# NVlabs/FasterViT

Measured on AMD Instinct MI355X. Metric: images/sec FasterViT-0 224x224 inference, bs=256/GPU, higher is better.
Workload: dtype f16; 1 GPU; faster_vit_0_224 inference, 224x224, batch 256/GPU, synthetic weights (tests/synth.py init family); global_batch=256, parallelism=dp1 (independent shards, no data-path collective), hat_operands=f16, streams=1

## Files before the change

fastervit_amd/_lib.py:

```python
from __future__ import annotations

import ctypes as C
import os
import subprocess

_HERE = os.path.dirname(os.path.abspath(__file__))
CSRC_DIR = os.path.join(_HERE, "csrc")
DIAG = os.environ.get("FVIT_DIAG", "0") == "1"
LIB_PATH = os.path.join(CSRC_DIR, "libfvit_hip_diag.so" if DIAG else "libfvit_hip.so")
if os.environ.get("FVIT_LIB_PATH"):
    LIB_PATH = os.path.abspath(os.environ["FVIT_LIB_PATH"])

FVIT_ABI_VERSION = 10
FVIT_F32, FVIT_F16, FVIT_BF16 = 0, 1, 2
FVIT_TILE_N, FVIT_TILE_K = 128, 64
FVIT_MASK_BIAS = -30000.0
FVIT_MAX_DENSE_SEQ = 208
FVIT_PROF_KINDS = 11

EXPORTED_SYMBOLS = (
    "fvit_abi_version", "fvit_last_error", "fvit_attention_spad", "fvit_attention_dense", "fvit_stage_workspace_bytes", "fvit_workspace_init",
    "fvit_hat_stage_forward", "fvit_hat_block_forward", "fvit_token_init", "fvit_token_init_dyn", "fvit_feature_tap", "fvit_token_init_dyn_backward", "fvit_feature_tap_backward", "fvit_window_partition", "fvit_window_reverse", "fvit_gemm_bias_act",
    "fvit_gemm_residual", "fvit_gemm_terms", "fvit_gemm_residual_splitk", "fvit_gemm_terms_lo", "fvit_window_attention_terms", "fvit_window_attention_long_terms",
    "fvit_gather_layernorm_terms", "fvit_win_mlp_fused_terms", "fvit_win_mlp_split_bytes", "fvit_win_mlp_fused_split", "fvit_win_block_fused_split",
    "fvit_win_block_fused_terms", "fvit_attn_block_fused_terms", "fvit_ct_block_fused_terms", "fvit_window_attention", "fvit_window_attention_long",
    "fvit_gather_layernorm", "fvit_ln_gemm_supported", "fvit_ln_gemm", "fvit_attn_block_supported", "fvit_attn_block_fused",
    "fvit_ct_block_supported", "fvit_ct_block_fused", "fvit_win_block_supported", "fvit_win_block_fused", "fvit_win_mlp_supported",
    "fvit_win_mlp_fused", "fvit_mlp_fused_supported", "fvit_mlp_fused", "fvit_bias_act_cl", "fvit_bias_residual_cl", "fvit_layernorm2d_cl", "fvit_map_pad_cl", "fvit_layernorm2d_crop_cl",
    "fvit_conv3x3_nhwc", "fvit_conv3x3_nhwc_terms", "fvit_conv3x3_dense_k", "fvit_conv3x3_patch_form", "fvit_conv3x3_nhwc_dense", "fvit_conv3x3_nhwc_px_dense", "fvit_conv3x3_c128_band_supported", "fvit_conv3x3_c128_band", "fvit_stem_conv3x3s2",
    "fvit_stem_fused", "fvit_window_attention_drop", "fvit_bwd_window_attention_drop", "fvit_global_avgpool_cl", "fvit_conv3x3_nhwc_px", "fvit_layernorm2d_px", "fvit_stem_conv3x3s2_px", "fvit_head_logits", "fvit_head_softmax_xent",
    "fvit_head_grad", "fvit_sgd_momentum", "fvit_bwd_blocks", "fvit_bwd_transpose16", "fvit_bwd_scale_cols", "fvit_bwd_gelu", "fvit_bwd_layernorm",
    "fvit_bwd_colsum_finish", "fvit_bwd_colsum16", "fvit_bwd_window_attention", "fvit_bwd_window_attention_long",
    "fvit_bwd_window_attention_long_workspace", "fvit_tune", "fvit_prof_enable", "fvit_prof_collect",
    "fvit_prof_records", "fvit_prof_kind_name",
    "fvit_hat_stage_forward_tail", "fvit_rows_avgpool", "fvit_conv3x3_c64_ln2d", "fvit_conv3x3_c128_band_ln2d",
)
DIAG_SYMBOLS = (
    "fvit_debug_lds_poison", "fvit_debug_regs_poison", "fvit_debug_poison_launches", "fvit_debug_rowhash_begin", "fvit_debug_rowhash_end",
    "fvit_debug_rowhash_dump", "fvit_debug_mlp_trace_begin", "fvit_debug_mlp_trace_end", "fvit_debug_mlp_inputs_begin", "fvit_debug_mlp_inputs_end",
    "fvit_debug_win_mlp_timeline", "fvit_debug_stem_timeline", "fvit_debug_conv_band_timeline", "fvit_debug_attn_block_timeline",
    "fvit_debug_ct_block_timeline",
)


class FvitDebugRowhashRecord(C.Structure):
    _fields_ = [("tag", C.c_char * 24), ("offset", C.c_int64), ("rows", C.c_int64)]


class FvitStageDesc(C.Structure):
    _fields_ = [(n, C.c_int32) for n in (
        "batch", "C", "heads", "dpad", "ws", "H", "W", "Hp", "Wp", "cw", "hier", "square", "hidden",
        "depth", "do_propagation", "operand_dtype", "spad", "gpad")] + [("qk_scale", C.c_float), ("weight_terms", C.c_int32)]


class FvitAttnWeights(C.Structure):
    _fields_ = [(n, C.c_void_p) for n in ("w_qkv", "b_qkv", "w_proj", "b_proj", "bias", "ln_w", "ln_b", "gamma",
                                                  "w_qkv_frag", "b_qkv_heads", "w_proj_frag", "rel_table")] + \
               [("rel_w", C.c_int32), ("rel_ng", C.c_int32)]


class FvitMlpWeights(C.Structure):
    _fields_ = [(n, C.c_void_p) for n in ("w_fc1", "b_fc1", "w_fc2", "b_fc2", "ln_w", "ln_b", "gamma", "w_fc1_frag", "w_fc2_frag")]


class FvitBlockWeights(C.Structure):
    _fields_ = [("attn", FvitAttnWeights), ("mlp", FvitMlpWeights), ("hat_attn", FvitAttnWeights),
                ("hat_mlp", FvitMlpWeights), ("pe_x", C.c_void_p), ("pe_ct", C.c_void_p),
                ("last", C.c_int32), ("_pad", C.c_int32)]


class FvitStageTables(C.Structure):
    _fields_ = [(n, C.c_void_p) for n in ("ln1_src", "ln1_add", "ct_src", "up_idx")]


class FvitStageTail(C.Structure):
    _fields_ = [("ln_w", C.c_void_p), ("ln_b", C.c_void_p), ("pool_out", C.c_void_p), ("ln_eps", C.c_float), ("pool_dtype", C.c_int32)]


class FvitMapView(C.Structure):
    _fields_ = [("data", C.c_void_p), ("stride_b", C.c_int64), ("stride_c", C.c_int64), ("stride_h", C.c_int64),
                ("stride_w", C.c_int64), ("dtype", C.c_int32), ("_pad", C.c_int32)]


class FvitProfEntry(C.Structure):
    _fields_ = [("launches", C.c_int64), ("ms", C.c_double), ("flops", C.c_double), ("bytes", C.c_double)]


class FvitProfRecord(C.Structure):
    _fields_ = [("kind", C.c_int32), ("grid", C.c_int32), ("ms", C.c_float), ("_pad", C.c_float), ("flops", C.c_double),
                ("bytes", C.c_double), ("name", C.c_char * 40)]


_lib = None


def build(verbose: bool = False) -> str:
    cmd = ["make", "-C", CSRC_DIR, "-j4"]
    res = subprocess.run(cmd, stdout=subprocess.PIPE, stderr=subprocess.STDOUT, text=True)
    if verbose:
        print(res.stdout)
    if res.returncode != 0 or not os.path.isfile(LIB_PATH):
        raise RuntimeError("building libfvit_hip.so failed:\n" + res.stdout)
    return LIB_PATH


def _declare(lib):
    vp, i32, f32 = C.c_void_p, C.c_int32, C.c_float
    lib.fvit_abi_version.restype = C.c_int
    lib.fvit_last_error.restype = C.c_char_p
    lib.fvit_attention_spad.restype = C.c_int
    lib.fvit_attention_spad.argtypes = [i32]
    lib.fvit_stage_workspace_bytes.restype = C.c_size_t
    lib.fvit_stage_workspace_bytes.argtypes = [C.POINTER(FvitStageDesc)]
    lib.fvit_workspace_init.restype = C.c_int
    lib.fvit_workspace_init.argtypes = [C.POINTER(FvitStageDesc), vp, C.c_size_t, vp]
    lib.fvit_hat_stage_forward.restype = C.c_int
    lib.fvit_hat_stage_forward.argtypes = [C.POINTER(FvitStageDesc), C.POINTER(FvitBlockWeights),
                                           C.POINTER(FvitStageTables), C.POINTER(FvitMapView), vp,
                                           C.POINTER(FvitMapView), vp, C.c_size_t, vp]
    lib.fvit_hat_stage_forward_tail.restype = C.c_int
    lib.fvit_hat_stage_forward_tail.argtypes = [C.POINTER(FvitStageDesc), C.POINTER(FvitBlockWeights),
                                                C.POINTER(FvitStageTables), C.POINTER(FvitMapView), vp,
                                                C.POINTER(FvitMapView), C.POINTER(FvitStageTail), vp, C.c_size_t, vp]
    lib.fvit_rows_avgpool.restype = C.c_int
    lib.fvit_rows_avgpool.argtypes = [i32, vp, vp, i32, i32, i32, vp]
    for fn in (lib.fvit_conv3x3_c64_ln2d, lib.fvit_conv3x3_c128_band_ln2d):
        fn.restype = C.c_int
        fn.argtypes = [i32, vp, vp, vp, vp, vp, vp, vp, f32, i32, i32, i32, vp, vp]
    lib.fvit_hat_block_forward.restype = C.c_int
    lib.fvit_hat_block_forward.argtypes = [C.POINTER(FvitStageDesc), C.POINTER(FvitBlockWeights),
                                           C.POINTER(FvitStageTables), vp, vp, vp, C.c_size_t, vp]
    lib.fvit_token_init.restype = C.c_int
    lib.fvit_token_init.argtypes = [C.POINTER(FvitMapView), vp, vp, vp, i32, i32, i32, i32, i32, i32, i32, i32, i32, vp]
    lib.fvit_token_init_dyn.restype = C.c_int
    lib.fvit_token_init_dyn.argtypes = [C.POINTER(FvitMapView), vp, vp, vp, i32, i32, i32, i32, i32, i32, i32, i32, i32, vp]
    lib.fvit_feature_tap.restype = C.c_int
    lib.fvit_feature_tap.argtypes = [C.POINTER(FvitMapView), i32, i32, i32, i32, vp, vp, vp, vp]
    lib.fvit_token_init_dyn_backward.restype = C.c_int
    lib.fvit_token_init_dyn_backward.argtypes = [C.POINTER(FvitMapView), vp, vp, vp, vp, vp, vp, i32, i32, i32, i32, i32, i32, i32, i32, i32, vp]
    lib.fvit_feature_tap_backward.restype = C.c_int
    lib.fvit_feature_tap_backward.argtypes = [vp, C.POINTER(FvitMapView), C.POINTER(FvitMapView), i32, i32, i32, i32, i32, i32, vp, vp, C.c_int64, vp, vp]
    lib.fvit_window_partition.restype = C.c_int
    lib.fvit_window_partition.argtypes = [C.POINTER(FvitMapView), i32, i32, i32, i32, i32, vp, vp]
    lib.fvit_window_reverse.restype = C.c_int
    lib.fvit_window_reverse.argtypes = [vp, i32, i32, i32, i32, i32, i32, i32, C.POINTER(FvitMapView), vp]
    lib.fvit_gemm_bias_act.restype = C.c_int
    lib.fvit_gemm_bias_act.argtypes = [i32, vp, i32, vp, i32, vp, vp, i32, i32, i32, i32, i32, vp]
    lib.fvit_gemm_residual.restype = C.c_int
    lib.fvit_gemm_residual.argtypes = [i32, vp, i32, vp, i32, vp, vp, vp, i32, i32, i32, i32, vp]
    lib.fvit_gemm_terms.restype = C.c_int
    lib.fvit_gemm_terms.argtypes = [i32, vp, i32, vp, i32, vp, vp, vp, i32, i32, i32, i32, i32, i32, vp]
    lib.fvit_gemm_residual_splitk.restype = C.c_int
    lib.fvit_gemm_residual_splitk.argtypes = [i32, vp, i32, vp, i32, vp, vp, vp, i32, i32, i32, i32, vp, C.c_size_t, vp]
    lib.fvit_gemm_terms_lo.restype = C.c_int
    lib.fvit_gemm_terms_lo.argtypes = [i32, vp, i32, vp, i32, vp, vp, vp, i32, i32, i32, i32, i32, i32, i32, vp]
    lib.fvit_window_attention_terms.restype = C.c_int
    lib.fvit_window_attention_terms.argtypes = [i32, vp, i32, i32, vp, i32, i32, vp, i32, i32, i32, i32, f32, vp]
    lib.fvit_window_attention_long_terms.restype = C.c_int
    lib.fvit_window_attention_long_terms.argtypes = [i32, vp, i32, i32, vp, i32, i32, vp, i32, i32, i32, i32, i32, i32, f32, vp]
    lib.fvit_gather_layernorm_terms.restype = C.c_int
    lib.fvit_gather_layernorm_terms.argtypes = [i32, vp, i32, vp, i32, vp, vp, vp, vp, vp, i32, i32, vp, vp, f32, i32, i32, i32, vp]
    lib.fvit_win_mlp_fused_terms.restype = C.c_int
    lib.fvit_win_mlp_fused_terms.argtypes = [i32, vp, i32, i32, i32, vp, vp, f32, vp, vp, vp, vp, vp, i32, vp]
    lib.fvit_win_mlp_split_bytes.restype = C.c_size_t
    lib.fvit_win_mlp_split_bytes.argtypes = [i32, i32, i32]
    lib.fvit_win_mlp_fused_split.restype = C.c_int
    lib.fvit_win_mlp_fused_split.argtypes = [i32, vp, i32, i32, i32, vp, vp, f32, vp, vp, vp, vp, vp, i32, vp, vp, i32, vp]
    lib.fvit_window_attention.restype = C.c_int
    lib.fvit_window_attention.argtypes = [i32, vp, i32, vp, i32, vp, i32, i32, i32, i32, f32, vp]
    lib.fvit_attention_dense.restype = C.c_int
    lib.fvit_attention_dense.argtypes = [i32, i32]
    lib.fvit_window_attention_long.restype = C.c_int
    lib.fvit_window_attention_long.argtypes = [i32, vp, i32, vp, i32, vp, i32, i32, i32, i32, i32, i32, f32, vp]
    lib.fvit_gather_layernorm.restype = C.c_int
    lib.fvit_gather_layernorm.argtypes = [i32, vp, i32, vp, i32, vp, vp, vp, vp, vp, i32, vp, vp, f32, i32, i32, i32, vp]
    lib.fvit_ln_gemm_supported.restype = C.c_int
    lib.fvit_ln_gemm_supported.argtypes = [i32, i32, i32, i32]
    lib.fvit_ln_gemm.restype = C.c_int
    lib.fvit_ln_gemm.argtypes = [i32, vp, i32, vp, i32, vp, vp, vp, vp, vp, vp, f32, i32, i32, i32, vp, i32, vp, vp, i32, i32, i32, vp]
    lib.fvit_attn_block_supported.restype = C.c_int
    lib.fvit_attn_block_supported.argtypes = [i32, i32, i32]
    lib.fvit_attn_block_fused.restype = C.c_int
    lib.fvit_attn_block_fused.argtypes = [i32, vp, i32, vp, i32, vp, vp, vp, vp, vp, f32, i32, vp, vp, vp, vp, vp, vp, vp, i32, i32, i32, i32,
                                          f32, vp]
    lib.fvit_mlp_fused_supported.restype = C.c_int
    lib.fvit_mlp_fused_supported.argtypes = [i32, i32]
    lib.fvit_mlp_fused.restype = C.c_int
    lib.fvit_mlp_fused.argtypes = [i32, vp, i32, i32, i32, vp, vp, f32, vp, vp, vp, vp, vp, vp]
    lib.fvit_bias_act_cl.restype = C.c_int
    lib.fvit_bias_act_cl.argtypes = [i32, vp, vp, C.c_int64, i32, i32, vp]
    lib.fvit_bias_residual_cl.restype = C.c_int
    lib.fvit_bias_residual_cl.argtypes = [i32, vp, vp, vp, C.c_int64, i32, vp]
    lib.fvit_layernorm2d_cl.restype = C.c_int
    lib.fvit_layernorm2d_cl.argtypes = [i32, vp, vp, vp, vp, f32, C.c_int64, i32, i32, vp]
    lib.fvit_map_pad_cl.restype = C.c_int
    lib.fvit_map_pad_cl.argtypes = [i32, vp, vp, i32, i32, i32, i32, i32, i32, vp]
    lib.fvit_layernorm2d_crop_cl.restype = C.c_int
    lib.fvit_layernorm2d_crop_cl.argtypes = [i32, vp, vp, vp, vp, f32, i32, i32, i32, i32, i32, i32, i32, vp]
    lib.fvit_conv3x3_nhwc.restype = C.c_int
    lib.fvit_conv3x3_nhwc.argtypes = [i32, vp, vp, vp, vp, vp, i32, i32, i32, i32, i32, i32, i32, vp, vp]
    lib.fvit_conv3x3_nhwc_terms.restype = C.c_int
    lib.fvit_conv3x3_nhwc_terms.argtypes = [i32, vp, vp, vp, vp, vp, i32, i32, i32, i32, i32, i32, i32, i32, vp, vp]
    lib.fvit_window_attention_drop.restype = C.c_int
    lib.fvit_window_attention_drop.argtypes = [i32, vp, i32, vp, i32, vp, i32, i32, i32, i32, f32, vp, vp]
    lib.fvit_bwd_window_attention_drop.restype = C.c_int
    lib.fvit_bwd_window_attention_drop.argtypes = [i32, vp, i32, vp, i32, vp, i32, f32, vp, vp, i32, i32, i32, i32, vp, vp]
# ... 176 lines not shown
```

fastervit_amd/conv_runtime.py:

```python
from __future__ import annotations

import ctypes
import os
from typing import NamedTuple, Optional

import torch
import torch.nn.functional as F

from . import _lib, hat_runtime

_CODE = {torch.float16: _lib.FVIT_F16, torch.bfloat16: _lib.FVIT_BF16}


def _stream(device=None):
    return torch.cuda.current_stream(device).cuda_stream


def _bn_scale_shift(bn):
    s = bn.weight.float() / torch.sqrt(bn.running_var.float() + bn.eps)
    t = bn.bias.float() - bn.running_mean.float() * s
    return s, t


def _fold(conv, bn, extra_scale=None):
    s, t = _bn_scale_shift(bn)
    w = conv.weight.float() * s.view(-1, 1, 1, 1)
    b = t if conv.bias is None else conv.bias.float() * s + t
    if extra_scale is not None:
        w = w * extra_scale.float().view(-1, 1, 1, 1)
        b = b * extra_scale.float()
    return w, b


def frag_pack_conv128(w2d: torch.Tensor) -> torch.Tensor:
    assert tuple(w2d.shape) == (128, 1152)
    dev = w2d.device
    wave = torch.arange(4, device=dev).view(4, 1, 1)
    ni = torch.arange(2, device=dev).view(1, 2, 1)
    sl = torch.arange(16, device=dev).view(1, 1, 16)
    ch = (32 * wave + (sl >> 2) * 8 + ni * 4 + (sl & 3)).reshape(-1)
    t = w2d[ch].view(4, 2, 16, 36, 4, 8)
    return t.permute(0, 3, 1, 4, 2, 5).contiguous().view(4, 36, 2, 64, 8)


class ConvWeight(NamedTuple):
    wcl: torch.Tensor
    wk: Optional[torch.Tensor]
    wband: Optional[torch.Tensor]
    terms: int
    cv: int
    wk_classic: Optional[torch.Tensor]


StemW = NamedTuple("StemW", [("conv0", ConvWeight), ("bias0", torch.Tensor), ("conv1", ConvWeight), ("bias1", torch.Tensor)])
BlockW = NamedTuple("BlockW", [("conv1", ConvWeight), ("bias1", torch.Tensor), ("conv2", ConvWeight), ("bias2", torch.Tensor)])
DownW = NamedTuple("DownW", [("ln_w", torch.Tensor), ("ln_b", torch.Tensor), ("eps", float), ("conv", ConvWeight), ("cin", int)])
TokW = NamedTuple("TokW", [("w", torch.Tensor), ("bias", torch.Tensor), ("pool_kernel", object), ("pool_stride", object), ("window", int)])
HeadW = NamedTuple("HeadW", [("w", torch.Tensor), ("b", torch.Tensor), ("ln", Optional[tuple])])


class DeployPlan:
    def __init__(self, model, dtype=torch.float16):
        if dtype not in _CODE:
            raise ValueError("deploy dtype must be torch.float16 or torch.bfloat16")
        self.model = model
        self.dtype = dtype
        self.code = _CODE[dtype]
        self.sig = None
        self.t = None
        self.zeros = None
        self.streams = 1
        self.shard_sizes = None
        self.serialize_shards = False
        self.join_from = None
        self.slot_base = 0
        self._warm_geometries = set()
        self.side = None
        self.dev = None
        self.use_hip_conv = True
        self.pad_channels = True
        self.down_weight_terms = int(os.environ.get("FVIT_DOWN_WEIGHT_TERMS", "1"))
        self.conv_weight_terms = int(os.environ.get("FVIT_CONV_WEIGHT_TERMS", "1"))
        self.precise = os.environ.get("FVIT_PRECISE_DEPLOY", "0") == "1"
        self.dense_k = os.environ.get("FVIT_CONV_DENSE_K", "1") != "0"
        self.fused_stem = os.environ.get("FVIT_NO_FUSED_STEM", "0") != "1"
        self.fuse_conv_ln2d = {64: os.environ.get("FVIT_FUSE_CONV64_LN2D", "1") != "0", 128: os.environ.get("FVIT_FUSE_CONV128_LN2D", "1") != "0"}
        self.fuse_reverse_ln2d = os.environ.get("FVIT_FUSE_REVERSE_LN2D", "1") != "0"
        self.fuse_pool = os.environ.get("FVIT_FUSE_POOL", "1") != "0"

    def _signature(self):
        m = self.model
        sig = []
        for name, p in list(m.named_parameters()) + list(m.named_buffers()):
            if ".blocks." in name and name.startswith(("levels.2.", "levels.3.")):
                continue
            sig.append((p.data_ptr(), p._version))
        sig.append(("options", self.precise, self.conv_weight_terms, self.down_weight_terms, self.dense_k))
        return tuple(sig)

    def _cp(self, c):
        return c if (c % 64 == 0 or c <= 3 or not (self.pad_channels and self.use_hip_conv)) else (c + 63) // 64 * 64

    def _padv(self, v, n):
        if v is None or v.numel() == n:
            return v
        out = torch.zeros(n, dtype=v.dtype, device=v.device)
        out[:v.numel()] = v
        return out

    def _cw(self, w, terms: int = 1) -> ConvWeight:
        co0, ci0 = w.shape[:2]
        cop, cip = self._cp(co0), self._cp(ci0)
        if (cop, cip) != (co0, ci0):
            wp = torch.zeros((cop, cip) + tuple(w.shape[2:]), dtype=w.dtype, device=w.device)
            wp[:co0, :ci0] = w
            w = wp
        wcl = w.to(self.dtype).contiguous(memory_format=torch.channels_last)
        co, ci, kh, kw = w.shape
        wk = wband = None
        cv = ci
        if self.use_hip_conv and kh == 3 and kw == 3 and ci % 64 == 0 and co % 64 == 0:
            wk = wcl.permute(0, 2, 3, 1).contiguous()
            lo = (w - wcl.float()).to(self.dtype).permute(0, 2, 3, 1).contiguous() if terms == 2 else None
            cv8 = (ci0 + 7) // 8 * 8
            if self.dense_k and cv8 < ci:
                cv, kd = cv8, (9 * cv8 + 63) // 64 * 64

                def dense(m):
                    d = torch.zeros((co, kd), dtype=m.dtype, device=m.device)
                    d[:, :9 * cv] = m[..., :cv].reshape(co, 9 * cv)
                    return d
                classic = wk.reshape(co, -1) if lo is None else torch.cat([wk.reshape(co, -1), lo.reshape(co, -1)], dim=1).contiguous()
                wk = dense(wk) if lo is None else torch.cat([dense(wk), dense(lo)], dim=1).contiguous()
                return ConvWeight(wcl, wk, None, terms, cv, classic)
            if terms == 2:
                wk = torch.cat([wk.reshape(co, -1), lo.reshape(co, -1)], dim=1).contiguous()
                return ConvWeight(wcl, wk, None, 2, cv, None)
            if (co, ci) == (128, 128):
                wband = frag_pack_conv128(wk.reshape(128, 1152))
        return ConvWeight(wcl, wk, wband, 1, cv, None)

    def _zero_page(self, device):
        if self.zeros is None or self.zeros.device != device:
            self.zeros = torch.zeros(256, dtype=self.dtype, device=device)
        return self.zeros.data_ptr()

    @staticmethod
    def _conv_launch_shape(x, w: ConvWeight, stride):
        B, Ci, Hi, Wi = x.shape
        wk, cv, Co = w.wk, w.cv, w.wk.shape[0]
        if w.wk_classic is not None and _lib.lib().fvit_conv3x3_patch_form(B, Hi, Wi, Ci, Co, stride):
            wk, cv = w.wk_classic, Ci
        return wk, cv, Co, (Hi - 1) // stride + 1, (Wi - 1) // stride + 1

    def _conv_ln2d_route(self, x, w: ConvWeight, d: "DownW"):
        C_ = x.shape[1]
        if self.precise or not self.use_hip_conv or not self.fuse_conv_ln2d.get(C_, False) or d.cin != C_ or w.wk is None or w.terms != 1 \
                or w.wk_classic is not None or not x.is_contiguous(memory_format=torch.channels_last):
            return None
        lib = _lib.lib()
        if C_ == 64 and tuple(w.wk.shape) == (64, 3, 3, 64):
            return "halo"
        if C_ == 128 and w.wband is not None and lib.fvit_conv3x3_c128_band_supported(x.shape[2], x.shape[3]):
            return "band"
        return None

    def _conv_ln2d(self, route, x, w: ConvWeight, bias, residual, d: "DownW"):
        B, _, Hi, Wi = x.shape
        fn, wt, name = ((_lib.lib().fvit_conv3x3_c64_ln2d, w.wk, "fvit_conv3x3_c64_ln2d") if route == "halo" else
                        (_lib.lib().fvit_conv3x3_c128_band_ln2d, w.wband, "fvit_conv3x3_c128_band_ln2d"))
        _lib.check(fn(self.code, x.data_ptr(), wt.data_ptr(), bias.data_ptr() if bias is not None else None, residual.data_ptr(), residual.data_ptr(),
                      d.ln_w.data_ptr(), d.ln_b.data_ptr(), d.eps, B, Hi, Wi, self._zero_page(x.device), _stream(self.dev)), name)
        return residual

    def _conv(self, x, w: ConvWeight, bias, stride, act, residual=None):
        B, Ci, Hi, Wi = x.shape
        if w.wk is not None and x.is_contiguous(memory_format=torch.channels_last):
            wk, cv, Co, Ho, Wo = self._conv_launch_shape(x, w, stride)
            out = residual if residual is not None else torch.empty((B, Co, Ho, Wo), dtype=self.dtype, device=x.device,
                                                                    memory_format=torch.channels_last)
            zeros = self._zero_page(x.device)
            if w.wband is not None and stride == 1 and _lib.lib().fvit_conv3x3_c128_band_supported(Hi, Wi):
                rc = _lib.lib().fvit_conv3x3_c128_band(self.code, x.data_ptr(), w.wband.data_ptr(), bias.data_ptr() if bias is not None else None,
                                                       residual.data_ptr() if residual is not None else None, out.data_ptr(), B, Hi, Wi, act,
                                                       zeros, _stream(self.dev))
                _lib.check(rc, "fvit_conv3x3_c128_band")
                return out
            rc = _lib.lib().fvit_conv3x3_nhwc_dense(self.code, x.data_ptr(), wk.data_ptr(), bias.data_ptr() if bias is not None else None,
                                                    residual.data_ptr() if residual is not None else None, out.data_ptr(), B, Hi, Wi,
                                                    Ci, cv, Co, stride, act, w.terms, zeros, _stream(self.dev))
            _lib.check(rc, "fvit_conv3x3_nhwc_dense")
            return out
        y = F.conv2d(x, w.wcl, None, stride, 1)
        if residual is not None:
            return self._bias_residual(residual, y, bias)
        return self._bias_act(y, bias, act) if bias is not None else y

    @torch.no_grad()
    def _build(self):
        m = self.model
        t = {}
        pe = m.patch_embed.conv_down
        w0, b0 = _fold(pe[0], pe[1])
        w1, b1 = _fold(pe[3], pe[4])
        ct = 2 if (self.conv_weight_terms == 2 or self.precise) else 1
        t["stem"] = StemW(self._cw(w0), self._padv(b0, self._cp(b0.numel())).contiguous(), self._cw(w1, terms=ct),
                          self._padv(b1, self._cp(b1.numel())).contiguous())
        t["stem_k"] = t["stem_k_lo"] = None
        co0 = self._cp(w0.shape[0])
        w0p = torch.zeros((co0,) + tuple(w0.shape[1:]), dtype=torch.float32, device=w0.device)
        w0p[:w0.shape[0]] = w0
        t["stem0_f32"] = (w0p.contiguous(memory_format=torch.channels_last), self._padv(b0, co0).contiguous(), tuple(pe[0].stride))
        if self.use_hip_conv and tuple(w0.shape) == (64, 3, 3, 3) and pe[0].stride == (2, 2):
            wk = torch.zeros(64, 32, device=w0.device, dtype=torch.float32)
            wk[:, :27] = w0.permute(0, 2, 3, 1).reshape(64, 27)
            t["stem_k"] = wk.to(self.dtype).contiguous()
            t["stem_k_lo"] = (wk - t["stem_k"].float()).to(self.dtype).contiguous()
        t["levels"] = []
        for lvl in m.levels:
            e = {}
            if not lvl.transformer_block:
                blocks = []
                for blk in lvl.blocks:
                    wa, ba = _fold(blk.conv1, blk.norm1)
                    wb, bb = _fold(blk.conv2, blk.norm2, blk.gamma if blk.layer_scale else None)
                    cpd = self._cp(ba.numel())
                    blocks.append(BlockW(self._cw(wa, terms=ct), self._padv(ba, cpd).contiguous(), self._cw(wb, terms=ct), self._padv(bb, cpd).contiguous()))
                e["blocks"] = blocks
            elif getattr(lvl, "do_gt", False):
                tk = lvl.global_tokenizer
                e["tok"] = TokW(self._cw(tk.pos_embed.weight.float()).wcl, tk.pos_embed.bias.to(self.dtype).contiguous(),
                                tk.to_global_feature.pool.kernel_size, tk.to_global_feature.pool.stride, tk.window_size)
            if lvl.downsample is not None:
                ds = lvl.downsample
                cin = ds.norm.weight.numel()
                e["down"] = DownW(self._padv(ds.norm.weight.float(), self._cp(cin)).contiguous(),
                                  self._padv(ds.norm.bias.float(), self._cp(cin)).contiguous(), float(ds.norm.eps),
                                  self._cw(ds.reduction[0].weight.float(), terms=2 if (self.down_weight_terms == 2 or ct == 2) else 1), cin)
            t["levels"].append(e)
        self._build_head(t)
        self.t = t

    def _build_head(self, t):
        m = self.model
        if isinstance(m.head, torch.nn.Linear):
            hw = m.head.weight.float()
            hb = m.head.bias.float() if m.head.bias is not None else torch.zeros(hw.shape[0], device=hw.device)
        else:
# ... 82 lines not shown

    def _forward_sharded(self, x):
        n = self.streams
        if n <= 1 or x.shape[0] < 2 * n:
            with hat_runtime.workspace_slot(self.slot_base):
                return self._forward_one(x)
        sb, sizes, warm = self.slot_base, self.shard_sizes, self._warm_geometries
        parts = x.split(list(sizes), dim=0) if sizes and sum(sizes) == x.shape[0] and len(sizes) == n else x.chunk(n, dim=0)
        outs = [None] * n
        ops = tuple(getattr(lvl, "hat_operand_dtype", "f16") for lvl in self.model.levels if lvl.transformer_block)
        wkey = (str(x.device), tuple(p.shape[0] for p in parts), tuple(x.shape[1:]), ops, self.join_from, sb)
        serial = self.serialize_shards or not self._hat_prepared(x.device) or wkey not in warm
        jf = self.join_from if (self.join_from is not None and 0 < self.join_from < len(self.model.levels)) else None
        front = (lambda xi: self._forward_one(xi, 0, jf)) if jf is not None else self._forward_one
        def _cat(xs):
            if isinstance(xs[0], tuple):
                return tuple(None if xs[0][k] is None else torch.cat([x_[k] for x_ in xs], dim=0) for k in range(3))
            return torch.cat(xs, dim=0)
        back = (lambda xs: self._forward_one(_cat(xs), jf, None)) if jf is not None else (lambda xs: torch.cat(xs, dim=0))
        if serial:
            for i in range(n):
                with hat_runtime.workspace_slot(sb + i):
                    outs[i] = front(parts[i])
            with hat_runtime.workspace_slot(sb):
                y = back(outs)
            if not torch.cuda.is_current_stream_capturing():
                warm.add(wkey)
            return y
        if self.side is None or len(self.side) != n - 1 or self.side[0].device != x.device:
            self.side = [torch.cuda.Stream(device=x.device) for _ in range(n - 1)]
        main = torch.cuda.current_stream(x.device)
        for i, s in enumerate(self.side):
            s.wait_stream(main)
            with torch.cuda.stream(s), hat_runtime.workspace_slot(sb + i + 1):
                outs[i + 1] = front(parts[i + 1])
        with hat_runtime.workspace_slot(sb):
            outs[0] = front(parts[0])
        for s in self.side:
            main.wait_stream(s)
        with hat_runtime.workspace_slot(sb):
            return back(outs)

    def shard_runner(self, x, n=None):
        return ShardRunner(self, x, n or max(self.streams, 1))

    def _conv_px(self, x, x_lo, w: ConvWeight, bias, stride, act, res=None, res_lo=None, want="planes"):
        if w.wk is None or not x.is_contiguous(memory_format=torch.channels_last):
            raise RuntimeError("precise deploy plan: this conv shape has no implicit-GEMM kernel (channel counts must pad to multiples of 64)")
        B, Ci, Hi, Wi = x.shape
        wk, cv, Co, Ho, Wo = self._conv_launch_shape(x, w, stride)
        zeros = self._zero_page(x.device)
        hi = lo = f32 = None
        if want == "f32":
            f32 = torch.empty((B, Co, Ho, Wo), dtype=torch.float32, device=x.device, memory_format=torch.channels_last)
        else:
            hi = res if res is not None else torch.empty((B, Co, Ho, Wo), dtype=self.dtype, device=x.device, memory_format=torch.channels_last)
            if want == "planes":
                lo = res_lo if res_lo is not None else torch.empty_like(hi)
        rc = _lib.lib().fvit_conv3x3_nhwc_px_dense(self.code, x.data_ptr(), x_lo.data_ptr() if x_lo is not None else None, wk.data_ptr(),
                                             bias.data_ptr() if bias is not None else None, res.data_ptr() if res is not None else None,
                                             res_lo.data_ptr() if res_lo is not None else None, hi.data_ptr() if hi is not None else None,
                                             lo.data_ptr() if lo is not None else None, f32.data_ptr() if f32 is not None else None,
                                             B, Hi, Wi, Ci, cv, Co, stride, act, w.terms, zeros, _stream(self.dev))
        _lib.check(rc, "fvit_conv3x3_nhwc_px_dense")
        return f32 if want == "f32" else (hi, lo)

    def _ln2d_px(self, x, x_lo, x_f32, w, b, eps, c_valid):
        src = x_f32 if x_f32 is not None else x
        B, C, H, W = src.shape
        if C % 8 or not src.is_contiguous(memory_format=torch.channels_last):
            raise RuntimeError("precise deploy plan: LayerNorm2d needs a channels_last map with C % 8 == 0")
        hi = torch.empty((B, C, H, W), dtype=self.dtype, device=src.device, memory_format=torch.channels_last)
        lo = torch.empty_like(hi)
        _lib.check(_lib.lib().fvit_layernorm2d_px(self.code, x.data_ptr() if x is not None else None, x_lo.data_ptr() if x_lo is not None else None,
                                                  x_f32.data_ptr() if x_f32 is not None else None, hi.data_ptr(), lo.data_ptr(), w.data_ptr(),
                                                  b.data_ptr(), eps, B * H * W, C, c_valid, _stream(self.dev)), "fvit_layernorm2d_px")
        return hi, lo

    def _forward_one(self, x, lv_from=0, lv_to=None):
        levels = self.model.levels
        with torch.autocast(device_type="cuda", enabled=False):
            if lv_from == 0:
                x = self._stem(x)
            for li, (lvl, e) in enumerate(zip(levels, self.t["levels"])):
                if li < lv_from or (lv_to is not None and li >= lv_to):
                    continue
                normed = pooled = False
                if "blocks" in e:
                    x, normed = self._conv_level(x, e["blocks"], e.get("down"))
                elif self._pool_tail(lvl, x, last=li + 1 == len(levels) and lv_to is None and "down" not in e):
                    x, pooled = self._hat_level_pooled(lvl, x), True
                else:
                    x, normed = self._hat_level(lvl, x, padded_out="down" in e, down=e.get("down"))
                if "down" in e:
                    x = self._downsample(x, e["down"], f32_out=li + 1 < len(levels) and levels[li + 1].transformer_block, normed=normed)
            if lv_to is not None:
                return x
            return self._head_logits(x, *self.t["head"][:2]) if pooled else self._head(x)

    def _stem(self, x):
        t, st = self.t, self.t["stem"]
        k27 = t["stem_k"] is not None and x.shape[1] == 3 and x.dtype in hat_runtime._DT
        if self.precise:
            if not k27:
                wf, bf, st0 = t["stem0_f32"]
                y = torch.relu(F.conv2d(x.float(), wf, bf, st0, 1)).to(self.dtype).contiguous(memory_format=torch.channels_last)
            else:
                B, _, Hi, Wi = x.shape
                y = torch.empty((B, 64, (Hi - 1) // 2 + 1, (Wi - 1) // 2 + 1), dtype=self.dtype, device=x.device, memory_format=torch.channels_last)
                view = hat_runtime._map_view(x)
                _lib.check(_lib.lib().fvit_stem_conv3x3s2_px(self.code, view, t["stem_k"].data_ptr(), t["stem_k_lo"].data_ptr(), st.bias0.data_ptr(),
                                                             y.data_ptr(), B, Hi, Wi, _stream(self.dev)), "fvit_stem_conv3x3s2_px")
            return (*self._conv_px(y, None, st.conv1, st.bias1, 2, 1), None)
        wk1 = st.conv1.wk
        if self.fused_stem and k27 and wk1 is not None and st.conv1.terms == 1 and tuple(wk1.shape) == (64, 3, 3, 64):
            B, _, Hi, Wi = x.shape
            H1, W1 = (Hi - 1) // 2 + 1, (Wi - 1) // 2 + 1
            y = torch.empty((B, 64, (H1 - 1) // 2 + 1, (W1 - 1) // 2 + 1), dtype=self.dtype, device=x.device,
                            memory_format=torch.channels_last)
            view = hat_runtime._map_view(x)
            _lib.check(_lib.lib().fvit_stem_fused(self.code, view, t["stem_k"].data_ptr(), st.bias0.data_ptr(), wk1.data_ptr(),
                                                  st.bias1.data_ptr(), y.data_ptr(), B, Hi, Wi, _stream(self.dev)), "fvit_stem_fused")
            return y
        if k27:
            B, _, Hi, Wi = x.shape
            y = torch.empty((B, 64, (Hi - 1) // 2 + 1, (Wi - 1) // 2 + 1), dtype=self.dtype, device=x.device,
                            memory_format=torch.channels_last)
            view = hat_runtime._map_view(x)
            _lib.check(_lib.lib().fvit_stem_conv3x3s2(self.code, view, t["stem_k"].data_ptr(), st.bias0.data_ptr(), y.data_ptr(),
                                                      B, Hi, Wi, _stream(self.dev)), "fvit_stem_conv3x3s2")
            return self._conv(y, st.conv1, st.bias1, 2, 1)
        x = x.to(self.dtype).contiguous(memory_format=torch.channels_last)
        return self._conv(self._conv(x, st.conv0, st.bias0, 2, 1), st.conv1, st.bias1, 2, 1)

    def _conv_level(self, x, blocks, down: Optional["DownW"] = None):
        if not self.precise:
            normed = False
            for i, b in enumerate(blocks):
                y = self._conv(x, b.conv1, b.bias1, 1, 2)
                route = self._conv_ln2d_route(y, b.conv2, down) if (down is not None and i + 1 == len(blocks)) else None
                if route is not None:
                    x, normed = self._conv_ln2d(route, y, b.conv2, b.bias2, x, down), True
                else:
                    x = self._conv(y, b.conv2, b.bias2, 1, 0, residual=x)
            return x, normed
        hi, lo, f32 = x
        if hi is None:
            hi = f32.to(self.dtype)
            lo = (f32 - hi.float()).to(self.dtype)
        for b in blocks:
            y, _ = self._conv_px(hi, None, b.conv1, b.bias1, 1, 2, want="single")
            hi, lo = self._conv_px(y, None, b.conv2, b.bias2, 1, 0, res=hi, res_lo=lo)
        return (hi, lo, None), False

    def _pool_tail(self, lvl, x, last):
        return (last and self.fuse_pool and not self.precise and self.t["head"].ln is None and torch.is_tensor(x) and len(lvl.blocks) > 0
                and x.shape[1] == lvl.blocks[0].attn.qkv.in_features and x.shape[1] % 16 == 0 and self.t["head"].w.shape[1] == x.shape[1]
                and hat_runtime.pool_tail_supported(lvl, x))

    def _hat_level_pooled(self, lvl, x):
        feat = torch.empty((x.shape[0], x.shape[1]), dtype=torch.float32, device=x.device)
        return hat_runtime.stage_forward(lvl, x, pool_out=feat)

    def _hat_level(self, lvl, x, padded_out, tokenizer=None, down: Optional["DownW"] = None):
        if self.precise:
            hi, lo, x = x
            if x is None:
                x = hi.float() + lo.float()
        creal = lvl.blocks[0].attn.qkv.in_features if len(lvl.blocks) else x.shape[1]
        xin = x[:, :creal] if x.shape[1] != creal else x
        cpo = self._cp(creal) if padded_out else creal
        xo = torch.empty((x.shape[0], cpo, x.shape[2], x.shape[3]), dtype=torch.float32 if self.precise else self.dtype, device=x.device,
                         memory_format=torch.channels_last)
        if cpo != creal:
            xo[:, creal:] = 0
            hat_runtime.stage_forward(lvl, xin, tokenizer=tokenizer, out=xo[:, :creal])
            return ((None, None, xo) if self.precise else xo), False
        if (down is not None and self.fuse_reverse_ln2d and not self.precise and down.cin == creal and len(lvl.blocks)
                and hat_runtime.ln2d_tail_supported(xin, xo)):
            return hat_runtime.stage_forward(lvl, xin, tokenizer=tokenizer, out=xo, ln2d=(down.ln_w, down.ln_b, down.eps)), True
        xo = hat_runtime.stage_forward(lvl, xin, tokenizer=tokenizer, out=xo)
        return ((None, None, xo) if self.precise else xo), False

    def _downsample(self, x, d: DownW, f32_out, normed=False):
        if not self.precise:
            return self._conv(x if normed else self._ln2d(x, d.ln_w, d.ln_b, d.eps, d.cin), d.conv, None, 2, 0)
        hi, lo, f32 = x
        if f32 is not None and not f32.is_contiguous(memory_format=torch.channels_last):
            f32 = f32.contiguous(memory_format=torch.channels_last)
        nh, nl = self._ln2d_px(hi, lo, f32, d.ln_w, d.ln_b, d.eps, d.cin)
        if f32_out:
            return None, None, self._conv_px(nh, nl, d.conv, None, 2, 0, want="f32")
        return (*self._conv_px(nh, nl, d.conv, None, 2, 0), None)

    def _head(self, x):
        hw, hb, ln = self.t["head"]
        if not self.precise:
            return self._pool_head(x if ln is None else self._ln2d(x, *ln), hw, hb)
        hi, lo, f32 = x
        if f32 is None:
            f32 = hi.float() + lo.float()
        if ln is not None:
            nh, nl = self._ln2d_px(None, None, f32.contiguous(memory_format=torch.channels_last), *ln, f32.shape[1])
            f32 = nh.float() + nl.float()
        return self._pool_head(f32, hw, hb)


class LevelMap(NamedTuple):
    x: torch.Tensor
    H: int
    W: int

    @property
    def dense(self) -> bool:
        return self.x.shape[2] == self.H and self.x.shape[3] == self.W


TapW = NamedTuple("TapW", [("scale", torch.Tensor), ("shift", torch.Tensor), ("channels", int)])


class BackboneDeployPlan(DeployPlan):

    def __init__(self, model, dtype=torch.float16):
        super().__init__(model, dtype)
        self._check_options()
        for i in model.out_indices:
            bn = getattr(model, f"norm{i}")
            hat_runtime._folded_bn(bn, (bn.running_mean if bn.running_mean is not None else next(model.parameters())).device)

    def _check_options(self):
        if self.precise:
            raise NotImplementedError("backbone deploy plan: precise=True is not implemented (there is no two-term feature tap); use the 16-bit plan, "
                                      "or module mode with set_hat_operand_dtype('f16x3')")
        if self.conv_weight_terms != 1 or self.down_weight_terms != 1:
            raise NotImplementedError("backbone deploy plan: two-term conv weights (conv_weight_terms / down_weight_terms = 2) are not implemented")
        if self.streams != 1:
            raise NotImplementedError("backbone deploy plan: streams > 1 (stream shards) is not implemented; detection batches are small")

    def _build_head(self, t):
        m = self.model
        dev = next(m.parameters()).device
        t["taps"] = {i: TapW(*hat_runtime._folded_bn(getattr(m, f"norm{i}"), dev), m.num_features[i]) for i in m.out_indices}

    def forward(self, x):
        self._check_options()
        self._enter(x)
        with torch.cuda.device(x.device):
            self._refresh()
            with hat_runtime.workspace_slot(self.slot_base):
                return self._walk(x)

    forward_single = forward

    def _walk(self, x):
        levels, taps = self.model.levels, self.t["taps"]
        outs = []
        with torch.autocast(device_type="cuda", enabled=False):
            y = self._stem(x)
            m = LevelMap(y, y.shape[2], y.shape[3])
            for li, (lvl, e) in enumerate(zip(levels, self.t["levels"])):
                if "blocks" in e:
                    m = self._conv_level_padded(m, e["blocks"], lvl.window_size)
                else:
                    m = self._hat_level_dyn(lvl, m, padded_out="down" in e)
                if li in taps:
                    outs.append(self._tap(m, taps[li]))
                if "down" in e:
                    m = self._downsample_crop(m, e["down"])
        return tuple(outs)
# ... 89 lines not shown
```

fastervit_amd/csrc/fvit_api.hip:

```cpp
#include <stdarg.h>
#include <stdlib.h>
#include <string.h>

#include <algorithm>
#include <map>
#include <mutex>
#include <string>
#include <vector>

#include "fvit_common.h"

namespace fvit {

static thread_local char g_err[512] = "";

void set_error(const char* fmt, ...) {
    va_list ap;
    va_start(ap, fmt);
    vsnprintf(g_err, sizeof(g_err), fmt, ap);
    va_end(ap);
}

int check_launch(const char* what) {
    hipError_t e = hipGetLastError();
// ... 423 lines not shown
        break;
    }
    case WinAttnRoute::CHAIN: {
        LnCall ln1 = ln_call(d, L, a.ln_w, a.ln_b, X, L.Mx, win.xn);
        ln1.rowsA = L.rpi; ln1.srcB = R; ln1.rowsB = L.G; ln1.src_idx = d.hier ? t.ln1_src : nullptr; ln1.add_idx = t.ln1_add; ln1.add = w.pe_x;
        ln1.x_out = X; ln1.rows_per_image = L.rpi;
        FVIT_TRY(launch_gather_layernorm(ln1, st));
        dbg_rowhash("win.gather", X, L.Mx, d.C * 4, st);
        FVIT_TRY(run_attn(d, L, a, AttnStart::QKV_GEMM, win, ws, st));
        break;
    }
    }
    return run_mlp(d, L, w.mlp, r.window_mlp, r, win, t, ws, st);
}

static int check_hat_call(const FvitStageDesc* desc, bool args_ok, const FvitStageTables* t, const void* workspace, size_t workspace_bytes,
                          const void* carrier, const char* no_carrier, StageLayout& L) {
    if (!desc || !args_ok) {
        set_error("null argument");
        return FVIT_EINVAL;
    }
    const FvitStageDesc& d = *desc;
    if (!make_layout(d, L)) return FVIT_EINVAL;
    if (!t || !t->ln1_add || (d.hier && (!t->ln1_src || !t->ct_src)) || (d.hier && d.do_propagation && !t->up_idx)) {
        set_error("stage tables missing (ln1_add%s)", d.hier ? ", ln1_src, ct_src, up_idx" : "");
        return FVIT_EINVAL;
    }
    if (!workspace || workspace_bytes < L.total) {
        set_error("workspace too small: %zu < %zu", workspace_bytes, L.total);
        return FVIT_EWORKSPACE;
    }
    if (d.hier && !carrier) {
        set_error("%s", no_carrier);
        return FVIT_EINVAL;
    }
    return FVIT_OK;
}

}

using namespace fvit;

extern "C" {

int fvit_abi_version(void) { return FVIT_ABI_VERSION; }
const char* fvit_last_error(void) { return g_err; }

int fvit_attention_dense(int32_t S, int32_t dpad) { return attention_dense(S, dpad) ? 1 : 0; }

int fvit_attention_spad(int32_t S) {
    int sb = (S + 15) / 16;
    if (sb == 9) sb = 10;
    if (sb == 11 || sb == 12) sb = 13;
    return sb * 16;
}

size_t fvit_stage_workspace_bytes(const FvitStageDesc* desc) {
    StageLayout L;
    if (!desc || !make_layout(*desc, L)) return 0;
    return L.total;
}

int fvit_workspace_init(const FvitStageDesc* desc, void* workspace, size_t bytes, fvit_stream_t stream) {
    StageLayout L;
    if (!desc || !make_layout(*desc, L)) return FVIT_EINVAL;
    if (!workspace || bytes < L.total) {
        set_error("workspace too small: %zu < %zu", bytes, L.total);
        return FVIT_EWORKSPACE;
    }
    if (hipMemsetAsync(workspace, 0, L.total, (hipStream_t)stream) != hipSuccess) return check_launch("workspace memset");
    return FVIT_OK;
}

int fvit_hat_stage_forward(const FvitStageDesc* desc, const FvitBlockWeights* blocks, const FvitStageTables* tables,
                           const FvitMapView* in, const float* ct_init, const FvitMapView* out, void* workspace,
                           size_t workspace_bytes, fvit_stream_t stream) {
    return fvit_hat_stage_forward_tail(desc, blocks, tables, in, ct_init, out, nullptr, workspace, workspace_bytes, stream);
}

int fvit_rows_avgpool(int32_t round_dtype, const float* x, float* out, int32_t B, int32_t rows, int32_t C, fvit_stream_t stream) {
    return launch_rows_avgpool(x, out, B, rows, C, round_dtype, (hipStream_t)stream);
}

int fvit_hat_stage_forward_tail(const FvitStageDesc* desc, const FvitBlockWeights* blocks, const FvitStageTables* tables,
                                const FvitMapView* in, const float* ct_init, const FvitMapView* out, const FvitStageTail* tail,
                                void* workspace, size_t workspace_bytes, fvit_stream_t stream) {
    StageLayout L;
    const bool pooled = tail && tail->pool_out;
    FVIT_TRY(check_hat_call(desc, blocks && in && (out || pooled), tables, workspace, workspace_bytes, ct_init, "hierarchical stage needs ct_init", L));
    const FvitStageDesc& d = *desc;
    if (tail && (!tail->ln_w != !tail->ln_b || (pooled && tail->ln_w))) {
        set_error("stage tail: LayerNorm2d needs both ln_w and ln_b, and excludes pool_out");
        return FVIT_EINVAL;
    }
    if (pooled && (d.hier || L.nW != 1 || L.ncw != 0 || d.H != d.Hp || d.W != d.Wp)) {
        set_error("stage tail: pool_out needs one window per image and no carrier tokens (hier=%d, %d windows, map %dx%d of %dx%d)", d.hier, L.nW, d.H, d.W,
                  d.Hp, d.Wp);
        return FVIT_EINVAL;
    }
    hipStream_t st = (hipStream_t)stream;
    char* ws = (char*)workspace;
    float* X = (float*)(ws + L.off_X);
    PartitionCall pc = {*in, d.batch, d.C, d.Hp, d.Wp, d.ws, X, L.S, L.ncw, d.hier ? ct_init : nullptr, L.ncw};
    FVIT_TRY(launch_partition(pc, st));
    dbg_rowhash("partition", X, L.Mx, d.C * 4, st);
    const RouteKnobs knobs{};
    std::vector<BlockRoute> routes;
    for (int i = 0; i < d.depth; ++i) routes.push_back(choose_route(d, L, blocks[i], knobs));
    for (int i = 0; i + 1 < d.depth; ++i) {
        if (routes[i].preadd_eligible && routes[i + 1].preadd_eligible && blocks[i + 1].pe_x) {
            routes[i].pe_next = blocks[i + 1].pe_x;
            routes[i + 1].window_attn = WinAttnRoute::LNGEMM_PREADDED;
        }
    }
    for (int i = 0; i < d.depth; ++i) FVIT_TRY(run_block(d, L, routes[i], blocks[i], *tables, ws, st));
    if (pooled)
        return launch_rows_avgpool(X, tail->pool_out, d.batch, L.S, d.C, tail->pool_dtype, st);
    const bool prop = d.hier && d.do_propagation && d.depth > 0 && blocks[d.depth - 1].last;
    ReverseCall rc = {X, L.S, L.ncw, d.batch, d.C, d.Hp, d.Wp, d.H, d.W, d.ws, *out,
                      prop ? blocks[d.depth - 1].hat_attn.gamma : nullptr, prop ? tables->up_idx : nullptr};
    if (tail && tail->ln_w) return launch_reverse_ln(rc, tail->ln_w, tail->ln_b, tail->ln_eps, st);
    FVIT_TRY(launch_reverse(rc, st));
    return FVIT_OK;
}

int fvit_hat_block_forward(const FvitStageDesc* desc, const FvitBlockWeights* block, const FvitStageTables* tables, float* x,
                           float* ct, void* workspace, size_t workspace_bytes, fvit_stream_t stream) {
    StageLayout L;
    FVIT_TRY(check_hat_call(desc, block && x, tables, workspace, workspace_bytes, ct, "hierarchical block needs carrier tokens", L));
    const FvitStageDesc& d = *desc;
    hipStream_t st = (hipStream_t)stream;
    char* ws = (char*)workspace;
    float* X = (float*)(ws + L.off_X);
    const int nwin = d.batch * L.nW;
    FVIT_TRY(launch_ct_copy(X, L.S, L.ncw, L.nloc, x, nwin, d.C, 1, st));
    if (d.hier) FVIT_TRY(launch_ct_copy(X, L.S, 0, L.ncw, ct, nwin, d.C, 1, st));
    FVIT_TRY(run_block(d, L, choose_route(d, L, *block, RouteKnobs{}), *block, *tables, ws, st));
    if (d.hier && block->last && d.do_propagation)
        FVIT_TRY(launch_propagate(X, block->hat_attn.gamma, tables->up_idx, L.S, L.ncw, L.nloc, nwin, d.C, st));
    FVIT_TRY(launch_ct_copy(X, L.S, L.ncw, L.nloc, x, nwin, d.C, 0, st));
    if (d.hier) FVIT_TRY(launch_ct_copy(X, L.S, 0, L.ncw, ct, nwin, d.C, 0, st));
    return FVIT_OK;
}

int fvit_token_init(const FvitMapView* in, const float* weight, const float* bias, float* ct_out, int32_t batch, int32_t C, int32_t Hp,
                    int32_t Wp, int32_t pool_kh, int32_t pool_kw, int32_t pool_sh, int32_t pool_sw, int32_t cw, fvit_stream_t stream) {
    if (!in || !weight || !bias || !ct_out) { set_error("null argument"); return FVIT_EINVAL; }
    return launch_token_init(*in, weight, bias, ct_out, batch, C, Hp, Wp, pool_kh, pool_kw, pool_sh, pool_sw, cw, (hipStream_t)stream);
}

int fvit_window_partition(const FvitMapView* in, int32_t batch, int32_t C, int32_t Hp, int32_t Wp, int32_t ws, float* windows,
                          fvit_stream_t stream) {
    if (!in || !windows) { set_error("null argument"); return FVIT_EINVAL; }
    PartitionCall pc = {*in, batch, C, Hp, Wp, ws, windows, ws * ws, 0, nullptr, 0};
    return launch_partition(pc, (hipStream_t)stream);
}

int fvit_window_reverse(const float* windows, int32_t batch, int32_t C, int32_t Hp, int32_t Wp, int32_t H, int32_t W, int32_t ws,
                        const FvitMapView* out, fvit_stream_t stream) {
    if (!out || !windows) { set_error("null argument"); return FVIT_EINVAL; }
    ReverseCall rc = {windows, ws * ws, 0, batch, C, Hp, Wp, H, W, ws, *out, nullptr, nullptr};
    return launch_reverse(rc, (hipStream_t)stream);
}

int fvit_gemm_bias_act(int32_t operand_dtype, const void* A, int32_t lda, const void* Wt, int32_t ldw, const float* bias, void* out,
                       int32_t ldo, int32_t M, int32_t N, int32_t K, int32_t act, fvit_stream_t stream) {
    GemmCall g = {operand_dtype, A, lda, Wt, ldw, bias, nullptr, out, ldo, M, N, K, act ? 1 : 0};
    return launch_gemm(g, (hipStream_t)stream);
}

int fvit_gemm_residual(int32_t operand_dtype, const void* A, int32_t lda, const void* Wt, int32_t ldw, const float* bias,
                       const float* gamma, float* x, int32_t ldx, int32_t M, int32_t N, int32_t K, fvit_stream_t stream) {
    GemmCall g = {operand_dtype, A, lda, Wt, ldw, bias, gamma, x, ldx, M, N, K, 2};
    return launch_gemm(g, (hipStream_t)stream);
}

int fvit_gemm_residual_splitk(int32_t operand_dtype, const void* A, int32_t lda, const void* Wt, int32_t ldw, const float* bias, const float* gamma,
                              float* x, int32_t ldx, int32_t M, int32_t N, int32_t K, float* slab, size_t slab_bytes, fvit_stream_t stream) {
    GemmCall g = {operand_dtype, A, lda, Wt, ldw, bias, gamma, x, ldx, M, N, K, 2};
    g.splitk_slab = slab;
    g.splitk_bytes = slab_bytes;
    return launch_gemm(g, (hipStream_t)stream);
}

int fvit_gemm_terms(int32_t operand_dtype, const void* A, int32_t lda, const void* Wt, int32_t ldw, const float* bias, const float* gamma,
                    void* out, int32_t ldo, int32_t M, int32_t N, int32_t K, int32_t ka, int32_t epilogue, fvit_stream_t stream) {
    if (epilogue < 0 || epilogue > 2) { set_error("gemm_terms: epilogue %d", epilogue); return FVIT_EINVAL; }
    GemmCall g = {operand_dtype, A, lda, Wt, ldw, bias, epilogue == 2 ? gamma : nullptr, out, ldo, M, N, K, epilogue};
    g.ka = ka;
    return launch_gemm(g, (hipStream_t)stream);
}

int fvit_gemm_terms_lo(int32_t operand_dtype, const void* A, int32_t lda, const void* Wt, int32_t ldw, const float* bias, const float* gamma,
                       void* out, int32_t ldo, int32_t out_lo_off, int32_t M, int32_t N, int32_t K, int32_t ka, int32_t epilogue,
                       fvit_stream_t stream) {
    if (epilogue < 0 || epilogue > 2) { set_error("gemm_terms_lo: epilogue %d", epilogue); return FVIT_EINVAL; }
    GemmCall g = {operand_dtype, A, lda, Wt, ldw, bias, epilogue == 2 ? gamma : nullptr, out, ldo, M, N, K, epilogue};
    g.ka = ka;
    g.out_lo_off = out_lo_off;
    return launch_gemm(g, (hipStream_t)stream);
}

int fvit_window_attention_terms(int32_t operand_dtype, const void* qkv, int32_t ldq, int32_t q_lo_off, void* out, int32_t ldo,
                                int32_t o_lo_off, const float* bias, int32_t nwin, int32_t S, int32_t heads, int32_t dpad, float scale,
                                fvit_stream_t stream) {
    AttnCall a = {operand_dtype, qkv, ldq, out, ldo, bias, nwin, S, heads, dpad, scale, nullptr, 0, 0, 0};
    a.q_lo_off = q_lo_off;
    a.o_lo_off = o_lo_off;
    if (q_lo_off <= 0 || o_lo_off <= 0) { set_error("window_attention_terms: q_lo_off / o_lo_off must be > 0"); return FVIT_EINVAL; }
    return launch_attention(a, (hipStream_t)stream);
}

int fvit_gather_layernorm_terms(int32_t operand_dtype, const float* srcA, int32_t rowsA, const float* srcB, int32_t rowsB,
                                const int32_t* src_idx, const int32_t* add_idx, const float* add, float* x_out, void* n_out, int32_t ldn,
                                int32_t lo_off, const float* ln_w, const float* ln_b, float eps, int32_t rows, int32_t rows_per_image,
                                int32_t C, fvit_stream_t stream) {
    LnCall c = {operand_dtype, srcA, rowsA, srcB, rowsB, src_idx, add_idx, add, x_out, n_out, ldn, ln_w, ln_b, eps, rows,
                rows_per_image, C};
    c.lo_off = lo_off;
    return launch_gather_layernorm(c, (hipStream_t)stream);
}

int fvit_window_attention(int32_t operand_dtype, const void* qkv, int32_t ldq, void* out, int32_t ldo, const float* bias,
                          int32_t nwin, int32_t S, int32_t heads, int32_t dpad, float scale, fvit_stream_t stream) {
    if (!attention_dense(S, dpad)) {
        set_error("window_attention: S=%d at dpad=%d is outside the dense-bias kernel (fvit_attention_dense); use fvit_window_attention_long", S, dpad);
        return FVIT_EINVAL;
    }
    AttnCall a = {operand_dtype, qkv, ldq, out, ldo, bias, nwin, S, heads, dpad, scale, nullptr, 0, 0, 0};
    return launch_attention(a, (hipStream_t)stream);
}
// ... 282 lines not shown
```

fastervit_amd/csrc/fvit_common.h:

```cpp
#pragma once
#include <hip/hip_runtime.h>
#include <stdint.h>
#include <atomic>
#include <mutex>
#include <stdio.h>

#include "../../include/fvit_hip.h"

namespace fvit {

typedef _Float16 h8 __attribute__((ext_vector_type(8)));
typedef _Float16 h4 __attribute__((ext_vector_type(4)));
typedef __bf16 b8 __attribute__((ext_vector_type(8)));
typedef __bf16 b4 __attribute__((ext_vector_type(4)));
typedef float f4 __attribute__((ext_vector_type(4)));

template <typename T> struct Op16;
template <> struct Op16<_Float16> {
    typedef h8 v8;
    typedef h4 v4;
    static __device__ __forceinline__ f4 mfma(v8 a, v8 b, f4 c) {
        return __builtin_amdgcn_mfma_f32_16x16x32_f16(a, b, c, 0, 0, 0);
    }
};
// ... 326 lines not shown
    const void* drop_mask = nullptr;
};
bool attention_dense(int S, int dpad);
int launch_attention(const AttnCall& c, hipStream_t stream);
int launch_attention_long(const AttnCall& c, hipStream_t stream);

struct LnCall {
    int dtype;
    const float* srcA;
    int rowsA;
    const float* srcB;
    int rowsB;
    const int32_t* src_idx;
    const int32_t* add_idx;
    const float* add;
    float* x_out;
    void* n_out;
    int ldn;
    const float* ln_w;
    const float* ln_b;
    float eps;
    int rows, rows_per_image, C;
    int lo_off = 0;
};
int launch_gather_layernorm(const LnCall& c, hipStream_t stream);

struct CtBlkCall {
    int dtype;
    const float* X; int rowsA;
    const int32_t* src_idx;
    const float* add;
    float* R;
    int batch, G, heads, C, hidden;
    const float* ln1_w; const float* ln1_b; const void* wqkv_f; const float* bqkv; const void* wproj_f; const float* bproj; const float* gamma1;
    const float* bias; float scale;
    const float* ln2_w; const float* ln2_b; const void* w1f; const float* b1; const void* w2f; const float* b2; const float* gamma2;
    float eps;
    int terms = 1;
    void* ts = nullptr;
};
bool ctblk_supported(int C, int heads, int G, int hidden);
int launch_ctblk(const CtBlkCall& c, hipStream_t stream);

struct LnGemmCall {
    LnCall ln;
    const void* W;
    int ldw;
    const float* bias;
    void* out;
    int ldo;
    int N;
    int epilogue;
};
bool ln_gemm_supported(int C, int N, int ldw, int ldo);
int launch_ln_gemm(const LnGemmCall& c, hipStream_t stream);

struct PartitionCall {
    FvitMapView in;
    int batch, C, Hp, Wp, ws;
    float* x;
    int rows_per_win;
    int row_off;
    const float* ct;
    int ncw;
};
int launch_partition(const PartitionCall& c, hipStream_t stream);

struct ReverseCall {
    const float* x;
    int rows_per_win, row_off;
    int batch, C, Hp, Wp, H, W, ws;
    FvitMapView out;
    const float* gamma;
    const int32_t* up_idx;
};
int launch_reverse(const ReverseCall& c, hipStream_t stream);
bool reverse_ln_supported(const ReverseCall& c);
int launch_reverse_ln(const ReverseCall& c, const float* ln_w, const float* ln_b, float eps, hipStream_t stream);
int launch_rows_avgpool(const float* x, float* out, int batch, int rows, int C, int round_dtype, hipStream_t stream);

int launch_ct_copy(float* x, int rows_per_win, int row_off, int ncw, float* ct, int nwin_total, int C, int to_x,
                   hipStream_t stream);
int launch_token_init(const FvitMapView& in, const float* w, const float* bias, float* out, int B, int C, int Hp, int Wp, int kh, int kw,
                      int sh, int sw, int cw, hipStream_t stream);
int launch_propagate(float* x, const float* gamma, const int32_t* up_idx, int rows_per_win, int ncw, int nloc,
                     int nwin_total, int C, hipStream_t stream);

}
```

fastervit_amd/csrc/fvit_conv.hip:

```cpp
#include "fvit_common.h"

namespace fvit {

namespace {

constexpr int BK = 64;

struct ConvParams {
    const void* in;
    const void* w;
    const float* bias;
    const void* res;
    void* out;
    const void* zeros;
    int B, Hi, Wi, Cin, Cout, Ho, Wo, stride, act;
    int M, tiles_m, tiles_n;
    int ablate;
    int wterms;
    const void* in_lo;
    const void* res_lo;
    void* out_lo;
    float* out_f32;
    int px;
    int cv, kd;
    float inv_cv;
};

__device__ __forceinline__ int swz_x(int r) { return (r >> 1) & 7; }
__device__ __forceinline__ int swz_w(int r) { return ((0x78 >> (2 * ((r >> 4) & 3))) & 3) | ((r & 2) << 1); }

__device__ __forceinline__ void glds16(const void* gsrc, char* lds_dst) {
    __builtin_amdgcn_global_load_lds((const __attribute__((address_space(1))) void*)gsrc,
                                     (__attribute__((address_space(3))) void*)lds_dst, 16, 0, 0);
}

template <int V> struct IntTag { static constexpr int value = V; };
template <typename F>
__device__ __forceinline__ void dispatch_epilogue(int act, bool has_res, F&& body) {
    if (has_res) {
        if (act == 0) body(IntTag<0>{}, IntTag<1>{});
        else if (act == 1) body(IntTag<1>{}, IntTag<1>{});
        else body(IntTag<2>{}, IntTag<1>{});
    } else {
        if (act == 0) body(IntTag<0>{}, IntTag<0>{});
        else if (act == 1) body(IntTag<1>{}, IntTag<0>{});
        else body(IntTag<2>{}, IntTag<0>{});
    }
}

constexpr int PATCH_H = 8, PATCH_W = 16, PHALO_W = PATCH_W + 2, PHALO_ROWS = (PATCH_H + 2) * PHALO_W;
constexpr int PHALO_PIECES = (PHALO_ROWS + 7) / 8;
constexpr int PHALO_BYTES = PHALO_PIECES * 1024;

template <typename T, int WM, int WN, int NI, bool PX = false, bool DENSE = false, bool HALO = false>
__global__ __launch_bounds__(256, 2) void conv3x3_kernel(ConvParams p) {
    typedef typename Op16<T>::v8 v8;
    static_assert(!HALO || (WM == 2 && WN == 2 && !DENSE), "halo form: 8 x 16 patches on the 2 x 2 wave grid, classic weight layout");
    constexpr int BM = 64 * WM, BN = 16 * NI * WN;
    constexpr int X_BYTES = HALO ? PHALO_BYTES : BM * BK * 2, W_BYTES = BN * BK * 2;
    constexpr int XP = BM / 8 / 4;
    constexpr int HP = (PHALO_PIECES + 3) / 4;
    constexpr int WPIECES = BN / 8;
    constexpr int WP = (WPIECES + 3) / 4;
    static_assert(2 * (X_BYTES + W_BYTES) <= 80 * 1024, "two workgroups per CU");
    __shared__ __attribute__((aligned(16))) char smem[2 * (X_BYTES + W_BYTES)];

    const int tid = threadIdx.x;
    const int lane = tid & 63;
    const int wave = __builtin_amdgcn_readfirstlane(tid >> 6);
    const int wm = wave / WN, wn = wave - wm * WN;

    const int nblk = gridDim.x, b = blockIdx.x;
    const int q = nblk >> 3, rr = nblk & 7, xcd = b & 7, idx = b >> 3;
    const int v = (xcd < rr ? xcd * (q + 1) : rr * (q + 1) + (xcd - rr) * q) + idx;
    const int tm = v / p.tiles_n, tn = v - tm * p.tiles_n;
    const int m0 = tm * BM, n0 = tn * BN;

    const T* __restrict__ In = (const T*)p.in;
    const T* __restrict__ W = (const T*)p.w;
    const T* __restrict__ Z = (const T*)p.zeros;
    const int ldw = DENSE ? p.wterms * p.kd * BK : p.wterms * 9 * p.Cin;

    f4 acc[NI][4];
#pragma unroll
    for (int i = 0; i < NI; ++i)
#pragma unroll
        for (int j = 0; j < 4; ++j) acc[i][j] = (f4){0.f, 0.f, 0.f, 0.f};

    const int g = lane >> 4, s = lane & 15;
    int bimg = 0, y0 = 0, x0 = 0;
    if constexpr (HALO) {
        const int tpx = (p.Wo + PATCH_W - 1) / PATCH_W, tpy = (p.Ho + PATCH_H - 1) / PATCH_H;
        bimg = tm / (tpy * tpx);
        const int rem = tm - bimg * (tpy * tpx);
        const int ty = rem / tpx;
        y0 = ty * PATCH_H;
        x0 = (rem - ty * tpx) * PATCH_W;
    }
    if constexpr (HALO) {
        int hoff[HP];
        int hvalid = 0;
        int hchunk[HP];
#pragma unroll
        for (int i = 0; i < HP; ++i) {
            const int piece = wave + 4 * i;
            const int r = piece * 8 + (lane >> 3);
            const int hy = r / PHALO_W, hx = r - hy * PHALO_W;
            const int iy = y0 - 1 + hy, ix = x0 - 1 + hx;
            const int chunk = ((lane & 7) ^ swz_x(r)) * 8;
            hchunk[i] = chunk;
            const bool ok = piece < PHALO_PIECES && r < PHALO_ROWS && iy >= 0 && iy < p.Hi && ix >= 0 && ix < p.Wi;
            if (ok) hvalid |= 1 << i;
            hoff[i] = ok ? ((bimg * p.Hi + iy) * p.Wi + ix) * p.Cin + chunk : 0;
        }
        const int ncc = p.Cin / BK;
        const int kpb_hi = p.wterms * 9;
        const int nblk_hi = ncc, nblk_all = ncc * ((PX && p.in_lo) ? 2 : 1);
        const int nk = nblk_hi * kpb_hi + (nblk_all - nblk_hi) * 9;
        const T* const InLo = (PX && p.in_lo) ? (const T*)p.in_lo : In;
        auto stage_halo = [&](int blk, char* xbuf) {
            const bool lo = blk >= nblk_hi;
            const T* const plane = lo ? InLo : In;
            const int c0 = (lo ? blk - nblk_hi : blk) * BK;
#pragma unroll
            for (int i = 0; i < HP; ++i) {
                const int piece = wave + 4 * i;
                if (piece < PHALO_PIECES) {
                    const T* src = ((hvalid >> i) & 1) ? plane + (hoff[i] + c0) : Z + hchunk[i];
                    glds16(src, xbuf + piece * 1024);
                }
            }
        };
        auto stage_w = [&](int blk, int kin, char* wbuf) {
            const bool lo = blk >= nblk_hi;
            const int c0 = (lo ? blk - nblk_hi : blk) * BK;
            const int col = kin * p.Cin + c0;
#pragma unroll
            for (int i = 0; i < WP; ++i) {
                const int piece = wave * WP + i;
// ... 149 lines not shown
            for (int i = 0; i < NI; ++i) wf[kk][i] = *(const v8*)(wt + wrow[i] * 128 + ((c ^ swz_w(wrow[i])) << 4));
        }
        __builtin_amdgcn_sched_barrier(0);
        if (!(p.ablate & 4))
#pragma unroll
        for (int kk = 0; kk < 2; ++kk)
#pragma unroll
            for (int ni = 0; ni < NI; ++ni)
#pragma unroll
                for (int mi = 0; mi < 4; ++mi) acc[ni][mi] = Op16<T>::mfma(wf[kk][ni], xf[kk][mi], acc[ni][mi]);
    }
    }
    if (p.ablate & 8) return;

    auto rowm = [&](int mi) {
        if constexpr (HALO) {
            const int y = y0 + wm * 4 + mi, x = x0 + s;
            return (y < p.Ho && x < p.Wo) ? (bimg * p.Ho + y) * p.Wo + x : p.M;
        } else {
            return m0 + wm * 64 + mi * 16 + s;
        }
    };
    constexpr int NC = 4 * NI;
    typedef T vout __attribute__((ext_vector_type(NC)));
    const int nb = n0 + wn * 16 * NI + g * NC;
    if (nb >= p.Cout) return;
    float bias[NC];
#pragma unroll
    for (int j = 0; j < NI; ++j) {
        const f4 t = p.bias ? *(const f4*)(p.bias + nb + j * 4) : (f4){0.f, 0.f, 0.f, 0.f};
        bias[j * 4 + 0] = t[0]; bias[j * 4 + 1] = t[1]; bias[j * 4 + 2] = t[2]; bias[j * 4 + 3] = t[3];
    }
    T* O = (T*)p.out;
    const T* R = (const T*)p.res;
    if constexpr (PX) {
        const T* RL = (const T*)p.res_lo;
        T* OL = (T*)p.out_lo;
        float* OF = p.out_f32;
        auto px_epilogue = [&](auto act_tag) {
            constexpr int ACT = decltype(act_tag)::value;
#pragma unroll
            for (int mi = 0; mi < 4; ++mi) {
                const int m = rowm(mi);
                if (m < p.M) {
                    float y[NC];
#pragma unroll
                    for (int ni = 0; ni < NI; ++ni)
#pragma unroll
                        for (int r = 0; r < 4; ++r) {
                            float v = acc[ni][mi][r] + bias[ni * 4 + r];
                            if (ACT == 1) v = fmaxf(v, 0.f);
                            y[ni * 4 + r] = v;
                        }
                    if constexpr (ACT == 2) gelu_erf_each<NC>(y);
                    if (R) {
                        const vout rv = *(const vout*)(R + (size_t)m * p.Cout + nb);
#pragma unroll
                        for (int j = 0; j < NC; ++j) y[j] += (float)rv[j];
                        if (RL) {
                            const vout rl = *(const vout*)(RL + (size_t)m * p.Cout + nb);
#pragma unroll
                            for (int j = 0; j < NC; ++j) y[j] += (float)rl[j];
                        }
                    }
                    if (OF) {
#pragma unroll
                        for (int j = 0; j < NC; j += 4) *(f4*)(OF + (size_t)m * p.Cout + nb + j) = (f4){y[j], y[j + 1], y[j + 2], y[j + 3]};
                    } else {
                        vout oh, ol;
#pragma unroll
                        for (int j = 0; j < NC; ++j) {
                            oh[j] = sat16<T>(y[j]);
                            ol[j] = sat16<T>(y[j] - (float)oh[j]);
                        }
                        *(vout*)(O + (size_t)m * p.Cout + nb) = oh;
                        if (OL) *(vout*)(OL + (size_t)m * p.Cout + nb) = ol;
                    }
                }
            }
        };
        if (p.act == 0) px_epilogue(IntTag<0>{});
        else if (p.act == 1) px_epilogue(IntTag<1>{});
        else px_epilogue(IntTag<2>{});
        return;
    }
    dispatch_epilogue(p.act, R != nullptr, [&](auto act_tag, auto res_tag) {
        constexpr int ACT = decltype(act_tag)::value;
        constexpr bool RES = decltype(res_tag)::value != 0;
        vout rvs[4];
        if (RES) {
#pragma unroll
            for (int mi = 0; mi < 4; ++mi) rvs[mi] = *(const vout*)(R + (size_t)min(rowm(mi), p.M - 1) * p.Cout + nb);
            __builtin_amdgcn_sched_barrier(0);
        }
#pragma unroll
        for (int mi = 0; mi < 4; ++mi) {
            const int m = rowm(mi);
            if (m < p.M) {
                vout rv;
                if (RES) rv = rvs[mi];
                vout ov;
                float yv[NI * 4];
#pragma unroll
                for (int ni = 0; ni < NI; ++ni) {
                    const f4 a = acc[ni][mi];
#pragma unroll
                    for (int r = 0; r < 4; ++r) {
                        float y = a[r] + bias[ni * 4 + r];
                        if (ACT == 1) y = fmaxf(y, 0.f);
                        yv[ni * 4 + r] = y;
                    }
                }
                if constexpr (ACT == 2) gelu_fast_each<NI * 4>(yv);
#pragma unroll
                for (int j = 0; j < NI * 4; ++j) ov[j] = (T)(RES ? yv[j] + (float)rv[j] : yv[j]);
                *(vout*)(O + (size_t)m * p.Cout + nb) = ov;
            }
        }
    });
}


struct StemParams {
    FvitMapView in;
    const void* w;
    const float* bias;
    void* out;
    int B, Hi, Wi, Ho, Wo, M;
    const void* w_lo;
};

__device__ __forceinline__ float stem_load(const FvitMapView& v, int64_t off) {
    if (v.dtype == FVIT_F32) return ((const float*)v.data)[off];
    if (v.dtype == FVIT_F16) return (float)((const _Float16*)v.data)[off];
    return (float)((const __bf16*)v.data)[off];
}

template <typename T, bool PX = false>
__global__ __launch_bounds__(256) void stem_conv_kernel(StemParams p) {
    typedef typename Op16<T>::v8 v8;
    const int lane = threadIdx.x & 63;
    const int g = lane >> 4, s = lane & 15;
    const T* __restrict__ W = (const T*)p.w;
    v8 wf[4], wl[4];
#pragma unroll
    for (int ni = 0; ni < 4; ++ni) wf[ni] = *(const v8*)(W + ((s >> 2) * 16 + ni * 4 + (s & 3)) * 32 + g * 8);
    if constexpr (PX) {
#pragma unroll
        for (int ni = 0; ni < 4; ++ni) wl[ni] = *(const v8*)((const T*)p.w_lo + ((s >> 2) * 16 + ni * 4 + (s & 3)) * 32 + g * 8);
    }
    float bias[16];
#pragma unroll
    for (int j = 0; j < 4; ++j) {
        const f4 t = *(const f4*)(p.bias + g * 16 + j * 4);
        bias[j * 4 + 0] = t[0]; bias[j * 4 + 1] = t[1]; bias[j * 4 + 2] = t[2]; bias[j * 4 + 3] = t[3];
    }
    T* __restrict__ O = (T*)p.out;
    const int hw = p.Ho * p.Wo;
    const int nblk16 = (p.M + 15) >> 4;
    int64_t toff[8];
    int tky[8], tkx[8];
#pragma unroll
    for (int e = 0; e < 8; ++e) {
        const int k = g * 8 + e;
        const int ky = k / 9, r9 = k - ky * 9, kx = r9 / 3, c = r9 - kx * 3;
        tky[e] = k < 27 ? ky : -100000;
// ... 874 lines not shown
                    }
                }
            }
            pf_sink ^= pf0 ^ pf1;
        }
        FVIT_SF_MARK(tsA)
        __syncthreads();
        FVIT_SF_MARK(tsBar)

        const char* hb = img + (2 * ph * 4) * SF_ROWPITCH;
        f4 acc[2][4];
#pragma unroll
        for (int i = 0; i < 2; ++i)
#pragma unroll
            for (int j = 0; j < 4; ++j) acc[i][j] = (f4){0.f, 0.f, 0.f, 0.f};
        v8 xf[2][4];
#pragma unroll
        for (int mi = 0; mi < 4; ++mi) xf[0][mi] = *(const v8*)(hb + (2 * mi) * SF_ROWPITCH + xoff[0]);
        __builtin_amdgcn_sched_barrier(0);
#pragma unroll
        for (int q = 0; q < 18; ++q) {
            const int tap = q >> 1, kk = q & 1;
            if (q + 1 < 18) {
                const int tap1 = (q + 1) >> 1, kk1 = (q + 1) & 1, ky1 = tap1 / 3, kx1 = tap1 - ky1 * 3;
                const int o = xoff[kx1] ^ (kk1 << 6);
#pragma unroll
                for (int mi = 0; mi < 4; ++mi) xf[(q + 1) & 1][mi] = *(const v8*)(hb + (2 * mi + ky1) * SF_ROWPITCH + o);
            }
#pragma unroll
            for (int ni = 0; ni < 2; ++ni)
#pragma unroll
                for (int mi = 0; mi < 4; ++mi) acc[ni][mi] = Op16<T>::mfma(wf[tap][kk][ni], xf[q & 1][mi], acc[ni][mi]);
            __builtin_amdgcn_sched_barrier(0);
        }

        FVIT_SF_MARK(tsB)
        const f4 t0 = *(const f4*)(sb2 + nb), t1 = *(const f4*)(sb2 + nb + 4);
        const float bias[8] = {t0[0], t0[1], t0[2], t0[3], t1[0], t1[1], t1[2], t1[3]};
        const int x = tx * HALO_TW + s;
#pragma unroll
        for (int mi = 0; mi < 4; ++mi) {
            const int y = ty * HALO_TH + ph * 4 + mi;
            if (y < p.H2 && x < p.W2) {
                v8 ov;
#pragma unroll
                for (int ni = 0; ni < 2; ++ni)
#pragma unroll
                    for (int r = 0; r < 4; ++r) ov[ni * 4 + r] = (T)fmaxf(acc[ni][mi][r] + bias[ni * 4 + r], 0.f);
                *(v8*)(O + (((size_t)b * p.H2 + y) * p.W2 + x) * 64 + nb) = ov;
            }
        }
        FVIT_SF_MARK(tsE)
    }
    if (pf_sink == 0x9E3779B1u && p.tiles == -12345) ((unsigned*)p.out)[0] = pf_sink;
    if constexpr (TS) {
        if (p.ts && lane == 0) {
            unsigned long long* o = p.ts + ((size_t)blockIdx.x * 4 + wave) * 8;
            o[0] = tsA; o[1] = tsBar; o[2] = tsB; o[3] = tsE; o[4] = tsBar0; o[5] = tsN; o[6] = __builtin_amdgcn_s_memtime() - tsT0; o[7] = 0;
        }
    }
#undef FVIT_SF_MARK
}

static bool patch_form_ok(const ConvParams& p) {
    if (!tune_get("conv_patch", 1) || p.stride != 1 || p.cv || p.Cout < 128 || (p.Cin % BK)) return false;
    if ((int64_t)p.B * p.Hi * p.Wi * p.Cin >= 0x7fffffffLL) return false;
    const int64_t tiles = (int64_t)p.B * ((p.Ho + PATCH_H - 1) / PATCH_H) * ((p.Wo + PATCH_W - 1) / PATCH_W);
    return tiles * 128 * 100 <= (int64_t)p.M * (100 + tune_get("conv_patch_max_waste_pct", 10));
}

template <typename T>
int launch_t(ConvParams& p, hipStream_t stream) {
    if (p.Cin == 64 && p.Cout == 64 && p.stride == 1 && p.wterms == 1 && !p.px && !p.cv && tune_get("conv_halo", 1)) {
        if (ablate_skip(64)) return FVIT_OK;
        return launch_halo_t<T>(p, stream);
    }
    if (ablate_skip(32)) return FVIT_OK;
    const double flops = 2.0 * p.M * (double)p.Cout * 9.0 * (p.cv ? p.cv : p.Cin);
    const double bytes = 2.0 * ((double)p.B * p.Hi * p.Wi * p.Cin * (p.in_lo ? 2.0 : 1.0) + (double)p.M * p.Cout * ((p.res ? (p.res_lo ? 2.0 : 1.0) : 0.0) + ((p.out_lo || p.out_f32) ? 2.0 : 1.0)) +
                               9.0 * p.wterms * p.Cin * p.Cout);
    ProfScope prof(FVIT_K_CONV, flops, bytes, stream);
    const int variant = tune_get("conv64_variant", 0);
    const int narrow = tune_get("conv128_narrow", 0);
    const bool patch = patch_form_ok(p) && (p.Cout % 128 == 0 || (p.Cout > 128 && tune_get("conv_n128_ragged", 1))) && !narrow;
    if (patch) {
        p.tiles_m = p.B * ((p.Ho + PATCH_H - 1) / PATCH_H) * ((p.Wo + PATCH_W - 1) / PATCH_W);
        p.tiles_n = (p.Cout + 127) / 128;
        const dim3 grid_(p.tiles_m * p.tiles_n);
        prof_note(p.px ? "conv3x3_kernel<2,2,4,px,patch>" : "conv3x3_kernel<2,2,4,patch>", p.tiles_m * p.tiles_n);
        if (p.px) hipLaunchKernelGGL((conv3x3_kernel<T, 2, 2, 4, true, false, true>), grid_, dim3(256), 0, stream, p);
        else hipLaunchKernelGGL((conv3x3_kernel<T, 2, 2, 4, false, false, true>), grid_, dim3(256), 0, stream, p);
        return check_launch("conv3x3_kernel<patch>");
    }
#define FVIT_CONV_LAUNCH(WM_, WN_, NI_, PX_)                                                                                            \
    do {                                                                                                                                \
        const dim3 grid_(p.tiles_m * p.tiles_n);                                                                                        \
        if (p.cv) hipLaunchKernelGGL((conv3x3_kernel<T, WM_, WN_, NI_, PX_, true>), grid_, dim3(256), 0, stream, p);                    \
        else hipLaunchKernelGGL((conv3x3_kernel<T, WM_, WN_, NI_, PX_, false>), grid_, dim3(256), 0, stream, p);                        \
    } while (0)
    if (p.px) {
        p.tiles_m = (p.M + 127) / 128;
        if (p.Cout % 128 == 0 || (p.Cout > 128 && tune_get("conv_n128_ragged", 1))) {
            p.tiles_n = (p.Cout + 127) / 128;
            prof_note(p.cv ? "conv3x3_kernel<2,2,4,px,dense>" : "conv3x3_kernel<2,2,4,px>", p.tiles_m * p.tiles_n);
            FVIT_CONV_LAUNCH(2, 2, 4, true);
        } else {
            p.tiles_n = p.Cout / 64;
            prof_note(p.cv ? "conv3x3_kernel<2,2,2,px,dense>" : "conv3x3_kernel<2,2,2,px>", p.tiles_m * p.tiles_n);
            FVIT_CONV_LAUNCH(2, 2, 2, true);
        }
        return check_launch("conv3x3_kernel<px>");
    }
    if ((p.Cout % 128 == 0 || (p.Cout > 128 && tune_get("conv_n128_ragged", 1))) && !narrow) {
        p.tiles_m = (p.M + 127) / 128;
        p.tiles_n = (p.Cout + 127) / 128;
        prof_note(p.cv ? "conv3x3_kernel<2,2,4,dense>" : "conv3x3_kernel<2,2,4>", p.tiles_m * p.tiles_n);
        FVIT_CONV_LAUNCH(2, 2, 4, false);
    } else if (variant == 1 && !p.cv) {
        p.tiles_m = (p.M + 255) / 256;
        p.tiles_n = p.Cout / 64;
        prof_note("conv3x3_kernel<4,1,4>", p.tiles_m * p.tiles_n);
        hipLaunchKernelGGL((conv3x3_kernel<T, 4, 1, 4>), dim3(p.tiles_m * p.tiles_n), dim3(256), 0, stream, p);
    } else {
        p.tiles_m = (p.M + 127) / 128;
        p.tiles_n = p.Cout / 64;
        prof_note(p.cv ? "conv3x3_kernel<2,2,2,dense>" : "conv3x3_kernel<2,2,2>", p.tiles_m * p.tiles_n);
        FVIT_CONV_LAUNCH(2, 2, 2, false);
    }
    return check_launch("conv3x3_kernel");
#undef FVIT_CONV_LAUNCH
}

}
}

using namespace fvit;

extern "C" int fvit_conv3x3_nhwc_terms(int32_t dtype, const void* in, const void* weight, const float* bias, const void* residual, void* out,
                                       int32_t B, int32_t Hi, int32_t Wi, int32_t Cin, int32_t Cout, int32_t stride, int32_t act,
                                       int32_t weight_terms, const void* zeros, fvit_stream_t stream);
extern "C" int fvit_conv3x3_nhwc_dense(int32_t dtype, const void* in, const void* weight, const float* bias, const void* residual, void* out,
                                       int32_t B, int32_t Hi, int32_t Wi, int32_t Cin, int32_t cin_valid, int32_t Cout, int32_t stride, int32_t act,
                                       int32_t weight_terms, const void* zeros, fvit_stream_t stream);

extern "C" int fvit_conv3x3_nhwc(int32_t dtype, const void* in, const void* weight, const float* bias, const void* residual, void* out,
                                 int32_t B, int32_t Hi, int32_t Wi, int32_t Cin, int32_t Cout, int32_t stride, int32_t act,
                                 const void* zeros, fvit_stream_t stream) {
    return fvit_conv3x3_nhwc_terms(dtype, in, weight, bias, residual, out, B, Hi, Wi, Cin, Cout, stride, act, 1, zeros, stream);
}

static bool set_dense(ConvParams& p, int cin_valid) {
    p.cv = 0; p.kd = 0; p.inv_cv = 0.f;
    if (cin_valid == p.Cin) return true;
    if (cin_valid <= 0 || cin_valid > p.Cin || (cin_valid % 8)) return false;
    p.cv = cin_valid;
    p.kd = (9 * cin_valid + BK - 1) / BK;
    p.inv_cv = 1.0f / (float)cin_valid;
    return true;
}

extern "C" int fvit_conv3x3_patch_form(int32_t B, int32_t Hi, int32_t Wi, int32_t Cin, int32_t Cout, int32_t stride) {
    if (B <= 0 || Hi <= 0 || Wi <= 0 || Cin <= 0 || Cout <= 0) return 0;
    ConvParams p;
    p.B = B; p.Hi = Hi; p.Wi = Wi; p.Cin = Cin; p.Cout = Cout; p.stride = stride; p.cv = 0;
    p.Ho = (Hi + 2 - 3) / stride + 1; p.Wo = (Wi + 2 - 3) / stride + 1;
    p.M = B * p.Ho * p.Wo;
    return patch_form_ok(p) && (Cout % 128 == 0 || (Cout > 128 && tune_get("conv_n128_ragged", 1))) && !tune_get("conv128_narrow", 0) ? 1 : 0;
}

extern "C" int fvit_conv3x3_dense_k(int32_t cin_valid) { return cin_valid > 0 && cin_valid % 8 == 0 ? (9 * cin_valid + BK - 1) / BK * BK : -1; }

extern "C" int fvit_conv3x3_nhwc_terms(int32_t dtype, const void* in, const void* weight, const float* bias, const void* residual, void* out,
                                       int32_t B, int32_t Hi, int32_t Wi, int32_t Cin, int32_t Cout, int32_t stride, int32_t act,
                                       int32_t weight_terms, const void* zeros, fvit_stream_t stream) {
    return fvit_conv3x3_nhwc_dense(dtype, in, weight, bias, residual, out, B, Hi, Wi, Cin, Cin, Cout, stride, act, weight_terms, zeros, stream);
}

extern "C" int fvit_conv3x3_nhwc_dense(int32_t dtype, const void* in, const void* weight, const float* bias, const void* residual, void* out,
                                       int32_t B, int32_t Hi, int32_t Wi, int32_t Cin, int32_t cin_valid, int32_t Cout, int32_t stride, int32_t act,
                                       int32_t weight_terms, const void* zeros, fvit_stream_t stream) {
    if (!in || !weight || !out || !zeros || B <= 0 || Hi <= 0 || Wi <= 0 || Cin <= 0 || Cout <= 0 || (Cin % 64) || (Cout % 64) ||
        (stride != 1 && stride != 2) || act < 0 || act > 2 || (weight_terms != 1 && weight_terms != 2)) {
        set_error("conv3x3: unsupported arguments Cin=%d Cout=%d stride=%d act=%d (need Cin %% 64 == 0, Cout %% 64 == 0, stride 1|2)",
                  Cin, Cout, stride, act);
        return FVIT_EINVAL;
    }
    ConvParams p;
    p.in = in; p.w = weight; p.bias = bias; p.res = residual; p.out = out; p.zeros = zeros;
    p.B = B; p.Hi = Hi; p.Wi = Wi; p.Cin = Cin; p.Cout = Cout; p.stride = stride; p.act = act;
    p.ablate = diag_knob("conv_ablate");
    p.wterms = weight_terms;
    p.in_lo = p.res_lo = nullptr; p.out_lo = nullptr; p.out_f32 = nullptr; p.px = 0;
    if (!set_dense(p, cin_valid)) {
        set_error("conv3x3: cin_valid=%d must be a multiple of 8 in (0, Cin=%d]", cin_valid, Cin);
        return FVIT_EINVAL;
    }
    p.Ho = (Hi + 2 - 3) / stride + 1;
    p.Wo = (Wi + 2 - 3) / stride + 1;
    const int64_t M = (int64_t)B * p.Ho * p.Wo;
    if (M > 0x7fffffff) {
        set_error("conv3x3: %lld output pixels exceed the 32-bit row index", (long long)M);
        return FVIT_EINVAL;
    }
    p.M = (int)M;
    if (dtype == FVIT_F16) return launch_t<_Float16>(p, (hipStream_t)stream);
    if (dtype == FVIT_BF16) return launch_t<__bf16>(p, (hipStream_t)stream);
    set_error("conv3x3: dtype %d not supported (16-bit maps only)", dtype);
    return FVIT_EINVAL;
}

extern "C" int fvit_conv3x3_nhwc_px_dense(int32_t dtype, const void* in, const void* in_lo, const void* weight, const float* bias, const void* residual,
                                          const void* residual_lo, void* out, void* out_lo, float* out_f32, int32_t B, int32_t Hi, int32_t Wi, int32_t Cin,
                                          int32_t cin_valid, int32_t Cout, int32_t stride, int32_t act, int32_t weight_terms, const void* zeros,
                                          fvit_stream_t stream);

extern "C" int fvit_conv3x3_nhwc_px(int32_t dtype, const void* in, const void* in_lo, const void* weight, const float* bias, const void* residual,
                                    const void* residual_lo, void* out, void* out_lo, float* out_f32, int32_t B, int32_t Hi, int32_t Wi, int32_t Cin,
                                    int32_t Cout, int32_t stride, int32_t act, int32_t weight_terms, const void* zeros, fvit_stream_t stream) {
    return fvit_conv3x3_nhwc_px_dense(dtype, in, in_lo, weight, bias, residual, residual_lo, out, out_lo, out_f32, B, Hi, Wi, Cin, Cin, Cout, stride, act,
                                      weight_terms, zeros, stream);
}

extern "C" int fvit_conv3x3_nhwc_px_dense(int32_t dtype, const void* in, const void* in_lo, const void* weight, const float* bias, const void* residual,
                                          const void* residual_lo, void* out, void* out_lo, float* out_f32, int32_t B, int32_t Hi, int32_t Wi, int32_t Cin,
                                          int32_t cin_valid, int32_t Cout, int32_t stride, int32_t act, int32_t weight_terms, const void* zeros,
                                          fvit_stream_t stream) {
    if (!in || !weight || (!out && !out_f32) || !zeros || B <= 0 || Hi <= 0 || Wi <= 0 || Cin <= 0 || Cout <= 0 || (Cin % 64) || (Cout % 64) ||
        (stride != 1 && stride != 2) || act < 0 || act > 2 || (weight_terms != 1 && weight_terms != 2) || (in_lo && weight_terms != 2) ||
        (residual_lo && !residual) || (out_f32 && out_lo) || (out_lo && !out)) {
        set_error("conv3x3_px: unsupported arguments Cin=%d Cout=%d stride=%d act=%d weight_terms=%d (need Cin %% 64 == 0, Cout %% 64 == 0, stride 1|2, "
                  "weight_terms 2 with a two-term input, out or out_f32)", Cin, Cout, stride, act, weight_terms);
        return FVIT_EINVAL;
    }
    ConvParams p;
    p.in = in; p.w = weight; p.bias = bias; p.res = residual; p.out = out; p.zeros = zeros;
    p.B = B; p.Hi = Hi; p.Wi = Wi; p.Cin = Cin; p.Cout = Cout; p.stride = stride; p.act = act;
    p.ablate = 0;
    p.wterms = weight_terms;
    p.in_lo = in_lo; p.res_lo = residual_lo; p.out_lo = out_lo; p.out_f32 = out_f32; p.px = 1;
    if (!set_dense(p, cin_valid)) {
        set_error("conv3x3_px: cin_valid=%d must be a multiple of 8 in (0, Cin=%d]", cin_valid, Cin);
        return FVIT_EINVAL;
    }
    p.Ho = (Hi + 2 - 3) / stride + 1;
    p.Wo = (Wi + 2 - 3) / stride + 1;
    const int64_t M = (int64_t)B * p.Ho * p.Wo;
    if (M > 0x7fffffff) {
        set_error("conv3x3_px: %lld output pixels exceed the 32-bit row index", (long long)M);
        return FVIT_EINVAL;
    }
    p.M = (int)M;
    if (dtype == FVIT_F16) return launch_t<_Float16>(p, (hipStream_t)stream);
    if (dtype == FVIT_BF16) return launch_t<__bf16>(p, (hipStream_t)stream);
    set_error("conv3x3_px: dtype %d not supported (16-bit planes only)", dtype);
    return FVIT_EINVAL;
}

extern "C" int fvit_stem_conv3x3s2_px(int32_t dtype, const FvitMapView* in, const void* weight, const void* weight_lo, const float* bias, void* out,
                                      int32_t B, int32_t Hi, int32_t Wi, fvit_stream_t stream);

extern "C" int fvit_stem_conv3x3s2(int32_t dtype, const FvitMapView* in, const void* weight, const float* bias, void* out, int32_t B,
                                   int32_t Hi, int32_t Wi, fvit_stream_t stream) {
    return fvit_stem_conv3x3s2_px(dtype, in, weight, nullptr, bias, out, B, Hi, Wi, stream);
}

extern "C" int fvit_stem_conv3x3s2_px(int32_t dtype, const FvitMapView* in, const void* weight, const void* weight_lo, const float* bias, void* out,
                                      int32_t B, int32_t Hi, int32_t Wi, fvit_stream_t stream) {
    if (!in || !in->data || !weight || !bias || !out || B <= 0 || Hi <= 0 || Wi <= 0) {
        set_error("stem_conv: null or empty argument");
        return FVIT_EINVAL;
    }
    StemParams p;
    p.in = *in; p.w = weight; p.w_lo = weight_lo; p.bias = bias; p.out = out; p.B = B; p.Hi = Hi; p.Wi = Wi;
    p.Ho = (Hi - 1) / 2 + 1;
    p.Wo = (Wi - 1) / 2 + 1;
    const int64_t M = (int64_t)B * p.Ho * p.Wo;
    if (M > 0x7fffffff) {
        set_error("stem_conv: too many output pixels");
        return FVIT_EINVAL;
    }
    p.M = (int)M;
    const int nblk16 = (p.M + 15) / 16;
    int grid = (nblk16 + 3) / 4;
    if (grid > 256 * 32) grid = 256 * 32;
    const double bytes = (double)B * 3 * Hi * Wi * (in->dtype == FVIT_F32 ? 4 : 2) + 2.0 * M * 64;
    ProfScope prof(FVIT_K_CONV, 2.0 * M * 64 * 27, bytes, (hipStream_t)stream);
    if (dtype == FVIT_F16 && weight_lo) hipLaunchKernelGGL((stem_conv_kernel<_Float16, true>), dim3(grid), dim3(256), 0, (hipStream_t)stream, p);
    else if (dtype == FVIT_BF16 && weight_lo) hipLaunchKernelGGL((stem_conv_kernel<__bf16, true>), dim3(grid), dim3(256), 0, (hipStream_t)stream, p);
    else if (dtype == FVIT_F16) hipLaunchKernelGGL((stem_conv_kernel<_Float16>), dim3(grid), dim3(256), 0, (hipStream_t)stream, p);
    else if (dtype == FVIT_BF16) hipLaunchKernelGGL((stem_conv_kernel<__bf16>), dim3(grid), dim3(256), 0, (hipStream_t)stream, p);
// ... 149 lines not shown
```

fastervit_amd/csrc/fvit_rows.hip:

```cpp
#include "fvit_common.h"

namespace fvit {

namespace {

struct LnParams {
    const float* srcA;
    const float* srcB;
    const int32_t* src_idx;
    const int32_t* add_idx;
    const float* add;
    float* x_out;
    void* n_out;
    const float* ln_w;
    const float* ln_b;
    float eps;
    int rowsA, rowsB, ldn;
    int rows, rows_per_image, C;
    int lw;
    int lo_off;
};

template <typename T, int MAXV>
__global__ __launch_bounds__(256) void ln_kernel(LnParams p) {
// ... 267 lines not shown
        const int pix = tp * 64 + pl;
        if (pix < npix) {
            const int y = pix / wwid, xx = pix - y * wwid;
            const int64_t moff = b * p.map.stride_b + y * p.map.stride_h + xx * p.map.stride_w;
            for (int cl = cl0; cl < 32; cl += 4) {
                const int c = tc * 32 + cl;
                if (c < p.C) tile[cl][pl] = load_elem(p.map.data, moff + c * p.map.stride_c, p.map.dtype);
            }
        }
        __syncthreads();
        const int cl = tid & 31, pl0 = tid >> 5;
        const int c = tc * 32 + cl;
        for (int pp = pl0; pp < 64; pp += 8) {
            const int pix2 = tp * 64 + pp;
            if (pix2 < npix && c < p.C) {
                const int y = pix2 / wwid, xx = pix2 - y * wwid;
                p.x[token_row(p, b, y, xx) * p.C + c] = tile[cl][pp];
            }
        }
    } else {
        const int cl = tid & 31, pl0 = tid >> 5;
        const int c = tc * 32 + cl;
        for (int pp = pl0; pp < 64; pp += 8) {
            const int pix2 = tp * 64 + pp;
            if (pix2 < npix && c < p.C) {
                const int y = pix2 / wwid, xx = pix2 - y * wwid;
                const int64_t trow = token_row(p, b, y, xx);
                float v = p.x[trow * p.C + c];
                if (p.up_idx) {
                    const int tok = (int)((trow % p.rows_per_win) - p.row_off);
                    const int64_t crow = trow - (trow % p.rows_per_win) + p.up_idx[tok];
                    v += (p.gamma ? p.gamma[c] : 1.f) * p.x[crow * p.C + c];
                }
                tile[cl][pp] = v;
            }
        }
        __syncthreads();
        const int pl = tid & 63, cl0 = tid >> 6;
        const int pix = tp * 64 + pl;
        if (pix < npix) {
            const int y = pix / wwid, xx = pix - y * wwid;
            const int64_t moff = b * p.map.stride_b + y * p.map.stride_h + xx * p.map.stride_w;
            for (int cl2 = cl0; cl2 < 32; cl2 += 4) {
                const int c2 = tc * 32 + cl2;
                if (c2 < p.C) store_elem(p.map.data, moff + c2 * p.map.stride_c, p.map.dtype, tile[cl2][pl]);
            }
        }
    }
}

__global__ __launch_bounds__(256) void ct_rows_kernel(float* x, float* ct, int rows_per_win, int row_off, int ncw,
                                                      int64_t nrows, int C4, int to_x) {
    const int64_t i = (int64_t)blockIdx.x * blockDim.x + threadIdx.x;
    if (i >= nrows * C4) return;
    const int64_t r = i / C4;
    const int c4 = (int)(i - r * C4);
    const int64_t win = r / ncw;
    const int j = (int)(r - win * ncw);
    f4* px = (f4*)(x + (win * rows_per_win + row_off + j) * (int64_t)C4 * 4) + c4;
    f4* pc = (f4*)(ct + r * (int64_t)C4 * 4) + c4;
    if (to_x) *px = *pc; else *pc = *px;
}

__global__ __launch_bounds__(256) void propagate_kernel(float* x, const float* gamma, const int32_t* up_idx, int rows_per_win,
                                                        int ncw, int nloc, int64_t nwin, int C4) {
    const int64_t i = (int64_t)blockIdx.x * blockDim.x + threadIdx.x;
    if (i >= nwin * nloc * C4) return;
    const int c4 = (int)(i % C4);
    const int64_t r = i / C4;
    const int64_t win = r / nloc;
    const int t = (int)(r - win * nloc);
    f4* px = (f4*)(x + (win * rows_per_win + ncw + t) * (int64_t)C4 * 4) + c4;
    const f4 cv = *((const f4*)(x + (win * rows_per_win + up_idx[t]) * (int64_t)C4 * 4) + c4);
    const f4 gv = gamma ? *((const f4*)gamma + c4) : (f4){1.f, 1.f, 1.f, 1.f};
    *px = *px + gv * cv;
}

struct TokParams {
    FvitMapView in;
    const float* w;
    const float* bias;
    float* out;
    int B, C, Hp, Wp, kh, kw, sh, sw, Ho, Wo, cw;
};

template <typename IN, bool SMALL>
__global__ __launch_bounds__(256) void token_init_kernel(TokParams p) {
    const int64_t i = (int64_t)blockIdx.x * blockDim.x + threadIdx.x;
    const int G = p.Ho * p.Wo;
    if (i >= (int64_t)p.B * G * p.C) return;
    const int c = (int)(i % p.C);
    const int64_t t = i / p.C;
    const int tok = (int)(t % G), b = (int)(t / G);
    const int kk = tok % p.cw, r1 = tok / p.cw, ii = r1 % p.cw, r2 = r1 / p.cw, nbw = p.Wo / p.cw, bb = r2 % nbw, a = r2 / nbw;
    const int oy = a * p.cw + ii, ox = bb * p.cw + kk;
    float wv[9];
#pragma unroll
    for (int j = 0; j < 9; ++j) wv[j] = p.w[c * 9 + j];
    const IN* __restrict__ src = (const IN*)p.in.data + b * p.in.stride_b + c * p.in.stride_c;
    float acc = 0.f;
    const int y0 = oy * p.sh - 1, x0 = ox * p.sw - 1;
    if constexpr (SMALL) {
        float val[8][8];
#pragma unroll
        for (int dy = 0; dy < 8; ++dy) {
            const int y = min(max(y0 + dy, 0), p.Hp - 1);
#pragma unroll
            for (int dx = 0; dx < 8; ++dx) {
                const int x = min(max(x0 + dx, 0), p.Wp - 1);
                val[dy][dx] = (float)src[y * p.in.stride_h + x * p.in.stride_w];
            }
        }
#pragma unroll
        for (int dy = 0; dy < 8; ++dy) {
            const int y = y0 + dy;
            const bool yok = dy < p.kh + 2 && y >= 0 && y < p.Hp;
            const int ky_lo = max(0, dy - p.kh + 1), ky_hi = min(2, dy);
            const float m0 = (yok && ky_lo <= 0 && ky_hi >= 0) ? 1.f : 0.f, m1 = (yok && ky_lo <= 1 && ky_hi >= 1) ? 1.f : 0.f, m2 = (yok && ky_hi >= 2) ? 1.f : 0.f;
            const float cw0 = m0 * wv[0] + m1 * wv[3] + m2 * wv[6];
            const float cw1 = m0 * wv[1] + m1 * wv[4] + m2 * wv[7];
            const float cw2 = m0 * wv[2] + m1 * wv[5] + m2 * wv[8];
#pragma unroll
            for (int dx = 0; dx < 8; ++dx) {
                const int x = x0 + dx;
                const bool xok = dx < p.kw + 2 && x >= 0 && x < p.Wp;
                const int kx_lo = max(0, dx - p.kw + 1), kx_hi = min(2, dx);
                const float wsum = (kx_lo <= 0 && kx_hi >= 0 ? cw0 : 0.f) + (kx_lo <= 1 && kx_hi >= 1 ? cw1 : 0.f) + (kx_hi >= 2 ? cw2 : 0.f);
                acc += (xok ? wsum : 0.f) * val[dy][dx];
            }
        }
    } else {
        for (int dy = 0; dy < p.kh + 2; ++dy) {
            const int y = y0 + dy;
            if (y < 0 || y >= p.Hp) continue;
            const int ky_lo = max(0, dy - p.kh + 1), ky_hi = min(2, dy);
            const float m0 = (ky_lo <= 0 && ky_hi >= 0) ? 1.f : 0.f, m1 = (ky_lo <= 1 && ky_hi >= 1) ? 1.f : 0.f, m2 = ky_hi >= 2 ? 1.f : 0.f;
            const float cw0 = m0 * wv[0] + m1 * wv[3] + m2 * wv[6];
            const float cw1 = m0 * wv[1] + m1 * wv[4] + m2 * wv[7];
            const float cw2 = m0 * wv[2] + m1 * wv[5] + m2 * wv[8];
            const IN* rowp = src + y * p.in.stride_h;
            for (int dx = 0; dx < p.kw + 2; ++dx) {
                const int x = x0 + dx;
                if (x < 0 || x >= p.Wp) continue;
                const int kx_lo = max(0, dx - p.kw + 1), kx_hi = min(2, dx);
                const float wsum = (kx_lo <= 0 && kx_hi >= 0 ? cw0 : 0.f) + (kx_lo <= 1 && kx_hi >= 1 ? cw1 : 0.f) + (kx_hi >= 2 ? cw2 : 0.f);
                acc += wsum * (float)rowp[x * p.in.stride_w];
            }
        }
    }
    p.out[i] = acc / (float)(p.kh * p.kw) + p.bias[c];
}

int launch_map(const MapParams& p, bool reverse, hipStream_t stream) {
    const int hh = reverse ? p.H : p.Hp, wwid = reverse ? p.W : p.Wp;
    if (p.map.stride_c == 1) {
        const int64_t pix = (int64_t)p.batch * hh * wwid;
        const int grid = (int)((pix + 3) / 4);
        const int esz = p.map.dtype == FVIT_F32 ? 4 : 2;
        const bool vec = esz == 2 && p.C % 8 == 0 && ((uintptr_t)p.map.data % 16) == 0 && (p.map.stride_b * esz) % 16 == 0 && (p.map.stride_h * esz) % 16 == 0 &&
                         (p.map.stride_w * esz) % 16 == 0;
#define FVIT_MAP_CL(MT_, VEC_) do { if (reverse) hipLaunchKernelGGL((map_rows_cl_kernel<true, MT_, VEC_>), dim3(grid), dim3(256), 0, stream, p); \
                                    else hipLaunchKernelGGL((map_rows_cl_kernel<false, MT_, VEC_>), dim3(grid), dim3(256), 0, stream, p); } while (0)
        if (p.map.dtype == FVIT_F32) FVIT_MAP_CL(float, false);
        else if (p.map.dtype == FVIT_F16) { if (vec) FVIT_MAP_CL(_Float16, true); else FVIT_MAP_CL(_Float16, false); }
        else { if (vec) FVIT_MAP_CL(__bf16, true); else FVIT_MAP_CL(__bf16, false); }
#undef FVIT_MAP_CL
    } else {
        const int tiles_p = (hh * wwid + 63) / 64, tiles_c = (p.C + 31) / 32;
        const int grid = p.batch * tiles_p * tiles_c;
        if (reverse) hipLaunchKernelGGL((map_rows_tiled_kernel<true>), dim3(grid), dim3(256), 0, stream, p);
        else hipLaunchKernelGGL((map_rows_tiled_kernel<false>), dim3(grid), dim3(256), 0, stream, p);
    }
    return check_launch(reverse ? "window_reverse" : "window_partition");
}

int elem_size(int dtype) { return dtype == FVIT_F32 ? 4 : 2; }

}

int launch_gather_layernorm(const LnCall& c, hipStream_t stream) {
    if (c.rows <= 0 || (c.C % 4) || (c.ldn % 4) || c.ldn < c.C || c.lo_off < 0 || (c.lo_off % 4) || (c.lo_off > 0 && (c.lo_off < c.C || c.ldn < 2 * c.lo_off))) {
        set_error("layernorm: unsupported shape rows=%d C=%d ldn=%d", c.rows, c.C, c.ldn);
        return FVIT_EINVAL;
    }
    LnParams p;
    p.srcA = c.srcA; p.srcB = c.srcB; p.src_idx = c.src_idx; p.add_idx = c.add_idx; p.add = c.add;
    p.x_out = c.x_out; p.n_out = c.n_out; p.ln_w = c.ln_w; p.ln_b = c.ln_b; p.eps = c.eps;
    p.rowsA = c.rowsA; p.rowsB = c.rowsB; p.ldn = c.ldn; p.rows = c.rows;
    p.rows_per_image = c.rows_per_image > 0 ? c.rows_per_image : 1; p.C = c.C;
    p.lo_off = c.lo_off; p.lw = c.lo_off > 0 ? c.lo_off : c.ldn;
    const double bytes = (double)c.rows * c.C * (4.0 + (c.x_out ? 4.0 : 0.0) + 2.0);
    ProfScope prof(FVIT_K_LAYERNORM, 8.0 * c.rows * (double)c.C, bytes, stream);
    prof_note("ln_kernel", (c.rows + 3) / 4);
    if (c.dtype == FVIT_F16) return launch_ln_t<_Float16>(p, stream);
    if (c.dtype == FVIT_BF16) return launch_ln_t<__bf16>(p, stream);
    set_error("layernorm: operand dtype %d not supported", c.dtype);
    return FVIT_EINVAL;
}

int launch_partition(const PartitionCall& c, hipStream_t stream) {
    if (c.ws <= 0 || (c.Hp % c.ws) || (c.Wp % c.ws) || (c.C % 4)) {
        set_error("window_partition: map %dx%d is not a multiple of the window %d (or C %% 4 != 0)", c.Hp, c.Wp, c.ws);
        return FVIT_EINVAL;
    }
    MapParams p;
    p.map = c.in; p.x = c.x; p.ct = c.ct; p.gamma = nullptr; p.up_idx = nullptr;
    p.batch = c.batch; p.C = c.C; p.Hp = c.Hp; p.Wp = c.Wp; p.H = c.Hp; p.W = c.Wp; p.ws = c.ws;
    p.rows_per_win = c.rows_per_win; p.row_off = c.row_off; p.ncw = c.ncw;
    p.nwx = c.Wp / c.ws; p.nw = (c.Hp / c.ws) * p.nwx;
    const double bytes = (double)c.batch * c.C * c.Hp * c.Wp * (elem_size(c.in.dtype) + 4.0);
    int rc;
    {
        ProfScope prof(FVIT_K_PARTITION, 0.0, bytes, stream);
        rc = launch_map(p, false, stream);
    }
    if (rc) return rc;
    if (c.ct && c.ncw > 0)
        rc = launch_ct_copy(c.x, c.rows_per_win, 0, c.ncw, const_cast<float*>(c.ct), c.batch * p.nw, c.C, 1, stream);
    return rc;
}

int launch_reverse(const ReverseCall& c, hipStream_t stream) {
    if (c.ws <= 0 || (c.Hp % c.ws) || (c.Wp % c.ws) || c.H > c.Hp || c.W > c.Wp) {
        set_error("window_reverse: bad geometry Hp=%d Wp=%d H=%d W=%d ws=%d", c.Hp, c.Wp, c.H, c.W, c.ws);
        return FVIT_EINVAL;
    }
    MapParams p;
    p.map = c.out; p.x = const_cast<float*>(c.x); p.ct = nullptr; p.gamma = c.gamma; p.up_idx = c.up_idx;
    p.batch = c.batch; p.C = c.C; p.Hp = c.Hp; p.Wp = c.Wp; p.H = c.H; p.W = c.W; p.ws = c.ws;
    p.rows_per_win = c.rows_per_win; p.row_off = c.row_off; p.ncw = c.row_off;
    p.nwx = c.Wp / c.ws; p.nw = (c.Hp / c.ws) * p.nwx;
    const double bytes = (double)c.batch * c.C * c.H * c.W * (elem_size(c.out.dtype) + 4.0);
    ProfScope prof(FVIT_K_REVERSE, 0.0, bytes, stream);
    return launch_map(p, true, stream);
}

bool reverse_ln_supported(const ReverseCall& c) {
    const int esz = 2;
    return (c.out.dtype == FVIT_F16 || c.out.dtype == FVIT_BF16) && c.out.stride_c == 1 && c.C % 8 == 0 && c.C <= 512 && ((uintptr_t)c.out.data % 16) == 0 &&
           (c.out.stride_b * esz) % 16 == 0 && (c.out.stride_h * esz) % 16 == 0 && (c.out.stride_w * esz) % 16 == 0;
}

int launch_reverse_ln(const ReverseCall& c, const float* ln_w, const float* ln_b, float eps, hipStream_t stream) {
    if (c.ws <= 0 || (c.Hp % c.ws) || (c.Wp % c.ws) || c.H > c.Hp || c.W > c.Wp || !ln_w || !ln_b) {
        set_error("window_reverse_ln: bad geometry Hp=%d Wp=%d H=%d W=%d ws=%d", c.Hp, c.Wp, c.H, c.W, c.ws);
        return FVIT_EINVAL;
    }
    if (!reverse_ln_supported(c)) {
        set_error("window_reverse_ln: needs a 16-bit channel-contiguous, 16-byte aligned map with C %% 8 == 0 and C <= 512 (C=%d, dtype %d)", c.C, c.out.dtype);
        return FVIT_EINVAL;
    }
    MapParams p;
    p.map = c.out; p.x = const_cast<float*>(c.x); p.ct = nullptr; p.gamma = c.gamma; p.up_idx = c.up_idx;
    p.batch = c.batch; p.C = c.C; p.Hp = c.Hp; p.Wp = c.Wp; p.H = c.H; p.W = c.W; p.ws = c.ws;
    p.rows_per_win = c.rows_per_win; p.row_off = c.row_off; p.ncw = c.row_off;
    p.nwx = c.Wp / c.ws; p.nw = (c.Hp / c.ws) * p.nwx;
    const int64_t pix = (int64_t)c.batch * c.H * c.W;
    const int grid = (int)((pix + 3) / 4);
    ProfScope prof(FVIT_K_REVERSE, 8.0 * pix * c.C, (double)pix * c.C * (2.0 + 4.0), stream);
    prof_note("map_rows_ln_cl_kernel", grid);
    if (c.out.dtype == FVIT_F16) hipLaunchKernelGGL((map_rows_ln_cl_kernel<_Float16>), dim3(grid), dim3(256), 0, stream, p, ln_w, ln_b, eps);
    else hipLaunchKernelGGL((map_rows_ln_cl_kernel<__bf16>), dim3(grid), dim3(256), 0, stream, p, ln_w, ln_b, eps);
    return check_launch("window_reverse_ln");
}

int launch_rows_avgpool(const float* x, float* out, int batch, int rows, int C, int round_dtype, hipStream_t stream) {
    if (!x || !out || batch <= 0 || rows <= 0 || C <= 0 || (C % 4) || (round_dtype != FVIT_F16 && round_dtype != FVIT_BF16)) {
        set_error("rows_avgpool: unsupported arguments batch=%d rows=%d C=%d dtype=%d (C %% 4 == 0, a 16-bit map type)", batch, rows, C, round_dtype);
        return FVIT_EINVAL;
    }
    const dim3 grid((C + 255) / 256, batch);
    ProfScope prof(FVIT_K_OTHER, (double)batch * rows * C, 4.0 * batch * C * (rows + 1.0), stream);
    prof_note("rows_avgpool_kernel", (int)(grid.x * grid.y));
    if (round_dtype == FVIT_F16) hipLaunchKernelGGL((rows_avgpool_kernel<_Float16>), grid, dim3(256), 0, stream, x, out, rows, C);
    else hipLaunchKernelGGL((rows_avgpool_kernel<__bf16>), grid, dim3(256), 0, stream, x, out, rows, C);
    return check_launch("rows_avgpool_kernel");
}

int launch_ct_copy(float* x, int rows_per_win, int row_off, int ncw, float* ct, int nwin_total, int C, int to_x,
                   hipStream_t stream) {
    const int64_t nrows = (int64_t)nwin_total * ncw;
    const int C4 = C / 4;
    const int64_t n = nrows * C4;
    ProfScope prof(FVIT_K_OTHER, 0.0, 8.0 * nrows * C, stream);
    hipLaunchKernelGGL(ct_rows_kernel, dim3((unsigned)((n + 255) / 256)), dim3(256), 0, stream, x, ct, rows_per_win, row_off, ncw,
                       nrows, C4, to_x);
    return check_launch("ct_rows_kernel");
}

int launch_token_init(const FvitMapView& in, const float* w, const float* bias, float* out, int B, int C, int Hp, int Wp, int kh, int kw,
                      int sh, int sw, int cw, hipStream_t stream) {
    TokParams p;
    p.in = in; p.w = w; p.bias = bias; p.out = out; p.B = B; p.C = C; p.Hp = Hp; p.Wp = Wp;
    p.kh = kh; p.kw = kw; p.sh = sh; p.sw = sw; p.cw = cw;
    p.Ho = (Hp - kh) / sh + 1;
    p.Wo = (Wp - kw) / sw + 1;
    if (kh <= 0 || kw <= 0 || sh <= 0 || sw <= 0 || cw <= 0 || p.Ho <= 0 || p.Wo <= 0 || (p.Ho % cw) || (p.Wo % cw)) {
        set_error("token_init: bad pooling geometry k=%dx%d s=%dx%d on %dx%d (cw=%d)", kh, kw, sh, sw, Hp, Wp, cw);
        return FVIT_EINVAL;
    }
    const int64_t n = (int64_t)B * p.Ho * p.Wo * C;
    ProfScope prof(FVIT_K_OTHER, 0.0, (double)B * C * Hp * Wp * 2.0 + 4.0 * n, stream);
    const dim3 grid((unsigned)((n + 255) / 256));
    const bool small_patch = kh + 2 <= 8 && kw + 2 <= 8;
#define FVIT_TOK(IN_) do { if (small_patch) hipLaunchKernelGGL((token_init_kernel<IN_, true>), grid, dim3(256), 0, stream, p); \
                           else hipLaunchKernelGGL((token_init_kernel<IN_, false>), grid, dim3(256), 0, stream, p); } while (0)
    if (in.dtype == FVIT_F32) FVIT_TOK(float);
    else if (in.dtype == FVIT_F16) FVIT_TOK(_Float16);
    else if (in.dtype == FVIT_BF16) FVIT_TOK(__bf16);
    else { set_error("token_init: map dtype %d not supported", in.dtype); return FVIT_EINVAL; }
#undef FVIT_TOK
    return check_launch("token_init_kernel");
}

int launch_propagate(float* x, const float* gamma, const int32_t* up_idx, int rows_per_win, int ncw, int nloc, int nwin_total,
                     int C, hipStream_t stream) {
    const int C4 = C / 4;
    const int64_t n = (int64_t)nwin_total * nloc * C4;
    ProfScope prof(FVIT_K_OTHER, 0.0, 12.0 * nwin_total * nloc * (double)C, stream);
    hipLaunchKernelGGL(propagate_kernel, dim3((unsigned)((n + 255) / 256)), dim3(256), 0, stream, x, gamma, up_idx, rows_per_win, ncw,
                       nloc, (int64_t)nwin_total, C4);
    return check_launch("propagate_kernel");
}

}
```

fastervit_amd/hat_runtime.py:

```python
from __future__ import annotations

import collections
import contextlib
import ctypes as C
import threading
import warnings
from typing import Optional

import torch
import torch.nn.functional as F

from . import _lib
from ._lib import (FVIT_BF16, FVIT_F16, FVIT_F32, FVIT_MASK_BIAS, FVIT_TILE_K, FVIT_TILE_N, FvitAttnWeights,
                   FvitBlockWeights, FvitMapView, FvitMlpWeights, FvitStageDesc, FvitStageTables)

_DT = {torch.float32: FVIT_F32, torch.float16: FVIT_F16, torch.bfloat16: FVIT_BF16}
from ._lib import FVIT_MAX_DENSE_SEQ

_OP = {"f16": (FVIT_F16, torch.float16, 1), "bf16": (FVIT_BF16, torch.bfloat16, 1),
       "f16x2": (FVIT_F16, torch.float16, 2), "bf16x2": (FVIT_BF16, torch.bfloat16, 2),
       "f16x3": (FVIT_F16, torch.float16, 3), "bf16x3": (FVIT_BF16, torch.bfloat16, 3)}
OPERAND_MODES = tuple(_OP)


def _rup(x: int, m: int) -> int:
    return (x + m - 1) // m * m


def _require_gpu(t: torch.Tensor, what: str) -> None:
    if not t.is_cuda:
        raise RuntimeError(
            f"{what}: the FasterViT HAT path runs only on a HIP device (got a {t.device.type} tensor); "
            "there is no CPU or eager fallback. Move the model and input to the GPU.")


def _stream_ptr(device=None) -> int:
    return torch.cuda.current_stream(device).cuda_stream


def _check_device(x: torch.Tensor, layer, what: str) -> None:
    for p in layer.parameters():
        if p.device != x.device:
            raise RuntimeError(f"{what}: parameters are on {p.device} but the input is on {x.device}; move the model with "
                               f".to('{x.device}') (there is no implicit cross-device copy on the HIP path)")
        break


def _map_view(t: torch.Tensor) -> FvitMapView:
    if t.dtype not in _DT:
        raise RuntimeError(f"unsupported feature-map dtype {t.dtype}")
    sb, sc, sh, sw = t.stride()
    return FvitMapView(t.data_ptr(), sb, sc, sh, sw, _DT[t.dtype], 0)


def build_tables(sr0: int, sr1: int, ws: int, cw: int, hier: bool):
    nW, nloc = sr0 * sr1, ws * ws
    ncw = cw * cw if hier else 0
    S, G = nloc + ncw, ncw * nW
    ln1_src = torch.arange(nW * S, dtype=torch.int64).view(nW, S).clone()
    ln1_add = torch.full((nW, S), -1, dtype=torch.int64)
    ln1_add[:, ncw:] = torch.arange(nloc)
    ct_src = torch.zeros(max(G, 1), dtype=torch.int64)
    up_idx = torch.zeros(nloc, dtype=torch.int64)
    if hier:
        ar = torch.arange(G)
        dew = ar.view(sr0, sr1, cw, cw).permute(0, 2, 1, 3).reshape(G)
        win = ar.view(sr1, cw, sr0, cw).permute(0, 2, 1, 3).reshape(G)
        ct_src = (dew // ncw) * S + dew % ncw
        ln1_src[:, :ncw] = -(win.view(nW, ncw) + 1)
        near = (torch.arange(ws) * cw) // ws
        up_idx = (near[:, None] * cw + near[None, :]).reshape(nloc)
    i32 = torch.int32
    return dict(ln1_src=ln1_src.reshape(-1).to(i32), ln1_add=ln1_add.reshape(-1).to(i32), ct_src=ct_src.to(i32),
                up_idx=up_idx.to(i32), nW=nW, S=S, G=G, ncw=ncw)


def _f32(t) -> torch.Tensor:
    return t.detach().float().contiguous()


def _gamma(g) -> Optional[torch.Tensor]:
    return _f32(g) if isinstance(g, torch.Tensor) else None


class _Keep:

    def __init__(self, op_dtype=None, terms: int = 1):
        self.tensors = []
        self.op_dtype = op_dtype
        self.terms = terms
# ... 281 lines not shown
        _PACKS += 1
        if dyn:
            st.packs[tkey] = (sig, keep, arr)
            _lru_touch(st.packs, tkey, DYN_CACHE_SIZE)
    lib = _lib.lib()
    desc_common = dict(C=Cdim, heads=heads, dpad=dpad, ws=ws, Hp=Hp, Wp=Wp, cw=cw if hier else 0, hier=int(hier),
                       square=int(hier and hasattr(blk0, "hat_pos_embed")), hidden=blk0.mlp.fc1.out_features,
                       depth=len(layer.blocks), do_propagation=int(bool(blk0.do_propagation)), operand_dtype=op_code,
                       spad=lib.fvit_attention_spad(tb["S"]), gpad=lib.fvit_attention_spad(tb["G"]) if hier else 0,
                       qk_scale=float(blk0.attn.scale), weight_terms=terms)
    return st, tb, ctables, desc_common


_TLS = threading.local()


def set_workspace_slot(slot: int) -> None:
    _TLS.slot = int(slot)


def _slot() -> int:
    return getattr(_TLS, "slot", 0)


@contextlib.contextmanager
def workspace_slot(slot: int):
    prev = _slot()
    set_workspace_slot(slot)
    try:
        yield
    finally:
        set_workspace_slot(prev)


def _drop_workspace(w: _Workspace) -> None:
    if w.event is not None:
        w.event.synchronize()


def _workspace(st: StageState, desc_common: dict, B: int, H: int, W: int, device, bounded: bool = False) -> _Workspace:
    terms = desc_common["weight_terms"]
    key = (B, desc_common["Hp"], desc_common["Wp"], H, W, desc_common["operand_dtype"], _slot()) + (("x3",) if terms == 3 else ())
    hit = st.workspaces.get(key)
    if hit is not None and bounded:
        _lru_touch(st.workspaces, key, DYN_CACHE_SIZE, _drop_workspace)
    if hit is not None:
        d = hit.descs.get(terms)
        if d is None:
            d = hit.descs[terms] = FvitStageDesc(batch=B, H=H, W=W, **desc_common)
        hit.desc = d
        return hit
    desc = FvitStageDesc(batch=B, H=H, W=W, **desc_common)
    lib = _lib.lib()
    nbytes = lib.fvit_stage_workspace_bytes(C.byref(desc))
    if nbytes == 0:
        _lib.check(-1, "fvit_stage_workspace_bytes")
    ws_t = torch.zeros(nbytes, dtype=torch.uint8, device=device)
    ws = st.workspaces[key] = _Workspace(desc, ws_t)
    ws.descs[terms] = desc
    if bounded:
        _lru_touch(st.workspaces, key, DYN_CACHE_SIZE, _drop_workspace)
    return ws


def _acquire(ws: _Workspace, device) -> int:
    stream = torch.cuda.current_stream(device)
    ptr = stream.cuda_stream
    if not torch.cuda.is_current_stream_capturing():
        if ws.last_stream is not None and ws.last_stream != ptr and ws.event is not None:
            stream.wait_event(ws.event)
    return ptr


def _release(ws: _Workspace, device) -> None:
    if torch.cuda.is_current_stream_capturing():
        return
    stream = torch.cuda.current_stream(device)
    if ws.event is None:
        ws.event = torch.cuda.Event()
    ws.event.record(stream)
    ws.last_stream = stream.cuda_stream


def token_init(tok, xp: torch.Tensor) -> torch.Tensor:
    _require_gpu(xp, "TokenInitializer")
    with torch.no_grad(), torch.cuda.device(xp.device):
        w, b = _token_weights(tok, xp)
        pool = tok.to_global_feature.pool
        kh, kw = pool.kernel_size if isinstance(pool.kernel_size, (tuple, list)) else (pool.kernel_size,) * 2
        sh, sw = pool.stride if isinstance(pool.stride, (tuple, list)) else (pool.stride,) * 2
        B, Cc, Hp, Wp = xp.shape
        Ho, Wo = (Hp - kh) // sh + 1, (Wp - kw) // sw + 1
        ct = torch.empty((B, Ho * Wo, Cc), dtype=torch.float32, device=xp.device)
        view = _map_view(xp)
        rc = _lib.lib().fvit_token_init(C.byref(view), w.data_ptr(), b.data_ptr(), ct.data_ptr(), B, Cc, Hp, Wp, kh, kw, sh, sw,
                                        tok.window_size, _stream_ptr(xp.device))
        _lib.check(rc, "fvit_token_init")
        return ct


def _token_weights(tok, xp: torch.Tensor):
    key = "_fvit_tok"
    cache = tok.__dict__.get(key)
    if not isinstance(cache, dict):
        cache = tok.__dict__[key] = {}
    wt, bs = tok.pos_embed.weight, tok.pos_embed.bias
    if wt.device != xp.device:
        raise RuntimeError(f"TokenInitializer: parameters are on {wt.device} but the input is on {xp.device}")
    replica = bool(getattr(tok, "_is_replica", False))
    sig = (float(wt.detach().float().sum()), float(bs.detach().float().sum())) if replica else \
        (wt.data_ptr(), wt._version, bs.data_ptr(), bs._version)
    st = cache.get(str(xp.device))
    if st is None or st[0] != sig:
        w = wt.detach().float().reshape(-1, 9).contiguous()
        b = bs.detach().float().contiguous()
        st = cache[str(xp.device)] = (sig, w, b)
    return st[1], st[2]


def token_geometry(Hp: int, Wp: int, ws: int, cw: int):
    ks, ss, outs = [], [], []
    for r in (Hp, Wp):
        o = int(cw * r / ws)
        if o < 1:
            raise ValueError(f"TokenInitializer: a {r}-pixel side gives no carrier token (window {ws}, ct_size {cw})")
        s = int(r / o)
        k = r - (o - 1) * s
        ks.append(k)
        ss.append(s)
        outs.append((r - k) // s + 1)
    Hq, Wq = (_rup(o, cw) for o in outs)
    return ks[0], ks[1], ss[0], ss[1], outs[0], outs[1], Hq, Wq


def token_init_dyn(tok, xp: torch.Tensor, ws: int) -> torch.Tensor:
    _require_gpu(xp, "TokenInitializer")
    with torch.no_grad(), torch.cuda.device(xp.device):
        w, b = _token_weights(tok, xp)
        B, Cc, Hp, Wp = xp.shape
        cw = tok.window_size
        kh, kw, sh, sw, _, _, Hq, Wq = token_geometry(Hp, Wp, ws, cw)
        ct = torch.empty((B, Hq * Wq, Cc), dtype=torch.float32, device=xp.device)
        rc = _lib.lib().fvit_token_init_dyn(C.byref(_map_view(xp)), w.data_ptr(), b.data_ptr(), ct.data_ptr(), B, Cc, Hp, Wp, kh, kw, sh, sw,
                                            cw, _stream_ptr(xp.device))
        _lib.check(rc, "fvit_token_init_dyn")
        return ct


def _folded_bn(bn, device):
    if bn.running_mean is None or bn.running_var is None:
        raise NotImplementedError("feature_tap: the BatchNorm2d has no running statistics (track_running_stats=False)")
    ts = [t for t in (bn.weight, bn.bias, bn.running_mean, bn.running_var) if t is not None]
    if any(t.device != device for t in ts):
        raise RuntimeError(f"feature_tap: BatchNorm2d is on {ts[0].device} but the input is on {device}")
    sig = (str(device),) + tuple((t.data_ptr(), t._version) for t in ts)
    hit = bn.__dict__.get("_fvit_fold")
    if hit is None or hit[0] != sig:
        with torch.no_grad(), torch.autocast(device_type=device.type, enabled=False):
            scale = torch.rsqrt(bn.running_var.double() + bn.eps)
            if bn.weight is not None:
                scale = scale * bn.weight.double()
            shift = -bn.running_mean.double() * scale
            if bn.bias is not None:
                shift = shift + bn.bias.double()
        hit = (sig, scale.float().contiguous(), shift.float().contiguous())
        bn.__dict__["_fvit_fold"] = hit
    return hit[1], hit[2]


def feature_tap(x: torch.Tensor, bn, H: Optional[int] = None, W: Optional[int] = None) -> torch.Tensor:
    _require_gpu(x, "feature_tap")
    if x.dim() != 4:
        raise ValueError(f"feature_tap: expected a (B, C, H, W) map, got {tuple(x.shape)}")
    B, Cc, Hs, Ws = x.shape
    H = Hs if H is None else int(H)
    W = Ws if W is None else int(W)
    if not (0 < H <= Hs and 0 < W <= Ws) or bn.num_features != Cc:
        raise ValueError(f"feature_tap: crop {H}x{W} of a {tuple(x.shape)} map with a {bn.num_features}-channel BatchNorm2d")
    with torch.no_grad(), torch.cuda.device(x.device):
        scale, shift = _folded_bn(bn, x.device)
        out = torch.empty((B, Cc, H, W), dtype=torch.float32, device=x.device)
        rc = _lib.lib().fvit_feature_tap(C.byref(_map_view(x)), B, Cc, H, W, scale.data_ptr(), shift.data_ptr(), out.data_ptr(),
                                         _stream_ptr(x.device))
        _lib.check(rc, "fvit_feature_tap")
        return out


_WARNED = set()


def _check_mode(layer, x: torch.Tensor, what: str):
    if layer.training:
        raise RuntimeError(f"{what}: the fused HIP stage kernels are inference-only (eval semantics: no stochastic depth); call model.eval(), or run the "
                           "stage through the module (FasterViTLayer.forward in train mode uses fastervit_amd.hat_backward: unit-kernel forward with "
                           "DropPath + kernel-sequence backward).")
    if torch.is_grad_enabled():
        if x.requires_grad and x.is_leaf:
            raise RuntimeError(f"{what}: the input requires grad, but this entry point is forward-only: its output would be silently detached. Use "
                               "model.enable_hat_backward() / FasterViTLayer.forward (differentiable where fastervit_amd.hat_backward covers the "
                               "geometry), or run under torch.no_grad().")
        if what not in _WARNED:
            _WARNED.add(what)
            warnings.warn(f"{what}: called with grad enabled; this forward-only HIP entry point returns DETACHED outputs (gradients do not flow "
                          "through it). Wrap inference in torch.no_grad(), or use model.enable_hat_backward().", RuntimeWarning, stacklevel=3)


def check_user_input(x: torch.Tensor, what: str = "FasterViT") -> None:
    if torch.is_grad_enabled() and x.requires_grad:
        raise RuntimeError(f"{what}: the input requires grad, but this model has a transformer stage whose geometry fastervit_amd.hat_backward does not "
                           "cover (windows or carrier grids of more than 64 tokens): the gradient w.r.t. the input would silently be cut. Run under "
                           "torch.no_grad() (or detach the input).")


def is_prepared(layer, device, batch: Optional[int] = None, hw=None, slots=(0,)) -> bool:
    states = layer.__dict__.get("_fvit_state")
    if not states or getattr(layer, "_is_replica", False):
        return False
    st = states.get((device.type, device.index if device.index is not None else torch.cuda.current_device()))
    if st is None or st.sig is None:
        return False
    op_name = getattr(layer, "hat_operand_dtype", "f16")
    if st.sig[:-2] != _signature(layer.blocks, device, op_name):
        return False
    if batch is None or hw is None:
        return True
    H, W = hw
    ws = layer.window_size
    Hp, Wp = H + (ws - H % ws) % ws, W + (ws - W % ws) % ws
    if (Hp, Wp) not in st.tables:
        return False
    op_code, _, terms = _OP[op_name]
    return all(((batch, Hp, Wp, H, W, op_code, s) + (("x3",) if terms == 3 else ())) in st.workspaces for s in slots)


def stage_refs(layer, device, batch: int, H: int, W: int, slot: int = 0) -> tuple:
    st = _state(layer, device)
    ws = layer.window_size
    Hp, Wp = H + (ws - H % ws) % ws, W + (ws - W % ws) % ws
    op_code, _, terms = _OP[getattr(layer, "hat_operand_dtype", "f16")]
    dyn = bool(getattr(layer, "dynamic_grid", False)) and bool(layer.blocks[0].do_sr_hat)
    with st.lock:
        tables = st.tables.get((Hp, Wp))
        pack = st.packs.get((Hp, Wp)) if dyn else (st.sig, st.keep, st.blocks_c)
        wsp = st.workspaces.get((batch, Hp, Wp, H, W, op_code, int(slot)) + (("x3",) if terms == 3 else ()))
    if tables is None or pack is None or pack[1] is None or wsp is None:
        raise RuntimeError(f"stage_refs: no stage call of a {batch} x {H} x {W} map in workspace slot {slot} has run on {device}")
    tok = getattr(layer, "global_tokenizer", None)
    tokw = tok.__dict__.get("_fvit_tok", {}).get(str(device)) if tok is not None else None
    return tables, pack, wsp, tokw


def pool_tail_supported(layer, x: torch.Tensor) -> bool:
    return bool(len(layer.blocks)) and not layer.blocks[0].do_sr_hat and x.shape[2] == x.shape[3] == layer.window_size and x.dtype in (torch.float16, torch.bfloat16)


def ln2d_tail_supported(x: torch.Tensor, out: torch.Tensor) -> bool:
    C_ = x.shape[1]
    return (out.dtype in (torch.float16, torch.bfloat16) and C_ % 8 == 0 and C_ <= 512 and out.stride(1) == 1 and out.data_ptr() % 16 == 0
            and all(out.stride(d) % 8 == 0 for d in (0, 2, 3)))


def stage_forward(layer, x: torch.Tensor, tokenizer=None, out: Optional[torch.Tensor] = None, ln2d=None,
                  pool_out: Optional[torch.Tensor] = None) -> torch.Tensor:
    _require_gpu(x, "FasterViTLayer")
    _check_mode(layer, x, "FasterViTLayer")
    if len(layer.blocks) == 0:
        return x
    _check_device(x, layer, "FasterViTLayer")
    lib = _lib.lib()
    with torch.no_grad(), torch.cuda.device(x.device):
        B, Cc, H, W = x.shape
        ws = layer.window_size
        pad_r = (ws - W % ws) % ws
        pad_b = (ws - H % ws) % ws
        xp = F.pad(x, (0, pad_r, 0, pad_b)) if (pad_r or pad_b) else x
        Hp, Wp = H + pad_b, W + pad_r
        ct = None
        blk0 = layer.blocks[0]
        if layer.do_gt and blk0.do_sr_hat:
            ct = tokenizer(xp) if tokenizer is not None else token_init(layer.global_tokenizer, xp)
        st = _state(layer, x.device)
        with st.lock:
            st, tb, ctables, dc = _prepare(layer, x.device, Hp, Wp)
            wsp = _workspace(st, dc, B, H, W, x.device, bounded=bool(getattr(layer, "dynamic_grid", False)))
            tail = None
            if pool_out is not None:
                if ln2d is not None or not pool_tail_supported(layer, x) or tuple(pool_out.shape) != (B, Cc) or pool_out.dtype != torch.float32 \
                        or not pool_out.is_contiguous() or pool_out.device != x.device:
                    raise RuntimeError("stage_forward: pool_out needs a contiguous fp32 (B, C) tensor, a 16-bit map of one window per image without "
                                       "carrier tokens, and excludes ln2d")
                tail = _lib.FvitStageTail(None, None, pool_out.data_ptr(), 0.0, _DT[x.dtype])
            elif out is None:
                out = torch.empty_like(x)
            elif out.shape != x.shape or out.dtype != x.dtype or out.device != x.device:
                raise RuntimeError(f"stage_forward: out {tuple(out.shape)} {out.dtype} does not match x {tuple(x.shape)} {x.dtype}")
            if ln2d is not None:
                ln_w, ln_b, eps = ln2d
                if not ln2d_tail_supported(x, out) or any(t.dtype != torch.float32 or t.numel() < Cc or not t.is_contiguous() or t.device != x.device
                                                          for t in (ln_w, ln_b)):
                    raise RuntimeError("stage_forward: ln2d needs fp32 [C] parameters and a 16-bit channel-contiguous out with C % 8 == 0, C <= 512")
                tail = _lib.FvitStageTail(ln_w.data_ptr(), ln_b.data_ptr(), None, float(eps), 0)
            vin = _map_view(xp)
            vout = _map_view(out) if pool_out is None else None
            stream = _acquire(wsp, x.device)
            rc = lib.fvit_hat_stage_forward_tail(C.byref(wsp.desc), st.blocks_c, C.byref(ctables), C.byref(vin),
                                                 ct.data_ptr() if ct is not None else None, C.byref(vout) if vout is not None else None,
                                                 C.byref(tail) if tail is not None else None, wsp.buf.data_ptr(), wsp.buf.numel(), stream)
            _lib.check(rc, "fvit_hat_stage_forward")
            _release(wsp, x.device)
        return out if pool_out is None else pool_out


def block_forward(blk, x: torch.Tensor, carrier_tokens: Optional[torch.Tensor]):
    _require_gpu(x, "HAT")
    _check_mode(blk, x, "HAT")
    _check_device(x, blk, "HAT")
    lib = _lib.lib()
    with torch.no_grad(), torch.cuda.device(x.device):
        Bw, T, Cc = x.shape
        ws = blk.window_size
        hier = bool(blk.do_sr_hat)
        sr0, sr1 = (blk.sr_ratio if hier else (1, 1))
        nW = sr0 * sr1
        if Bw % nW:
            raise ValueError(f"HAT.forward: {Bw} windows is not a multiple of {nW} windows per image")
        B = Bw // nW
        holder = blk.__dict__.get("_fvit_holder")
        if holder is None or holder.blocks[0] is not blk:
            holder = _BlockHolder(blk)
            blk.__dict__["_fvit_holder"] = holder
        st = _state(holder, x.device)
        with st.lock:
            st, tb, ctables, dc = _prepare(holder, x.device, sr0 * ws, sr1 * ws)
            dc = dict(dc, depth=1)
            wsp = _workspace(st, dc, B, sr0 * ws, sr1 * ws, x.device)
            xf = x.float().contiguous().clone()
            ctf = None
            if hier:
                if carrier_tokens is None:
                    raise ValueError("hierarchical HAT block needs carrier tokens")
                ctf = carrier_tokens.float().contiguous().clone()
            stream = _acquire(wsp, x.device)
            rc = lib.fvit_hat_block_forward(C.byref(wsp.desc), st.blocks_c, C.byref(ctables), xf.data_ptr(),
                                            ctf.data_ptr() if ctf is not None else None, wsp.buf.data_ptr(), wsp.buf.numel(), stream)
            _lib.check(rc, "fvit_hat_block_forward")
            _release(wsp, x.device)
        if hier:
            return xf.to(x.dtype), ctf.to(carrier_tokens.dtype)
        return xf.to(x.dtype), carrier_tokens


class _BlockHolder:

    def __init__(self, blk):
        self.blocks = [blk]
        self.window_size = blk.window_size
        self.training = False

    @property
    def _is_replica(self):
        return bool(getattr(self.blocks[0], "_is_replica", False))

    def parameters(self):
        return self.blocks[0].parameters()

    @property
    def hat_operand_dtype(self):
        return getattr(self.blocks[0], "hat_operand_dtype", "f16")


def workspace_bytes(layer) -> int:
    states = layer.__dict__.get("_fvit_state") or {}
    return sum(w.buf.numel() for st in states.values() for w in st.workspaces.values())
```

include/fvit_hip.h:

```cpp
#ifndef FVIT_HIP_H
#define FVIT_HIP_H

#include <stddef.h>
#include <stdint.h>

#ifdef __cplusplus
extern "C" {
#endif

#define FVIT_ABI_VERSION 10

#define FVIT_OK 0
#define FVIT_EINVAL (-1)
#define FVIT_EWORKSPACE (-2)
#define FVIT_ELAUNCH (-3)

#define FVIT_F32 0
#define FVIT_F16 1
#define FVIT_BF16 2

#define FVIT_TILE_N 128
#define FVIT_TILE_K 64
#define FVIT_MASK_BIAS (-30000.0f)
#define FVIT_MAX_DENSE_SEQ 208
// ... 20 lines not shown
    float qk_scale;
    int32_t weight_terms;
} FvitStageDesc;

typedef struct FvitAttnWeights {
    const void* w_qkv;
    const float* b_qkv;
    const void* w_proj;
    const float* b_proj;
    const float* bias;
    const float* ln_w;
    const float* ln_b;
    const float* gamma;
    const void* w_qkv_frag;
    const float* b_qkv_heads;
    const void* w_proj_frag;
    const float* rel_table;
    int32_t rel_w;
    int32_t rel_ng;
} FvitAttnWeights;

typedef struct FvitMlpWeights {
    const void* w_fc1;
    const float* b_fc1;
    const void* w_fc2;
    const float* b_fc2;
    const float* ln_w;
    const float* ln_b;
    const float* gamma;
    const void* w_fc1_frag;
    const void* w_fc2_frag;
} FvitMlpWeights;

typedef struct FvitBlockWeights {
    FvitAttnWeights attn;
    FvitMlpWeights mlp;
    FvitAttnWeights hat_attn;
    FvitMlpWeights hat_mlp;
    const float* pe_x;
    const float* pe_ct;
    int32_t last;
    int32_t _pad;
} FvitBlockWeights;

typedef struct FvitStageTables {
    const int32_t* ln1_src;
    const int32_t* ln1_add;
    const int32_t* ct_src;
    const int32_t* up_idx;
} FvitStageTables;

typedef struct FvitMapView {
    void* data;
    int64_t stride_b, stride_c, stride_h, stride_w;
    int32_t dtype;
    int32_t _pad;
} FvitMapView;

int fvit_abi_version(void);
const char* fvit_last_error(void);

int fvit_attention_spad(int32_t S);
int fvit_attention_dense(int32_t S, int32_t dpad);

size_t fvit_stage_workspace_bytes(const FvitStageDesc* desc);
int fvit_workspace_init(const FvitStageDesc* desc, void* workspace, size_t bytes, fvit_stream_t stream);

int fvit_hat_stage_forward(const FvitStageDesc* desc, const FvitBlockWeights* blocks,
                           const FvitStageTables* tables, const FvitMapView* in,
                           const float* ct_init, const FvitMapView* out, void* workspace,
                           size_t workspace_bytes, fvit_stream_t stream);

typedef struct FvitStageTail {
    const float* ln_w;
    const float* ln_b;
    float* pool_out;
    float ln_eps;
    int32_t pool_dtype;
} FvitStageTail;
int fvit_hat_stage_forward_tail(const FvitStageDesc* desc, const FvitBlockWeights* blocks,
                                const FvitStageTables* tables, const FvitMapView* in,
                                const float* ct_init, const FvitMapView* out, const FvitStageTail* tail,
                                void* workspace, size_t workspace_bytes, fvit_stream_t stream);
int fvit_rows_avgpool(int32_t round_dtype, const float* x, float* out, int32_t B, int32_t rows, int32_t C, fvit_stream_t stream);

int fvit_hat_block_forward(const FvitStageDesc* desc, const FvitBlockWeights* block,
                           const FvitStageTables* tables, float* x, float* ct, void* workspace,
                           size_t workspace_bytes, fvit_stream_t stream);

int fvit_token_init(const FvitMapView* in, const float* weight, const float* bias, float* ct_out, int32_t batch, int32_t C,
                    int32_t Hp, int32_t Wp, int32_t pool_kh, int32_t pool_kw, int32_t pool_sh, int32_t pool_sw, int32_t cw,
                    fvit_stream_t stream);

int fvit_token_init_dyn(const FvitMapView* in, const float* weight, const float* bias, float* ct_out, int32_t batch, int32_t C,
                        int32_t Hp, int32_t Wp, int32_t pool_kh, int32_t pool_kw, int32_t pool_sh, int32_t pool_sw, int32_t cw,
                        fvit_stream_t stream);

int fvit_feature_tap(const FvitMapView* in, int32_t batch, int32_t C, int32_t H, int32_t W, const float* scale, const float* shift,
                     float* out, fvit_stream_t stream);

int fvit_token_init_dyn_backward(const FvitMapView* in, const float* weight, const float* dct, float* dx, float* dweight, float* dbias,
                                 float* partials, int32_t batch, int32_t C, int32_t Hp, int32_t Wp, int32_t pool_kh, int32_t pool_kw,
                                 int32_t pool_sh, int32_t pool_sw, int32_t cw, fvit_stream_t stream);

int fvit_feature_tap_backward(const float* dout, const FvitMapView* x, const FvitMapView* dx, int32_t batch, int32_t C, int32_t H, int32_t W,
                              int32_t Hs, int32_t Ws, const float* scale, float* partials, int64_t partial_floats, float* sums,
                              fvit_stream_t stream);

int fvit_window_partition(const FvitMapView* in, int32_t batch, int32_t C, int32_t Hp, int32_t Wp,
                          int32_t ws, float* windows, fvit_stream_t stream);
int fvit_window_reverse(const float* windows, int32_t batch, int32_t C, int32_t Hp, int32_t Wp,
                        int32_t H, int32_t W, int32_t ws, const FvitMapView* out, fvit_stream_t stream);


int fvit_gemm_bias_act(int32_t operand_dtype, const void* A, int32_t lda, const void* Wt, int32_t ldw,
                       const float* bias, void* out, int32_t ldo, int32_t M, int32_t N, int32_t K,
                       int32_t act, fvit_stream_t stream);
int fvit_gemm_residual(int32_t operand_dtype, const void* A, int32_t lda, const void* Wt, int32_t ldw,
                       const float* bias, const float* gamma, float* x, int32_t ldx, int32_t M,
                       int32_t N, int32_t K, fvit_stream_t stream);

int fvit_gemm_residual_splitk(int32_t operand_dtype, const void* A, int32_t lda, const void* Wt, int32_t ldw, const float* bias, const float* gamma,
                              float* x, int32_t ldx, int32_t M, int32_t N, int32_t K, float* slab, size_t slab_bytes, fvit_stream_t stream);

int fvit_gemm_terms(int32_t operand_dtype, const void* A, int32_t lda, const void* Wt, int32_t ldw, const float* bias, const float* gamma,
                    void* out, int32_t ldo, int32_t M, int32_t N, int32_t K, int32_t ka, int32_t epilogue, fvit_stream_t stream);
int fvit_gemm_terms_lo(int32_t operand_dtype, const void* A, int32_t lda, const void* Wt, int32_t ldw, const float* bias, const float* gamma,
                       void* out, int32_t ldo, int32_t out_lo_off, int32_t M, int32_t N, int32_t K, int32_t ka, int32_t epilogue,
                       fvit_stream_t stream);
int fvit_window_attention_terms(int32_t operand_dtype, const void* qkv, int32_t ldq, int32_t q_lo_off, void* out, int32_t ldo,
                                int32_t o_lo_off, const float* bias, int32_t nwin, int32_t S, int32_t heads, int32_t dpad, float scale,
                                fvit_stream_t stream);
int fvit_window_attention_long_terms(int32_t operand_dtype, const void* qkv, int32_t ldq, int32_t q_lo_off, void* out, int32_t ldo, int32_t o_lo_off,
                                     const float* rel_table, int32_t rel_w, int32_t rel_ng, int32_t nwin, int32_t S, int32_t heads, int32_t dpad, float scale,
                                     fvit_stream_t stream);
int fvit_gather_layernorm_terms(int32_t operand_dtype, const float* srcA, int32_t rowsA, const float* srcB, int32_t rowsB,
                                const int32_t* src_idx, const int32_t* add_idx, const float* add, float* x_out, void* n_out, int32_t ldn,
                                int32_t lo_off, const float* ln_w, const float* ln_b, float eps, int32_t rows, int32_t rows_per_image,
                                int32_t C, fvit_stream_t stream);
int fvit_window_attention(int32_t operand_dtype, const void* qkv, int32_t ldq, void* out, int32_t ldo,
                          const float* bias, int32_t nwin, int32_t S, int32_t heads, int32_t dpad,
                          float scale, fvit_stream_t stream);
int fvit_window_attention_drop(int32_t operand_dtype, const void* qkv, int32_t ldq, void* out, int32_t ldo, const float* bias, int32_t nwin, int32_t S,
                               int32_t heads, int32_t dpad, float scale, const void* drop_mask, fvit_stream_t stream);
int fvit_window_attention_long(int32_t operand_dtype, const void* qkv, int32_t ldq, void* out, int32_t ldo,
                               const float* rel_table, int32_t rel_w, int32_t rel_ng, int32_t nwin, int32_t S,
                               int32_t heads, int32_t dpad, float scale, fvit_stream_t stream);
int fvit_gather_layernorm(int32_t operand_dtype, const float* srcA, int32_t rowsA, const float* srcB,
                          int32_t rowsB, const int32_t* src_idx, const int32_t* add_idx,
                          const float* add, float* x_out, void* n_out, int32_t ldn, const float* ln_w,
                          const float* ln_b, float eps, int32_t rows, int32_t rows_per_image, int32_t C,
                          fvit_stream_t stream);

int fvit_ln_gemm_supported(int32_t C, int32_t N, int32_t ldw, int32_t ldo);
int fvit_ln_gemm(int32_t operand_dtype, const float* srcA, int32_t rowsA, const float* srcB, int32_t rowsB, const int32_t* src_idx,
                 const int32_t* add_idx, const float* add, float* x_out, const float* ln_w, const float* ln_b, float eps, int32_t rows,
                 int32_t rows_per_image, int32_t C, const void* Wt, int32_t ldw, const float* bias, void* out, int32_t ldo, int32_t N,
                 int32_t act, fvit_stream_t stream);

int fvit_win_mlp_supported(int32_t C, int32_t hidden);
int fvit_win_mlp_fused(int32_t operand_dtype, float* x, int32_t M, int32_t C, int32_t hidden, const float* ln_w, const float* ln_b,
                       float eps, const void* w_fc1_frag, const float* b_fc1, const void* w_fc2_frag, const float* b_fc2,
                       const float* gamma, fvit_stream_t stream);
int fvit_win_mlp_fused_terms(int32_t operand_dtype, float* x, int32_t M, int32_t C, int32_t hidden, const float* ln_w, const float* ln_b,
                             float eps, const void* w_fc1_frag, const float* b_fc1, const void* w_fc2_frag, const float* b_fc2,
                             const float* gamma, int32_t terms, fvit_stream_t stream);
size_t fvit_win_mlp_split_bytes(int32_t M, int32_t C, int32_t nsplit);
int fvit_win_mlp_fused_split(int32_t operand_dtype, float* x, int32_t M, int32_t C, int32_t hidden, const float* ln_w, const float* ln_b,
                             float eps, const void* w_fc1_frag, const float* b_fc1, const void* w_fc2_frag, const float* b_fc2,
                             const float* gamma, int32_t terms, float* slab, int32_t* counters, int32_t nsplit, fvit_stream_t stream);

int fvit_win_block_supported(int32_t C, int32_t heads, int32_t S);
int fvit_win_block_fused(int32_t operand_dtype, const float* srcA, int32_t rowsA, const float* srcB, int32_t rowsB,
                         const int32_t* src_idx, const int32_t* add_idx, const float* add, const float* ln_w,
                         const float* ln_b, float eps, int32_t rows_per_image, const void* w_qkv_frag,
                         const float* b_qkv_heads, const void* w_proj_frag, const float* b_proj, const float* gamma,
                         const float* bias, float* x_out, int32_t nwin, int32_t S, int32_t heads, int32_t C, float scale,
                         fvit_stream_t stream);
int fvit_win_block_fused_split(int32_t operand_dtype, const float* srcA, int32_t rowsA, const float* srcB, int32_t rowsB, const int32_t* src_idx,
                               const int32_t* add_idx, const float* add, const float* ln_w, const float* ln_b, float eps,
                               int32_t rows_per_image, const void* w_qkv_frag, const float* b_qkv_heads, const void* w_proj_frag,
                               const float* b_proj, const float* gamma, const float* bias, float* x_out, int32_t nwin, int32_t S,
                               int32_t heads, int32_t C, float scale, float* slab, int32_t* counters, int32_t nsplit, fvit_stream_t stream);

int fvit_win_block_fused_terms(int32_t operand_dtype, const float* srcA, int32_t rowsA, const float* srcB, int32_t rowsB, const int32_t* src_idx,
                               const int32_t* add_idx, const float* add, const float* ln_w, const float* ln_b, float eps,
                               int32_t rows_per_image, const void* w_qkv_frag, const float* b_qkv_heads, const void* w_proj_frag,
                               const float* b_proj, const float* gamma, const float* bias, float* x_out, int32_t nwin, int32_t S,
                               int32_t heads, int32_t C, float scale, int32_t terms, fvit_stream_t stream);
int fvit_attn_block_fused_terms(int32_t operand_dtype, const float* srcA, int32_t rowsA, const float* srcB, int32_t rowsB, const int32_t* src_idx,
                                const int32_t* add_idx, const float* add, const float* ln_w, const float* ln_b, float eps,
                                int32_t rows_per_image, const void* w_qkv_frag, const float* b_qkv_heads, const void* w_proj_frag,
                                const float* b_proj, const float* gamma, const float* bias, float* x_out, int32_t nwin, int32_t S,
                                int32_t heads, int32_t C, float scale, int32_t terms, fvit_stream_t stream);

int fvit_ct_block_supported(int32_t C, int32_t heads, int32_t G, int32_t hidden);
int fvit_ct_block_fused(int32_t operand_dtype, const float* X, int32_t rowsA, const int32_t* src_idx, const float* add, float* R,
                        int32_t batch, int32_t G, int32_t heads, int32_t C, int32_t hidden, const float* ln1_w, const float* ln1_b,
                        const void* w_qkv_frag, const float* b_qkv_heads, const void* w_proj_frag, const float* b_proj, const float* gamma1,
                        const float* bias, float scale, const float* ln2_w, const float* ln2_b, const void* w_fc1_frag, const float* b_fc1,
                        const void* w_fc2_frag, const float* b_fc2, const float* gamma2, float eps, fvit_stream_t stream);

int fvit_ct_block_fused_terms(int32_t operand_dtype, const float* X, int32_t rowsA, const int32_t* src_idx, const float* add, float* R,
                              int32_t batch, int32_t G, int32_t heads, int32_t C, int32_t hidden, const float* ln1_w, const float* ln1_b,
                              const void* w_qkv_frag, const float* b_qkv_heads, const void* w_proj_frag, const float* b_proj, const float* gamma1,
                              const float* bias, float scale, const float* ln2_w, const float* ln2_b, const void* w_fc1_frag, const float* b_fc1,
                              const void* w_fc2_frag, const float* b_fc2, const float* gamma2, float eps, int32_t terms, fvit_stream_t stream);

int fvit_attn_block_supported(int32_t C, int32_t heads, int32_t S);
int fvit_attn_block_fused(int32_t operand_dtype, const float* srcA, int32_t rowsA, const float* srcB, int32_t rowsB,
                          const int32_t* src_idx, const int32_t* add_idx, const float* add, const float* ln_w,
                          const float* ln_b, float eps, int32_t rows_per_image, const void* w_qkv_frag,
                          const float* b_qkv_heads, const void* w_proj_frag, const float* b_proj, const float* gamma,
                          const float* bias, float* x_out, int32_t nwin, int32_t S, int32_t heads, int32_t C, float scale,
                          fvit_stream_t stream);

int fvit_mlp_fused_supported(int32_t C, int32_t hidden);
int fvit_mlp_fused(int32_t operand_dtype, float* x, int32_t M, int32_t C, int32_t hidden, const float* ln_w,
                   const float* ln_b, float eps, const void* w_fc1_frag, const float* b_fc1, const void* w_fc2_frag,
                   const float* b_fc2, const float* gamma, fvit_stream_t stream);

int fvit_bias_act_cl(int32_t dtype, void* x, const float* bias, int64_t n_pixels, int32_t C, int32_t act,
                     fvit_stream_t stream);
int fvit_bias_residual_cl(int32_t dtype, void* x, const void* y, const float* bias, int64_t n_pixels, int32_t C,
                          fvit_stream_t stream);
int fvit_layernorm2d_cl(int32_t dtype, const void* in, void* out, const float* weight, const float* bias, float eps,
                        int64_t n_pixels, int32_t C, int32_t C_valid, fvit_stream_t stream);
int fvit_map_pad_cl(int32_t dtype, const void* in, void* out, int32_t B, int32_t H, int32_t W, int32_t Hp, int32_t Wp, int32_t C,
                    fvit_stream_t stream);
int fvit_layernorm2d_crop_cl(int32_t dtype, const void* in, void* out, const float* weight, const float* bias, float eps, int32_t B, int32_t H,
                             int32_t W, int32_t Hp, int32_t Wp, int32_t C, int32_t C_valid, fvit_stream_t stream);

int fvit_global_avgpool_cl(int32_t dtype, const void* in, float* out, int32_t B, int32_t HW, int32_t C, fvit_stream_t stream);

int fvit_conv3x3_nhwc(int32_t dtype, const void* in, const void* weight, const float* bias, const void* residual,
                      void* out, int32_t B, int32_t Hi, int32_t Wi, int32_t Cin, int32_t Cout, int32_t stride,
                      int32_t act, const void* zeros, fvit_stream_t stream);
int fvit_conv3x3_nhwc_terms(int32_t dtype, const void* in, const void* weight, const float* bias, const void* residual,
                            void* out, int32_t B, int32_t Hi, int32_t Wi, int32_t Cin, int32_t Cout, int32_t stride,
                            int32_t act, int32_t weight_terms, const void* zeros, fvit_stream_t stream);

int fvit_conv3x3_nhwc_px(int32_t dtype, const void* in, const void* in_lo, const void* weight, const float* bias, const void* residual,
                         const void* residual_lo, void* out, void* out_lo, float* out_f32, int32_t B, int32_t Hi, int32_t Wi, int32_t Cin,
                         int32_t Cout, int32_t stride, int32_t act, int32_t weight_terms, const void* zeros, fvit_stream_t stream);
int fvit_conv3x3_dense_k(int32_t cin_valid);
int fvit_conv3x3_patch_form(int32_t B, int32_t Hi, int32_t Wi, int32_t Cin, int32_t Cout, int32_t stride);
int fvit_conv3x3_nhwc_dense(int32_t dtype, const void* in, const void* weight, const float* bias, const void* residual,
                            void* out, int32_t B, int32_t Hi, int32_t Wi, int32_t Cin, int32_t cin_valid, int32_t Cout, int32_t stride,
                            int32_t act, int32_t weight_terms, const void* zeros, fvit_stream_t stream);
int fvit_conv3x3_nhwc_px_dense(int32_t dtype, const void* in, const void* in_lo, const void* weight, const float* bias, const void* residual,
                               const void* residual_lo, void* out, void* out_lo, float* out_f32, int32_t B, int32_t Hi, int32_t Wi, int32_t Cin,
                               int32_t cin_valid, int32_t Cout, int32_t stride, int32_t act, int32_t weight_terms, const void* zeros,
                               fvit_stream_t stream);
int fvit_layernorm2d_px(int32_t dtype, const void* in, const void* in_lo, const float* in_f32, void* out, void* out_lo, const float* weight,
                        const float* bias, float eps, int64_t n_pixels, int32_t C, int32_t C_valid, fvit_stream_t stream);
int fvit_stem_conv3x3s2_px(int32_t dtype, const FvitMapView* in, const void* weight, const void* weight_lo, const float* bias, void* out,
                           int32_t B, int32_t Hi, int32_t Wi, fvit_stream_t stream);

int fvit_conv3x3_c128_band_supported(int32_t H, int32_t W);
int fvit_conv3x3_c128_band(int32_t dtype, const void* in, const void* w_frag, const float* bias, const void* residual, void* out,
                           int32_t B, int32_t H, int32_t W, int32_t act, const void* zeros, fvit_stream_t stream);

int fvit_conv3x3_c64_ln2d(int32_t dtype, const void* in, const void* weight, const float* bias, const void* residual, void* out,
                          const float* ln_w, const float* ln_b, float eps, int32_t B, int32_t H, int32_t W, const void* zeros,
                          fvit_stream_t stream);
int fvit_conv3x3_c128_band_ln2d(int32_t dtype, const void* in, const void* w_frag, const float* bias, const void* residual, void* out,
                                const float* ln_w, const float* ln_b, float eps, int32_t B, int32_t H, int32_t W, const void* zeros,
                                fvit_stream_t stream);

int fvit_stem_conv3x3s2(int32_t dtype, const FvitMapView* in, const void* weight, const float* bias, void* out,
                        int32_t B, int32_t Hi, int32_t Wi, fvit_stream_t stream);

int fvit_stem_fused(int32_t dtype, const FvitMapView* in, const void* w1, const float* b1, const void* w2, const float* b2,
                    void* out, int32_t B, int32_t Hi, int32_t Wi, fvit_stream_t stream);

int32_t fvit_bwd_blocks(int32_t M);
int fvit_bwd_transpose16(int32_t operand_dtype, const void* in, int32_t ld_in, void* out, int32_t ld_out, int32_t M, int32_t N, fvit_stream_t stream);
int fvit_bwd_scale_cols(int32_t operand_dtype, const float* dy, const void* z, int32_t ldz, const float* gamma, void* dz, int32_t lddz, float* part,
                        int32_t M, int32_t C, fvit_stream_t stream);
int fvit_bwd_gelu(int32_t operand_dtype, const void* a, int32_t lda, const void* dh, int32_t lddh, void* out, int32_t ldo, float* part, int32_t M,
                  int32_t H, fvit_stream_t stream);
int fvit_bwd_layernorm(const float* x, const float* dxn, const float* dy, const float* ln_w, float eps, float* dx, float* stats, float* part,
                       int32_t M, int32_t C, fvit_stream_t stream);
int fvit_bwd_colsum16(int32_t operand_dtype, const void* in, int32_t ld, float* part, int32_t M, int32_t N, fvit_stream_t stream);
int fvit_bwd_window_attention(int32_t operand_dtype, const void* qkv, int32_t ld, const void* dO, int32_t ldo, const float* bias, int32_t spad,
                              float scale, void* dqkv, float* dbias_part, int32_t nwin, int32_t S, int32_t heads, int32_t D, fvit_stream_t stream);
int fvit_bwd_window_attention_drop(int32_t operand_dtype, const void* qkv, int32_t ld, const void* dO, int32_t ldo, const float* bias, int32_t spad,
                                   float scale, void* dqkv, float* dbias_part, int32_t nwin, int32_t S, int32_t heads, int32_t D, const void* drop_mask,
                                   fvit_stream_t stream);
size_t fvit_bwd_window_attention_long_workspace(int32_t nwin, int32_t S, int32_t heads, int32_t D, int32_t rel_w);
int fvit_bwd_window_attention_long(int32_t operand_dtype, const void* qkv, int32_t ld, const void* dO, int32_t ldo, const float* bias, int32_t spad,
                                   const float* rel_table, int32_t rel_w, int32_t rel_ng, float scale, void* dqkv, float* dbias, void* workspace,
                                   size_t workspace_bytes, int32_t nwin, int32_t S, int32_t heads, int32_t D, fvit_stream_t stream);
int fvit_bwd_colsum_finish(const float* part, int32_t blocks, int32_t stride, float* out, int32_t n, int32_t accumulate, fvit_stream_t stream);

int fvit_head_logits(const float* feat, const float* W, const float* bias, float* logits, int32_t B, int32_t N, int32_t F,
                     fvit_stream_t stream);
int fvit_head_softmax_xent(float* logits_inout, const int64_t* target, float* loss_rows, float* row_stats, int32_t B, int32_t N,
                           float smoothing, float inv_global_batch, fvit_stream_t stream);
int fvit_head_grad(const float* dlogits, const float* feat, const float* loss_rows, float* grad_flat, int32_t B, int32_t N, int32_t F,
                   float inv_global_batch, fvit_stream_t stream);
int fvit_sgd_momentum(float* param, float* momentum, const float* grad, int64_t n, float lr, float mu, float weight_decay,
                      fvit_stream_t stream);

int fvit_tune(const char* key, int32_t value);

#ifdef FVIT_DIAG
int fvit_debug_lds_poison(void* sink, int32_t blocks, int32_t spin, fvit_stream_t stream);
int fvit_debug_regs_poison(void* sink, int32_t blocks, int32_t spin, uint32_t pattern, fvit_stream_t stream);
int fvit_debug_poison_launches(void* sink, uint32_t pattern);

#define FVIT_DEBUG_MAX_RECORDS 512
typedef struct { char tag[24]; int64_t offset; int64_t rows; } FvitDebugRowhashRecord;
int fvit_debug_rowhash_begin(void* buf, int64_t capacity_words);
int fvit_debug_rowhash_end(FvitDebugRowhashRecord* out, int32_t max_records);
int fvit_debug_rowhash_dump(int32_t record, void* dst, int64_t capacity_bytes);
int fvit_debug_ct_block_timeline(const float* X, int32_t rowsA, const int32_t* src_idx, const float* add, float* R,
                                 int32_t batch, int32_t G, int32_t heads, int32_t C, int32_t hidden, const float* ln1_w, const float* ln1_b,
                                 const void* w_qkv_frag, const float* b_qkv_heads, const void* w_proj_frag, const float* b_proj, const float* gamma1,
                                 const float* bias, float scale, const float* ln2_w, const float* ln2_b, const void* w_fc1_frag, const float* b_fc1,
                                 const void* w_fc2_frag, const float* b_fc2, const float* gamma2, float eps, void* stamps, fvit_stream_t stream);
int fvit_debug_attn_block_timeline(const float* srcA, int32_t rowsA, const float* srcB, int32_t rowsB, const int32_t* src_idx,
                                   const int32_t* add_idx, const float* add, const float* ln_w, const float* ln_b, float eps,
// ... 53 lines not shown
```

Before: 91470 images/s.

## Write downsample conv output directly into next stage's window-partitioned token rows

Adds a ROWS epilogue to the 3x3 stride-2 downsample conv. It writes each output pixel as fp32 straight into the next HAT stage's windowed workspace rows, and a new stage entry point skips the partition kernel. Token init gets a pitched variant that writes carrier tokens into the same row buffer. This removes one partition launch and a map round trip per stage transition, in exchange for scattered fp32 stores in the conv epilogue and tighter coupling between the conv and the stage workspace.

Measured after the change: 92130 images/s (median of 6 runs). Within noise of the previous version (+0.7%).

```diff
diff --git a/fastervit_amd/_lib.py b/fastervit_amd/_lib.py
--- a/fastervit_amd/_lib.py
+++ b/fastervit_amd/_lib.py
@@ -34,6 +34,7 @@
     "fvit_bwd_window_attention_long_workspace", "fvit_tune", "fvit_prof_enable", "fvit_prof_collect",
     "fvit_prof_records", "fvit_prof_kind_name",
     "fvit_hat_stage_forward_tail", "fvit_rows_avgpool", "fvit_conv3x3_c64_ln2d", "fvit_conv3x3_c128_band_ln2d",
+    "fvit_stage_rows_layout", "fvit_hat_stage_forward_rows", "fvit_token_init_rows", "fvit_conv3x3_nhwc_rows",
 )
 DIAG_SYMBOLS = (
     "fvit_debug_lds_poison", "fvit_debug_regs_poison", "fvit_debug_poison_launches", "fvit_debug_rowhash_begin", "fvit_debug_rowhash_end",
@@ -122,6 +123,15 @@
     lib.fvit_hat_stage_forward_tail.argtypes = [C.POINTER(FvitStageDesc), C.POINTER(FvitBlockWeights),
                                                 C.POINTER(FvitStageTables), C.POINTER(FvitMapView), vp,
                                                 C.POINTER(FvitMapView), C.POINTER(FvitStageTail), vp, C.c_size_t, vp]
+    lib.fvit_stage_rows_layout.restype = C.c_int
+    lib.fvit_stage_rows_layout.argtypes = [C.POINTER(FvitStageDesc), C.POINTER(C.c_size_t), C.POINTER(i32), C.POINTER(i32)]
+    lib.fvit_hat_stage_forward_rows.restype = C.c_int
+    lib.fvit_hat_stage_forward_rows.argtypes = [C.POINTER(FvitStageDesc), C.POINTER(FvitBlockWeights), C.POINTER(FvitStageTables),
+                                                C.POINTER(FvitMapView), C.POINTER(FvitStageTail), vp, C.c_size_t, vp]
+    lib.fvit_token_init_rows.restype = C.c_int
+    lib.fvit_token_init_rows.argtypes = [C.POINTER(FvitMapView), vp, vp, vp, i32, i32, i32, i32, i32, i32, i32, i32, i32, i32, i32, vp]
+    lib.fvit_conv3x3_nhwc_rows.restype = C.c_int
+    lib.fvit_conv3x3_nhwc_rows.argtypes = [i32, vp, vp, vp, vp, vp, i32, i32, i32, i32, i32, i32, i32, i32, i32, vp, vp]
     lib.fvit_rows_avgpool.restype = C.c_int
     lib.fvit_rows_avgpool.argtypes = [i32, vp, vp, i32, i32, i32, vp]
     for fn in (lib.fvit_conv3x3_c64_ln2d, lib.fvit_conv3x3_c128_band_ln2d):
diff --git a/fastervit_amd/conv_runtime.py b/fastervit_amd/conv_runtime.py
--- a/fastervit_amd/conv_runtime.py
+++ b/fastervit_amd/conv_runtime.py
@@ -87,6 +87,7 @@
         self.fuse_conv_ln2d = {64: os.environ.get("FVIT_FUSE_CONV64_LN2D", "1") != "0", 128: os.environ.get("FVIT_FUSE_CONV128_LN2D", "1") != "0"}
         self.fuse_reverse_ln2d = os.environ.get("FVIT_FUSE_REVERSE_LN2D", "1") != "0"
         self.fuse_pool = os.environ.get("FVIT_FUSE_POOL", "1") != "0"
+        self.fuse_down_rows = os.environ.get("FVIT_FUSE_DOWN_ROWS", "1") != "0"
 
     def _signature(self):
         m = self.model
@@ -164,6 +165,32 @@
         if C_ == 128 and w.wband is not None and lib.fvit_conv3x3_c128_band_supported(x.shape[2], x.shape[3]):
             return "band"
         return None
+
+    def _down_rows_route(self, x, d: "DownW", nxt):
+        w = d.conv
+        if nxt is None or not self.fuse_down_rows or self.precise or not self.use_hip_conv or w.wk is None or w.terms != 1 or w.wk_classic is not None \
+                or w.cv != x.shape[1] or not x.is_contiguous(memory_format=torch.channels_last):
+            return None
+        B, _, Hi, Wi = x.shape
+        Co = w.wk.shape[0]
+        shape = (B, Co, (Hi - 1) // 2 + 1, (Wi - 1) // 2 + 1)
+        if Co % 128 or Hi % 2 or Wi % 2 or not nxt.transformer_block or not hat_runtime.stage_rows_supported(nxt, shape, self.dtype):
+            return None
+        return "classic"
+
+    def _conv_rows(self, x, w: ConvWeight, nxt):
+        B, Ci, Hi, Wi = x.shape
+        Co = w.wk.shape[0]
+        shape = (B, Co, (Hi - 1) // 2 + 1, (Wi - 1) // 2 + 1)
+        rows = hat_runtime.stage_rows(nxt, shape, self.dtype, x.device)
+        out = None
+        if nxt.do_gt and nxt.blocks[0].do_sr_hat:
+            out = torch.empty(shape, dtype=self.dtype, device=x.device, memory_format=torch.channels_last)
+        rc = _lib.lib().fvit_conv3x3_nhwc_rows(self.code, x.data_ptr(), w.wk.data_ptr(), None, out.data_ptr() if out is not None else None, rows.ptr,
+                                               B, Hi, Wi, Ci, Co, 2, rows.window_size, rows.rows_per_win, rows.row_off, self._zero_page(x.device),
+                                               _stream(self.dev))
+        _lib.check(rc, "fvit_conv3x3_nhwc_rows")
+        return (out if out is not None else rows.spec), rows
 
     def _conv_ln2d(self, route, x, w: ConvWeight, bias, residual, d: "DownW"):
         B, _, Hi, Wi = x.shape
@@ -412,6 +439,7 @@
         with torch.autocast(device_type="cuda", enabled=False):
             if lv_from == 0:
                 x = self._stem(x)
+            rows = None
             for li, (lvl, e) in enumerate(zip(levels, self.t["levels"])):
                 if li < lv_from or (lv_to is not None and li >= lv_to):
                     continue
@@ -419,11 +447,13 @@
                 if "blocks" in e:
                     x, normed = self._conv_level(x, e["blocks"], e.get("down"))
                 elif self._pool_tail(lvl, x, last=li + 1 == len(levels) and lv_to is None and "down" not in e):
-                    x, pooled = self._hat_level_pooled(lvl, x), True
+                    x, pooled = self._hat_level_pooled(lvl, x, rows), True
                 else:
-                    x, normed = self._hat_level(lvl, x, padded_out="down" in e, down=e.get("down"))
+                    x, normed = self._hat_level(lvl, x, padded_out="down" in e, down=e.get("down"), rows=rows)
+                rows = None
                 if "down" in e:
-                    x = self._downsample(x, e["down"], f32_out=li + 1 < len(levels) and levels[li + 1].transformer_block, normed=normed)
+                    nxt = levels[li + 1] if li + 1 < len(levels) and (lv_to is None or li + 1 < lv_to) else None
+                    x, rows = self._downsample(x, e["down"], f32_out=li + 1 < len(levels) and levels[li + 1].transformer_block, normed=normed, nxt=nxt)
             if lv_to is not None:
                 return x
             return self._head_logits(x, *self.t["head"][:2]) if pooled else self._head(x)
@@ -484,15 +514,20 @@
         return (hi, lo, None), False
 
     def _pool_tail(self, lvl, x, last):
-        return (last and self.fuse_pool and not self.precise and self.t["head"].ln is None and torch.is_tensor(x) and len(lvl.blocks) > 0
+        return (last and self.fuse_pool and not self.precise and self.t["head"].ln is None and (torch.is_tensor(x) or isinstance(x, hat_runtime.MapSpec)) and len(lvl.blocks) > 0
                 and x.shape[1] == lvl.blocks[0].attn.qkv.in_features and x.shape[1] % 16 == 0 and self.t["head"].w.shape[1] == x.shape[1]
                 and hat_runtime.pool_tail_supported(lvl, x))
 
-    def _hat_level_pooled(self, lvl, x):
+    def _hat_level_pooled(self, lvl, x, rows=None):
         feat = torch.empty((x.shape[0], x.shape[1]), dtype=torch.float32, device=x.device)
-        return hat_runtime.stage_forward(lvl, x, pool_out=feat)
-
-    def _hat_level(self, lvl, x, padded_out, tokenizer=None, down: Optional["DownW"] = None):
+        return hat_runtime.stage_forward(lvl, x, pool_out=feat, rows=rows)
+
+    def _hat_level(self, lvl, x, padded_out, tokenizer=None, down: Optional["DownW"] = None, rows=None):
+        if rows is not None:
+            xo = torch.empty(tuple(x.shape), dtype=self.dtype, device=x.device, memory_format=torch.channels_last)
+            if down is not None and self.fuse_reverse_ln2d and down.cin == x.shape[1] and hat_runtime.ln2d_tail_supported(x, xo):
+                return hat_runtime.stage_forward(lvl, x, out=xo, ln2d=(down.ln_w, down.ln_b, down.eps), rows=rows), True
+            return hat_runtime.stage_forward(lvl, x, out=xo, rows=rows), False
         if self.precise:
             hi, lo, x = x
             if x is None:
@@ -512,9 +547,15 @@
         xo = hat_runtime.stage_forward(lvl, xin, tokenizer=tokenizer, out=xo)
         return ((None, None, xo) if self.precise else xo), False
 
-    def _downsample(self, x, d: DownW, f32_out, normed=False):
+    def _downsample(self, x, d: DownW, f32_out, normed=False, nxt=None):
         if not self.precise:
-            return self._conv(x if normed else self._ln2d(x, d.ln_w, d.ln_b, d.eps, d.cin), d.conv, None, 2, 0)
+            xn = x if normed else self._ln2d(x, d.ln_w, d.ln_b, d.eps, d.cin)
+            if self._down_rows_route(xn, d, nxt) is not None:
+                return self._conv_rows(xn, d.conv, nxt)
+            return self._conv(xn, d.conv, None, 2, 0), None
+        return self._downsample_px(x, d, f32_out), None
+
+    def _downsample_px(self, x, d: DownW, f32_out):
         hi, lo, f32 = x
         if f32 is not None and not f32.is_contiguous(memory_format=torch.channels_last):
             f32 = f32.contiguous(memory_format=torch.channels_last)
diff --git a/fastervit_amd/csrc/fvit_api.hip b/fastervit_amd/csrc/fvit_api.hip
--- a/fastervit_amd/csrc/fvit_api.hip
+++ b/fastervit_amd/csrc/fvit_api.hip
@@ -529,12 +529,42 @@
     return launch_rows_avgpool(x, out, B, rows, C, round_dtype, (hipStream_t)stream);
 }
 
+int fvit_stage_rows_layout(const FvitStageDesc* desc, size_t* x_offset, int32_t* rows_per_win, int32_t* row_off) {
+    StageLayout L;
+    if (!desc || !x_offset || !rows_per_win || !row_off) { set_error("null argument"); return FVIT_EINVAL; }
+    if (!make_layout(*desc, L)) return FVIT_EINVAL;
+    *x_offset = L.off_X;
+    *rows_per_win = L.S;
+    *row_off = L.ncw;
+    return FVIT_OK;
+}
+
+static int stage_forward_impl(const FvitStageDesc* desc, const FvitBlockWeights* blocks, const FvitStageTables* tables, const FvitMapView* in,
+                              const float* ct_init, const FvitMapView* out, const FvitStageTail* tail, void* workspace, size_t workspace_bytes,
+                              fvit_stream_t stream, bool rows_filled);
+
 int fvit_hat_stage_forward_tail(const FvitStageDesc* desc, const FvitBlockWeights* blocks, const FvitStageTables* tables,
                                 const FvitMapView* in, const float* ct_init, const FvitMapView* out, const FvitStageTail* tail,
                                 void* workspace, size_t workspace_bytes, fvit_stream_t stream) {
+    return stage_forward_impl(desc, blocks, tables, in, ct_init, out, tail, workspace, workspace_bytes, stream, false);
+}
+
+int fvit_hat_stage_forward_rows(const FvitStageDesc* desc, const FvitBlockWeights* blocks, const FvitStageTables* tables, const FvitMapView* out,
+                                const FvitStageTail* tail, void* workspace, size_t workspace_bytes, fvit_stream_t stream) {
+    if (desc && (desc->H != desc->Hp || desc->W != desc->Wp)) {
+        set_error("stage_forward_rows: a window-padded map (%dx%d of %dx%d) has pad rows only the partition writes", desc->H, desc->W, desc->Hp, desc->Wp);
+        return FVIT_EINVAL;
+    }
+    return stage_forward_impl(desc, blocks, tables, nullptr, nullptr, out, tail, workspace, workspace_bytes, stream, true);
+}
+
+static int stage_forward_impl(const FvitStageDesc* desc, const FvitBlockWeights* blocks, const FvitStageTables* tables, const FvitMapView* in,
+                              const float* ct_init, const FvitMapView* out, const FvitStageTail* tail, void* workspace, size_t workspace_bytes,
+                              fvit_stream_t stream, bool rows_filled) {
     StageLayout L;
     const bool pooled = tail && tail->pool_out;
-    FVIT_TRY(check_hat_call(desc, blocks && in && (out || pooled), tables, workspace, workspace_bytes, ct_init, "hierarchical stage needs ct_init", L));
+    FVIT_TRY(check_hat_call(desc, blocks && (in || rows_filled) && (out || pooled), tables, workspace, workspace_bytes,
+                            rows_filled ? workspace : (const void*)ct_init, "hierarchical stage needs ct_init", L));
     const FvitStageDesc& d = *desc;
     if (tail && (!tail->ln_w != !tail->ln_b || (pooled && tail->ln_w))) {
         set_error("stage tail: LayerNorm2d needs both ln_w and ln_b, and excludes pool_out");
@@ -548,8 +578,10 @@
     hipStream_t st = (hipStream_t)stream;
     char* ws = (char*)workspace;
     float* X = (float*)(ws + L.off_X);
-    PartitionCall pc = {*in, d.batch, d.C, d.Hp, d.Wp, d.ws, X, L.S, L.ncw, d.hier ? ct_init : nullptr, L.ncw};
-    FVIT_TRY(launch_partition(pc, st));
+    if (!rows_filled) {
+        PartitionCall pc = {*in, d.batch, d.C, d.Hp, d.Wp, d.ws, X, L.S, L.ncw, d.hier ? ct_init : nullptr, L.ncw};
+        FVIT_TRY(launch_partition(pc, st));
+    }
     dbg_rowhash("partition", X, L.Mx, d.C * 4, st);
     const RouteKnobs knobs{};
     std::vector<BlockRoute> routes;
@@ -594,6 +626,13 @@
                     int32_t Wp, int32_t pool_kh, int32_t pool_kw, int32_t pool_sh, int32_t pool_sw, int32_t cw, fvit_stream_t stream) {
     if (!in || !weight || !bias || !ct_out) { set_error("null argument"); return FVIT_EINVAL; }
     return launch_token_init(*in, weight, bias, ct_out, batch, C, Hp, Wp, pool_kh, pool_kw, pool_sh, pool_sw, cw, (hipStream_t)stream);
+}
+
+int fvit_token_init_rows(const FvitMapView* in, const float* weight, const float* bias, float* rows, int32_t batch, int32_t C, int32_t Hp,
+                         int32_t Wp, int32_t pool_kh, int32_t pool_kw, int32_t pool_sh, int32_t pool_sw, int32_t cw, int32_t row_pitch,
+                         int32_t row_off, fvit_stream_t stream) {
+    if (!in || !weight || !bias || !rows || row_pitch <= 0) { set_error("token_init_rows: null argument or no row pitch"); return FVIT_EINVAL; }
+    return launch_token_init(*in, weight, bias, rows, batch, C, Hp, Wp, pool_kh, pool_kw, pool_sh, pool_sw, cw, (hipStream_t)stream, row_pitch, row_off);
 }
 
 int fvit_window_partition(const FvitMapView* in, int32_t batch, int32_t C, int32_t Hp, int32_t Wp, int32_t ws, float* windows,
diff --git a/fastervit_amd/csrc/fvit_common.h b/fastervit_amd/csrc/fvit_common.h
--- a/fastervit_amd/csrc/fvit_common.h
+++ b/fastervit_amd/csrc/fvit_common.h
@@ -432,7 +432,7 @@
 int launch_ct_copy(float* x, int rows_per_win, int row_off, int ncw, float* ct, int nwin_total, int C, int to_x,
                    hipStream_t stream);
 int launch_token_init(const FvitMapView& in, const float* w, const float* bias, float* out, int B, int C, int Hp, int Wp, int kh, int kw,
-                      int sh, int sw, int cw, hipStream_t stream);
+                      int sh, int sw, int cw, hipStream_t stream, int out_pitch = 0, int out_off = 0);
 int launch_propagate(float* x, const float* gamma, const int32_t* up_idx, int rows_per_win, int ncw, int nloc,
                      int nwin_total, int C, hipStream_t stream);
 
diff --git a/fastervit_amd/csrc/fvit_conv.hip b/fastervit_amd/csrc/fvit_conv.hip
--- a/fastervit_amd/csrc/fvit_conv.hip
+++ b/fastervit_amd/csrc/fvit_conv.hip
@@ -24,6 +24,8 @@
     int px;
     int cv, kd;
     float inv_cv;
+    float* rows_x = nullptr;
+    int rows_ws = 0, rows_per_win = 0, rows_off = 0;
 };
 
 __device__ __forceinline__ int swz_x(int r) { return (r >> 1) & 7; }
@@ -52,9 +54,10 @@
 constexpr int PHALO_PIECES = (PHALO_ROWS + 7) / 8;
 constexpr int PHALO_BYTES = PHALO_PIECES * 1024;
 
-template <typename T, int WM, int WN, int NI, bool PX = false, bool DENSE = false, bool HALO = false>
+template <typename T, int WM, int WN, int NI, bool PX = false, bool DENSE = false, bool HALO = false, bool ROWS = false>
 __global__ __launch_bounds__(256, 2) void conv3x3_kernel(ConvParams p) {
     typedef typename Op16<T>::v8 v8;
+    static_assert(!ROWS || !PX, "token-row epilogue: single-plane maps");
     static_assert(!HALO || (WM == 2 && WN == 2 && !DENSE), "halo form: 8 x 16 patches on the 2 x 2 wave grid, classic weight layout");
     constexpr int BM = 64 * WM, BN = 16 * NI * WN;
     constexpr int X_BYTES = HALO ? PHALO_BYTES : BM * BK * 2, W_BYTES = BN * BK * 2;
@@ -370,6 +373,29 @@
         if (p.act == 0) px_epilogue(IntTag<0>{});
         else if (p.act == 1) px_epilogue(IntTag<1>{});
         else px_epilogue(IntTag<2>{});
+        return;
+    }
+    if constexpr (ROWS) {
+        const int hw = p.Ho * p.Wo, nwx = p.Wo / p.rows_ws, nw = (p.Ho / p.rows_ws) * nwx;
+#pragma unroll
+        for (int mi = 0; mi < 4; ++mi) {
+            const int m = rowm(mi);
+            if (m < p.M) {
+                vout ov;
+#pragma unroll
+                for (int ni = 0; ni < NI; ++ni)
+#pragma unroll
+                    for (int r = 0; r < 4; ++r) ov[ni * 4 + r] = (T)(acc[ni][mi][r] + bias[ni * 4 + r]);
+                if (O) *(vout*)(O + (size_t)m * p.Cout + nb) = ov;
+                const int bb = m / hw, rem = m - bb * hw;
+                const int y = rem / p.Wo, x = rem - y * p.Wo;
+                const int wy = y / p.rows_ws, wx = x / p.rows_ws;
+                const int64_t row = ((int64_t)bb * nw + wy * nwx + wx) * p.rows_per_win + p.rows_off + (y - wy * p.rows_ws) * p.rows_ws + (x - wx * p.rows_ws);
+                float* xr = p.rows_x + row * p.Cout + nb;
+#pragma unroll
+                for (int j = 0; j < NC; j += 4) *(f4*)(xr + j) = (f4){(float)ov[j], (float)ov[j + 1], (float)ov[j + 2], (float)ov[j + 3]};
+            }
+        }
         return;
     }
     dispatch_epilogue(p.act, R != nullptr, [&](auto act_tag, auto res_tag) {
@@ -1410,6 +1436,13 @@
     ProfScope prof(FVIT_K_CONV, flops, bytes, stream);
     const int variant = tune_get("conv64_variant", 0);
     const int narrow = tune_get("conv128_narrow", 0);
+    if (p.rows_x) {
+        p.tiles_m = (p.M + 127) / 128;
+        p.tiles_n = p.Cout / 128;
+        prof_note("conv3x3_kernel<2,2,4,rows>", p.tiles_m * p.tiles_n);
+        hipLaunchKernelGGL((conv3x3_kernel<T, 2, 2, 4, false, false, false, true>), dim3(p.tiles_m * p.tiles_n), dim3(256), 0, stream, p);
+        return check_launch("conv3x3_kernel<rows>");
+    }
     const bool patch = patch_form_ok(p) && (p.Cout % 128 == 0 || (p.Cout > 128 && tune_get("conv_n128_ragged", 1))) && !narrow;
     if (patch) {
         p.tiles_m = p.B * ((p.Ho + PATCH_H - 1) / PATCH_H) * ((p.Wo + PATCH_W - 1) / PATCH_W);
@@ -1534,6 +1567,38 @@
     if (dtype == FVIT_F16) return launch_t<_Float16>(p, (hipStream_t)stream);
     if (dtype == FVIT_BF16) return launch_t<__bf16>(p, (hipStream_t)stream);
     set_error("conv3x3: dtype %d not supported (16-bit maps only)", dtype);
+    return FVIT_EINVAL;
+}
+
+extern "C" int fvit_conv3x3_nhwc_rows(int32_t dtype, const void* in, const void* weight, const float* bias, void* out, float* rows, int32_t B, int32_t Hi,
+                                      int32_t Wi, int32_t Cin, int32_t Cout, int32_t stride, int32_t ws, int32_t rows_per_win, int32_t row_off,
+                                      const void* zeros, fvit_stream_t stream) {
+    if (!in || !weight || !rows || !zeros || B <= 0 || Hi <= 0 || Wi <= 0 || Cin <= 0 || Cout <= 0 || (Cin % 64) || (Cout % 128) ||
+        (stride != 1 && stride != 2) || ws <= 0 || row_off < 0 || rows_per_win < row_off + ws * ws) {
+        set_error("conv3x3_rows: unsupported arguments Cin=%d Cout=%d stride=%d ws=%d rows_per_win=%d row_off=%d (need Cin %% 64 == 0, Cout %% 128 == 0, "
+                  "stride 1|2, rows_per_win >= row_off + ws * ws)", Cin, Cout, stride, ws, rows_per_win, row_off);
+        return FVIT_EINVAL;
+    }
+    ConvParams p;
+    p.in = in; p.w = weight; p.bias = bias; p.res = nullptr; p.out = out; p.zeros = zeros;
+    p.B = B; p.Hi = Hi; p.Wi = Wi; p.Cin = Cin; p.Cout = Cout; p.stride = stride; p.act = 0;
+    p.ablate = 0;
+    p.wterms = 1;
+    p.in_lo = p.res_lo = nullptr; p.out_lo = nullptr; p.out_f32 = nullptr; p.px = 0;
+    set_dense(p, Cin);
+    p.Ho = (Hi + 2 - 3) / stride + 1;
+    p.Wo = (Wi + 2 - 3) / stride + 1;
+    const int64_t M = (int64_t)B * p.Ho * p.Wo;
+    if ((p.Ho % ws) || (p.Wo % ws) || M > 0x7fffffff) {
+        set_error("conv3x3_rows: the %dx%d output map is not a multiple of the window %d (or %lld pixels exceed the 32-bit row index)", p.Ho, p.Wo, ws,
+                  (long long)M);
+        return FVIT_EINVAL;
+    }
+    p.M = (int)M;
+    p.rows_x = rows; p.rows_ws = ws; p.rows_per_win = rows_per_win; p.rows_off = row_off;
+    if (dtype == FVIT_F16) return launch_t<_Float16>(p, (hipStream_t)stream);
+    if (dtype == FVIT_BF16) return launch_t<__bf16>(p, (hipStream_t)stream);
+    set_error("conv3x3_rows: dtype %d not supported (16-bit maps only)", dtype);
     return FVIT_EINVAL;
 }
 
diff --git a/fastervit_amd/csrc/fvit_rows.hip b/fastervit_amd/csrc/fvit_rows.hip
--- a/fastervit_amd/csrc/fvit_rows.hip
+++ b/fastervit_amd/csrc/fvit_rows.hip
@@ -373,6 +373,7 @@
     const float* bias;
     float* out;
     int B, C, Hp, Wp, kh, kw, sh, sw, Ho, Wo, cw;
+    int out_pitch, out_off;
 };
 
 template <typename IN, bool SMALL>
@@ -439,7 +440,13 @@
             }
         }
     }
-    p.out[i] = acc / (float)(p.kh * p.kw) + p.bias[c];
+    int64_t orow = t;
+    if (p.out_pitch > 0) {
+        const int ncw = p.cw * p.cw;
+        const int64_t win = t / ncw;
+        orow = win * p.out_pitch + p.out_off + (t - win * ncw);
+    }
+    p.out[orow * p.C + c] = acc / (float)(p.kh * p.kw) + p.bias[c];
 }
 
 int launch_map(const MapParams& p, bool reverse, hipStream_t stream) {
@@ -580,8 +587,13 @@
 }
 
 int launch_token_init(const FvitMapView& in, const float* w, const float* bias, float* out, int B, int C, int Hp, int Wp, int kh, int kw,
-                      int sh, int sw, int cw, hipStream_t stream) {
+                      int sh, int sw, int cw, hipStream_t stream, int out_pitch, int out_off) {
+    if (out_pitch < 0 || out_off < 0 || (out_pitch > 0 && out_pitch < out_off + cw * cw)) {
+        set_error("token_init: bad row placement pitch=%d offset=%d for %d carrier rows per window", out_pitch, out_off, cw * cw);
+        return FVIT_EINVAL;
+    }
     TokParams p;
+    p.out_pitch = out_pitch; p.out_off = out_off;
     p.in = in; p.w = w; p.bias = bias; p.out = out; p.B = B; p.C = C; p.Hp = Hp; p.Wp = Wp;
     p.kh = kh; p.kw = kw; p.sh = sh; p.sw = sw; p.cw = cw;
     p.Ho = (Hp - kh) / sh + 1;
diff --git a/fastervit_amd/hat_runtime.py b/fastervit_amd/hat_runtime.py
--- a/fastervit_amd/hat_runtime.py
+++ b/fastervit_amd/hat_runtime.py
@@ -5,7 +5,7 @@
 import ctypes as C
 import threading
 import warnings
-from typing import Optional
+from typing import NamedTuple, Optional
 
 import torch
 import torch.nn.functional as F
@@ -453,7 +453,7 @@
     ws.last_stream = stream.cuda_stream
 
 
-def token_init(tok, xp: torch.Tensor) -> torch.Tensor:
+def token_init(tok, xp: torch.Tensor, rows: Optional["StageRows"] = None) -> Optional[torch.Tensor]:
     _require_gpu(xp, "TokenInitializer")
     with torch.no_grad(), torch.cuda.device(xp.device):
         w, b = _token_weights(tok, xp)
@@ -462,8 +462,17 @@
         sh, sw = pool.stride if isinstance(pool.stride, (tuple, list)) else (pool.stride,) * 2
         B, Cc, Hp, Wp = xp.shape
         Ho, Wo = (Hp - kh) // sh + 1, (Wp - kw) // sw + 1
+        view = _map_view(xp)
+        if rows is not None:
+            ws_ = rows.window_size
+            if tuple(xp.shape) != rows.shape or rows.row_off != tok.window_size ** 2 or Ho * Wo != (Hp // ws_) * (Wp // ws_) * rows.row_off:
+                raise RuntimeError(f"token_init: a {Ho}x{Wo} carrier grid of {tuple(xp.shape)} does not fill the {rows.row_off} carrier rows per window of "
+                                   f"the stage's window tensor ({rows.shape})")
+            rc = _lib.lib().fvit_token_init_rows(C.byref(view), w.data_ptr(), b.data_ptr(), rows.ptr, B, Cc, Hp, Wp, kh, kw, sh, sw,
+                                                 tok.window_size, rows.rows_per_win, 0, _stream_ptr(xp.device))
+            _lib.check(rc, "fvit_token_init_rows")
+            return None
         ct = torch.empty((B, Ho * Wo, Cc), dtype=torch.float32, device=xp.device)
-        view = _map_view(xp)
         rc = _lib.lib().fvit_token_init(C.byref(view), w.data_ptr(), b.data_ptr(), ct.data_ptr(), B, Cc, Hp, Wp, kh, kw, sh, sw,
                                         tok.window_size, _stream_ptr(xp.device))
         _lib.check(rc, "fvit_token_init")
@@ -621,6 +630,49 @@
     return tables, pack, wsp, tokw
 
 
+class MapSpec(NamedTuple):
+    shape: tuple
+    dtype: torch.dtype
+    device: torch.device
+
+
+class StageRows(NamedTuple):
+    ptr: int
+    rows_per_win: int
+    row_off: int
+    window_size: int
+    shape: tuple
+    dtype: torch.dtype
+    device: torch.device
+    wsp: object
+
+    @property
+    def spec(self) -> MapSpec:
+        return MapSpec(self.shape, self.dtype, self.device)
+
+
+def stage_rows_supported(layer, shape, dtype) -> bool:
+    ws = layer.window_size
+    return (len(layer.blocks) > 0 and not layer.training and dtype in (torch.float16, torch.bfloat16) and not getattr(layer, "dynamic_grid", False)
+            and shape[2] % ws == 0 and shape[3] % ws == 0 and shape[1] == layer.blocks[0].attn.qkv.in_features)
+
+
+def stage_rows(layer, shape, dtype, device) -> StageRows:
+    if not stage_rows_supported(layer, shape, dtype):
+        raise RuntimeError(f"stage_rows: a {tuple(shape)} {dtype} map is not a 16-bit map of whole {layer.window_size}-pixel windows of this level")
+    B, _, H, W = shape
+    lib = _lib.lib()
+    with torch.no_grad(), torch.cuda.device(device):
+        st = _state(layer, device)
+        with st.lock:
+            st, tb, ctables, dc = _prepare(layer, device, H, W)
+            wsp = _workspace(st, dc, B, H, W, device)
+            off, S, ncw = C.c_size_t(0), C.c_int32(0), C.c_int32(0)
+            _lib.check(lib.fvit_stage_rows_layout(C.byref(wsp.desc), C.byref(off), C.byref(S), C.byref(ncw)), "fvit_stage_rows_layout")
+            _acquire(wsp, device)
+    return StageRows(wsp.buf.data_ptr() + off.value, S.value, ncw.value, layer.window_size, tuple(shape), dtype, device, wsp)
+
+
 def pool_tail_supported(layer, x: torch.Tensor) -> bool:
     return bool(len(layer.blocks)) and not layer.blocks[0].do_sr_hat and x.shape[2] == x.shape[3] == layer.window_size and x.dtype in (torch.float16, torch.bfloat16)
 
@@ -632,7 +684,9 @@
 
 
 def stage_forward(layer, x: torch.Tensor, tokenizer=None, out: Optional[torch.Tensor] = None, ln2d=None,
-                  pool_out: Optional[torch.Tensor] = None) -> torch.Tensor:
+                  pool_out: Optional[torch.Tensor] = None, rows: Optional[StageRows] = None) -> torch.Tensor:
+    if rows is not None:
+        return _stage_forward_rows(layer, x, rows, out, ln2d, pool_out)
     _require_gpu(x, "FasterViTLayer")
     _check_mode(layer, x, "FasterViTLayer")
     if len(layer.blocks) == 0:
@@ -654,23 +708,7 @@
         with st.lock:
             st, tb, ctables, dc = _prepare(layer, x.device, Hp, Wp)
             wsp = _workspace(st, dc, B, H, W, x.device, bounded=bool(getattr(layer, "dynamic_grid", False)))
-            tail = None
-            if pool_out is not None:
-                if ln2d is not None or not pool_tail_supported(layer, x) or tuple(pool_out.shape) != (B, Cc) or pool_out.dtype != torch.float32 \
-                        or not pool_out.is_contiguous() or pool_out.device != x.device:
-                    raise RuntimeError("stage_forward: pool_out needs a contiguous fp32 (B, C) tensor, a 16-bit map of one window per image without "
-                                       "carrier tokens, and excludes ln2d")
-                tail = _lib.FvitStageTail(None, None, pool_out.data_ptr(), 0.0, _DT[x.dtype])
-            elif out is None:
-                out = torch.empty_like(x)
-            elif out.shape != x.shape or out.dtype != x.dtype or out.device != x.device:
-                raise RuntimeError(f"stage_forward: out {tuple(out.shape)} {out.dtype} does not match x {tuple(x.shape)} {x.dtype}")
-            if ln2d is not None:
-                ln_w, ln_b, eps = ln2d
-                if not ln2d_tail_supported(x, out) or any(t.dtype != torch.float32 or t.numel() < Cc or not t.is_contiguous() or t.device != x.device
-                                                          for t in (ln_w, ln_b)):
-                    raise RuntimeError("stage_forward: ln2d needs fp32 [C] parameters and a 16-bit channel-contiguous out with C % 8 == 0, C <= 512")
-                tail = _lib.FvitStageTail(ln_w.data_ptr(), ln_b.data_ptr(), None, float(eps), 0)
+            out, tail = _stage_tail(layer, x, out, ln2d, pool_out)
             vin = _map_view(xp)
             vout = _map_view(out) if pool_out is None else None
             stream = _acquire(wsp, x.device)
@@ -679,6 +717,58 @@
                                                  C.byref(tail) if tail is not None else None, wsp.buf.data_ptr(), wsp.buf.numel(), stream)
             _lib.check(rc, "fvit_hat_stage_forward")
             _release(wsp, x.device)
+        return out if pool_out is None else pool_out
+
+
+def _stage_tail(layer, x, out, ln2d, pool_out):
+    B, Cc = x.shape[:2]
+    tail = None
+    if pool_out is not None:
+        if ln2d is not None or not pool_tail_supported(layer, x) or tuple(pool_out.shape) != (B, Cc) or pool_out.dtype != torch.float32 \
+                or not pool_out.is_contiguous() or pool_out.device != x.device:
+            raise RuntimeError("stage_forward: pool_out needs a contiguous fp32 (B, C) tensor, a 16-bit map of one window per image without "
+                               "carrier tokens, and excludes ln2d")
+        tail = _lib.FvitStageTail(None, None, pool_out.data_ptr(), 0.0, _DT[x.dtype])
+    elif out is None:
+        out = torch.empty_like(x) if torch.is_tensor(x) else torch.empty(x.shape, dtype=x.dtype, device=x.device, memory_format=torch.channels_last)
+    elif tuple(out.shape) != tuple(x.shape) or out.dtype != x.dtype or out.device != x.device:
+        raise RuntimeError(f"stage_forward: out {tuple(out.shape)} {out.dtype} does not match x {tuple(x.shape)} {x.dtype}")
+    if ln2d is not None:
+        ln_w, ln_b, eps = ln2d
+        if not ln2d_tail_supported(x, out) or any(t.dtype != torch.float32 or t.numel() < Cc or not t.is_contiguous() or t.device != x.device
+                                                  for t in (ln_w, ln_b)):
+            raise RuntimeError("stage_forward: ln2d needs fp32 [C] parameters and a 16-bit channel-contiguous out with C % 8 == 0, C <= 512")
+        tail = _lib.FvitStageTail(ln_w.data_ptr(), ln_b.data_ptr(), None, float(eps), 0)
+    return out, tail
+
+
+def _stage_forward_rows(layer, x, rows: StageRows, out, ln2d, pool_out):
+    if not stage_rows_supported(layer, rows.shape, rows.dtype) or tuple(x.shape) != rows.shape or x.dtype != rows.dtype or x.device != rows.device:
+        raise RuntimeError(f"stage_forward: rows were laid out for a {rows.shape} {rows.dtype} map on {rows.device}, the call has "
+                           f"{tuple(x.shape)} {x.dtype} on {x.device}")
+    if torch.is_tensor(x):
+        _check_mode(layer, x, "FasterViTLayer")
+        _check_device(x, layer, "FasterViTLayer")
+    lib = _lib.lib()
+    with torch.no_grad(), torch.cuda.device(rows.device):
+        B, Cc, H, W = rows.shape
+        if layer.do_gt and layer.blocks[0].do_sr_hat:
+            if not torch.is_tensor(x):
+                raise RuntimeError("stage_forward: this level's TokenInitializer reads the 16-bit map; rows alone do not carry it")
+            token_init(layer.global_tokenizer, x, rows=rows)
+        st = _state(layer, rows.device)
+        with st.lock:
+            st, tb, ctables, dc = _prepare(layer, rows.device, H, W)
+            wsp = _workspace(st, dc, B, H, W, rows.device)
+            if wsp is not rows.wsp:
+                raise RuntimeError("stage_forward: rows belong to another workspace (slot or geometry changed since stage_rows)")
+            out, tail = _stage_tail(layer, x, out, ln2d, pool_out)
+            vout = _map_view(out) if pool_out is None else None
+            stream = _acquire(wsp, rows.device)
+            rc = lib.fvit_hat_stage_forward_rows(C.byref(wsp.desc), st.blocks_c, C.byref(ctables), C.byref(vout) if vout is not None else None,
+                                                 C.byref(tail) if tail is not None else None, wsp.buf.data_ptr(), wsp.buf.numel(), stream)
+            _lib.check(rc, "fvit_hat_stage_forward_rows")
+            _release(wsp, rows.device)
         return out if pool_out is None else pool_out
 
 
diff --git a/include/fvit_hip.h b/include/fvit_hip.h
--- a/include/fvit_hip.h
+++ b/include/fvit_hip.h
@@ -126,6 +126,10 @@
                                 const FvitStageTables* tables, const FvitMapView* in,
                                 const float* ct_init, const FvitMapView* out, const FvitStageTail* tail,
                                 void* workspace, size_t workspace_bytes, fvit_stream_t stream);
+int fvit_stage_rows_layout(const FvitStageDesc* desc, size_t* x_offset, int32_t* rows_per_win, int32_t* row_off);
+int fvit_hat_stage_forward_rows(const FvitStageDesc* desc, const FvitBlockWeights* blocks, const FvitStageTables* tables,
+                                const FvitMapView* out, const FvitStageTail* tail, void* workspace, size_t workspace_bytes,
+                                fvit_stream_t stream);
 int fvit_rows_avgpool(int32_t round_dtype, const float* x, float* out, int32_t B, int32_t rows, int32_t C, fvit_stream_t stream);
 
 int fvit_hat_block_forward(const FvitStageDesc* desc, const FvitBlockWeights* block,
@@ -135,6 +139,10 @@
 int fvit_token_init(const FvitMapView* in, const float* weight, const float* bias, float* ct_out, int32_t batch, int32_t C,
                     int32_t Hp, int32_t Wp, int32_t pool_kh, int32_t pool_kw, int32_t pool_sh, int32_t pool_sw, int32_t cw,
                     fvit_stream_t stream);
+
+int fvit_token_init_rows(const FvitMapView* in, const float* weight, const float* bias, float* rows, int32_t batch, int32_t C,
+                         int32_t Hp, int32_t Wp, int32_t pool_kh, int32_t pool_kw, int32_t pool_sh, int32_t pool_sw, int32_t cw,
+                         int32_t row_pitch, int32_t row_off, fvit_stream_t stream);
 
 int fvit_token_init_dyn(const FvitMapView* in, const float* weight, const float* bias, float* ct_out, int32_t batch, int32_t C,
                         int32_t Hp, int32_t Wp, int32_t pool_kh, int32_t pool_kw, int32_t pool_sh, int32_t pool_sw, int32_t cw,
@@ -283,6 +291,10 @@
 int fvit_conv3x3_nhwc_terms(int32_t dtype, const void* in, const void* weight, const float* bias, const void* residual,
                             void* out, int32_t B, int32_t Hi, int32_t Wi, int32_t Cin, int32_t Cout, int32_t stride,
                             int32_t act, int32_t weight_terms, const void* zeros, fvit_stream_t stream);
+
+int fvit_conv3x3_nhwc_rows(int32_t dtype, const void* in, const void* weight, const float* bias, void* out, float* rows, int32_t B,
+                           int32_t Hi, int32_t Wi, int32_t Cin, int32_t Cout, int32_t stride, int32_t ws, int32_t rows_per_win,
+                           int32_t row_off, const void* zeros, fvit_stream_t stream);
 
 int fvit_conv3x3_nhwc_px(int32_t dtype, const void* in, const void* in_lo, const void* weight, const float* bias, const void* residual,
                          const void* residual_lo, void* out, void* out_lo, float* out_f32, int32_t B, int32_t Hi, int32_t Wi, int32_t Cin,
```
